# Alxaline/BraTS21

Measured on AMD Instinct MI355X. Metric: train patches/sec (4x128^3, width-48), higher is better.
Workload: dtype bf16; 1 GPU; equiunet width=48, batch=2/GPU of 4x128^3 synthetic patches, fwd + deep-supervision Dice + bwd + ranger (BASELINE.json configs[1]); global_batch=2, parallelism=dp1

## Files before the change

### brats21_amd/csrc/conv_wgrad.hip

```cpp
#include <stdlib.h>
#include "twin_begin.hpp"
#include "common.hpp"

typedef __attribute__((ext_vector_type(4))) short s16x4;

struct WgradParams {
  const void* x1; const void* x2; int c1, c2, p1, p2;
  const void* dy; int dyp;
  float* ws;
  int N, D, H, W, cin, cout;
  int tz, ty, tx, ntiles, nsplit;
  int nlane;
  int ntaps, dil;
  int seglen, nsegz;
};

constexpr int WG_TZ = 4, WG_TY = 4, WG_TX = 16, WG_VOX = 256;

template <typename T, int DIL, int COF, int CIF, int KS = 3>
struct WgGeom {
  static constexpr bool BF = std::is_same<T, bf16_t>::value;
  static constexpr int ESZ = sizeof(T);
  static constexpr int EPL = 16 / ESZ;
  static constexpr int R = KS == 3 ? DIL : 0;
  static constexpr int HY = WG_TY + 2 * R, HX = WG_TX + 2 * R;
  static constexpr int HVOX = WG_TZ * HY * HX;
  static constexpr int CI_T = 16 * CIF, CO_T = 16 * COF;
  static constexpr int XROWB = CI_T * ESZ, YROWB = CO_T * ESZ;
  static constexpr int SX = BF ? (CIF == 1 ? 32 : 96) : XROWB + 16;
  static constexpr int SY = BF ? (COF == 1 ? 32 : 96) : YROWB + 16;
  static constexpr int XPPV = XROWB / 16, YPPV = YROWB / 16;
  static constexpr int XPPR = HX * XPPV, XIPR = (XPPR + 63) / 64, XROWS = WG_TZ * HY, XRPW = (XROWS + 3) / 4;
  static constexpr int YPPR = WG_TX * YPPV, YIPR = (YPPR + 63) / 64, YROWS = WG_TZ * WG_TY, YRPW = YROWS / 4;
  static constexpr int LDS_X = HVOX * SX, LDS_Y = WG_VOX * SY;
  static constexpr int LDS = LDS_X + LDS_Y;
  static constexpr int PAIRS = (KS == 3 ? 9 : 1) * CIF;
  static constexpr int PPW = (PAIRS + 3) / 4;
  static constexpr int NB = BF ? 32 : 64;
};

DEVI bf16x8 tr_pair(const char* p0, const char* p1) {
  const s16x4 lo = __builtin_amdgcn_ds_read_tr16_b64_v4i16((__attribute__((address_space(3))) s16x4*)p0);
  const s16x4 hi = __builtin_amdgcn_ds_read_tr16_b64_v4i16((__attribute__((address_space(3))) s16x4*)p1);
  typedef __attribute__((ext_vector_type(8))) short s16x8;
  const s16x8 v = {lo[0], lo[1], lo[2], lo[3], hi[0], hi[1], hi[2], hi[3]};
  return __builtin_bit_cast(bf16x8, v);
}

template <typename T, int DIL, int COF, int CIF, int KS = 3>
__global__ __launch_bounds__(256, 2) void conv_wgrad_kernel(const WgradParams p) {
  using G = WgGeom<T, DIL, COF, CIF, KS>;
  extern __shared__ __attribute__((aligned(16))) char lds[];
  char* ldx = lds;
  char* ldy = lds + G::LDS_X;
  const int tid = threadIdx.x, lane = tid & 63;
  const int wave = __builtin_amdgcn_readfirstlane(tid >> 6);
  const int q = lane >> 4, v = lane & 15;
  const int NP = KS == 3 ? 3 : p.ntaps;
  const int lane8 = blockIdx.x % p.nlane, rr = blockIdx.x / p.nlane;
  const int tzg = rr % NP, gsub = rr / NP, g8 = gridDim.x / (NP * p.nlane);
  const int shz = (KS == 3 || p.ntaps == 1) ? 0 : (tzg / 9 - 1) * p.dil;
  const int shy = (KS == 3 || p.ntaps == 1) ? 0 : ((tzg / 3) % 3 - 1) * p.dil;
  const int shx = (KS == 3 || p.ntaps == 1) ? 0 : (tzg % 3 - 1) * p.dil;
  const int split = lane8 + p.nlane * gsub;
  const int tpx = (p.ntiles + p.nlane - 1) / p.nlane;
  const int tile_end = min(p.ntiles, (lane8 + 1) * tpx);
  const int cot = blockIdx.y, cit = blockIdx.z;
  const int co0 = cot * G::CO_T, ci0 = cit * G::CI_T;
  const T* xsrc;
  int xpitch;
  if (ci0 < p.c1) { xsrc = (const T*)p.x1 + ci0; xpitch = p.p1; }
  else { xsrc = (const T*)p.x2 + (ci0 - p.c1); xpitch = p.p2; }
  const int ci_lim = (ci0 < p.c1 ? p.c1 : p.c1 + p.c2) - ci0;
  const int co_lim = p.cout - co0;

  int xhx[G::XIPR], xlo[G::XIPR];
  int xvo[G::XRPW][G::XIPR];
#pragma unroll
  for (int j = 0; j < G::XIPR; ++j) {
    const int pc = lane + 64 * j;
    const int hx = pc / G::XPPV, part = pc % G::XPPV;
    const bool ok = pc < G::XPPR && part * G::EPL < ci_lim;
    xhx[j] = ok ? hx : -100000;
    xlo[j] = pc < G::XPPR ? wave * (G::HX * G::SX) + hx * G::SX + part * 16 : -1;
#pragma unroll
    for (int k = 0; k < G::XRPW; ++k) {
      const int row = wave + 4 * k;
      xvo[k][j] = (((row / G::HY) * p.H + row % G::HY) * p.W + hx) * xpitch * G::ESZ + part * 16;
    }
  }
  int yvx[G::YIPR], ylo[G::YIPR];
  int yvo[G::YRPW][G::YIPR];
#pragma unroll
  for (int j = 0; j < G::YIPR; ++j) {
    const int pc = lane + 64 * j;
    const int vx = pc / G::YPPV, part = pc % G::YPPV;
    const bool ok = pc < G::YPPR && part * G::EPL < co_lim;
    yvx[j] = ok ? vx : 100000;
    ylo[j] = pc < G::YPPR ? wave * (WG_TX * G::SY) + vx * G::SY + part * 16 : -1;
#pragma unroll
    for (int k = 0; k < G::YRPW; ++k) {
      const int row = wave + 4 * k;
      yvo[k][j] = (((row / WG_TY) * p.H + row % WG_TY) * p.W + vx) * p.dyp * G::ESZ + part * 16;
    }
  }
  const unsigned xsample_bytes = (unsigned)p.D * p.H * p.W * xpitch * G::ESZ;
  const unsigned ysample_bytes = (unsigned)p.D * p.H * p.W * p.dyp * G::ESZ;

  int poff[G::PPW];
#pragma unroll
  for (int jj = 0; jj < G::PPW; ++jj) {
    const int pid = wave + 4 * jj;
    const int t9 = pid / CIF, nn = pid % CIF;
    poff[jj] = pid < G::PAIRS ? (((t9 / 3) * G::R) * G::HX + (t9 % 3) * G::R) * G::SX + nn * G::NB : 0;
  }
  f32x4 acc[G::PPW][COF];
#pragma unroll
  for (int jj = 0; jj < G::PPW; ++jj)
#pragma unroll
    for (int m = 0; m < COF; ++m) acc[jj][m] = f32x4{0.f, 0.f, 0.f, 0.f};

  u32x4 rx[G::XRPW][G::XIPR], ry[G::YRPW][G::YIPR];
  auto issue_loads = [&](int tile) {
    int bt = tile;
    const int x0 = (bt % p.tx) * WG_TX; bt /= p.tx;
    const int y0 = (bt % p.ty) * WG_TY; bt /= p.ty;
    const int z0 = (bt % p.tz) * WG_TZ;
    const int n = bt / p.tz;
    const int gz0 = KS == 3 ? z0 + (tzg - 1) * DIL : z0 + shz;
    const int gy0 = KS == 3 ? y0 - DIL : y0 + shy, gx0 = KS == 3 ? x0 - DIL : x0 + shx;
    const size_t sample_vox = (size_t)n * p.D * p.H * p.W;
    const __amdgpu_buffer_rsrc_t xrs = __builtin_amdgcn_make_buffer_rsrc((void*)(xsrc + sample_vox * xpitch), (short)0,
                                                                          (int)xsample_bytes, 0x00020000);
    const __amdgpu_buffer_rsrc_t yrs = __builtin_amdgcn_make_buffer_rsrc((void*)((const T*)p.dy + sample_vox * p.dyp + co0),
                                                                          (short)0, (int)ysample_bytes, 0x00020000);
    const int xorg = ((gz0 * p.H + gy0) * p.W + gx0) * xpitch * G::ESZ;
    const int yorg = ((z0 * p.H + y0) * p.W + x0) * p.dyp * G::ESZ;
    bool xok[G::XIPR], yok[G::YIPR];
#pragma unroll
    for (int j = 0; j < G::XIPR; ++j) xok[j] = (unsigned)(gx0 + xhx[j]) < (unsigned)p.W;
#pragma unroll
    for (int j = 0; j < G::YIPR; ++j) yok[j] = x0 + yvx[j] < p.W;
#pragma unroll
    for (int k = 0; k < G::XRPW; ++k) {
      const int row = wave + 4 * k;
      const int gz = gz0 + row / G::HY, gy = gy0 + row % G::HY;
      const bool row_ok = row < G::XROWS && (unsigned)gz < (unsigned)p.D && (unsigned)gy < (unsigned)p.H;
#pragma unroll
      for (int j = 0; j < G::XIPR; ++j) {
        const int vo = (row_ok && xok[j]) ? xorg + xvo[k][j] : -1;
        rx[k][j] = __builtin_bit_cast(u32x4, __builtin_amdgcn_raw_buffer_load_b128(xrs, vo, 0, 0));
      }
    }
#pragma unroll
    for (int k = 0; k < G::YRPW; ++k) {
      const int row = wave + 4 * k;
      const bool row_ok = z0 + row / WG_TY < p.D && y0 + row % WG_TY < p.H;
#pragma unroll
      for (int j = 0; j < G::YIPR; ++j) {
        const int vo = (row_ok && yok[j]) ? yorg + yvo[k][j] : -1;
        ry[k][j] = __builtin_bit_cast(u32x4, __builtin_amdgcn_raw_buffer_load_b128(yrs, vo, 0, 0));
      }
    }
  };
  constexpr bool PREFETCH = !(G::BF && KS == 3 && DIL == 2 && COF * CIF == 9);
  const int tile_first = lane8 * tpx + gsub;
  if (PREFETCH && tile_first < tile_end) issue_loads(tile_first);
// ... 117 lines not shown
  const int ci_lim = (ci0 < p.c1 ? p.c1 : p.c1 + p.c2) - ci0;
  const T* xsrc;
  int xpitch;
  if (ci0 < p.c1) { xsrc = (const T*)p.x1 + ci0; xpitch = p.p1; }
  else { xsrc = (const T*)p.x2 + (ci0 - p.c1); xpitch = p.p2; }

  int xcode[G::XI], ycode[G::YI];
#pragma unroll
  for (int i = 0; i < G::XI; ++i) {
    const int P = tid + 512 * i;
    const int vox = P / G::XPPV, part = P % G::XPPV;
    const int hx = vox % G::HX, hy = (vox / G::HX) % G::HY, hz = vox / (G::HX * G::HY);
    xcode[i] = (P < G::XPIECES && part * 8 < ci_lim) ? (hz | hy << 3 | hx << 6 | part << 11 | 1 << 14) : 0;
  }
#pragma unroll
  for (int i = 0; i < G::YI; ++i) {
    const int P = tid + 512 * i;
    const int vox = P / G::YPPV, part = P % G::YPPV;
    ycode[i] = (vox >> 6) | ((vox >> 4) & 3) << 3 | (vox & 15) << 6 | part << 11 | 1 << 14;
  }
  const unsigned xsample_bytes = (unsigned)p.D * p.H * p.W * xpitch * 2;
  const unsigned ysample_bytes = (unsigned)p.D * p.H * p.W * p.dyp * 2;

  int poff[G::PPW];
#pragma unroll
  for (int jj = 0; jj < G::PPW; ++jj) {
    const int pid = wave + 8 * jj;
    const int t = pid / CIF, nn = pid % CIF;
    poff[jj] = pid < G::PAIRS ? (((t / 9) * G::HY + (t / 3) % 3) * G::HX + t % 3) * G::SX + nn * 32 : 0;
  }
  f32x4 acc[G::PPW][COF];
#pragma unroll
  for (int jj = 0; jj < G::PPW; ++jj)
#pragma unroll
    for (int m = 0; m < COF; ++m) acc[jj][m] = f32x4{0.f, 0.f, 0.f, 0.f};

  u32x4 rx[G::XI], ry[G::YI];
  auto issue_loads = [&](int tile) {
    int bt = tile;
    const int x0 = (bt % p.tx) * WG_TX; bt /= p.tx;
    const int y0 = (bt % p.ty) * WG_TY; bt /= p.ty;
    const int z0 = (bt % p.tz) * WG_TZ;
    const int n = bt / p.tz;
    const size_t sample_vox = (size_t)n * p.D * p.H * p.W;
    const __amdgpu_buffer_rsrc_t xrs = __builtin_amdgcn_make_buffer_rsrc((void*)(xsrc + sample_vox * xpitch), (short)0,
                                                                          (int)xsample_bytes, 0x00020000);
    const __amdgpu_buffer_rsrc_t yrs = __builtin_amdgcn_make_buffer_rsrc((void*)((const T*)p.dy + sample_vox * p.dyp + co0),
                                                                          (short)0, (int)ysample_bytes, 0x00020000);
    unsigned zm = 0, ym = 0, xm = 0, zy = 0, yy = 0, xy = 0;
#pragma unroll
    for (int h = 0; h < G::HZ; ++h) zm |= ((unsigned)(z0 - 1 + h) < (unsigned)p.D ? 1u : 0u) << h;
#pragma unroll
    for (int h = 0; h < G::HY; ++h) ym |= ((unsigned)(y0 - 1 + h) < (unsigned)p.H ? 1u : 0u) << h;
#pragma unroll
    for (int h = 0; h < G::HX; ++h) xm |= ((unsigned)(x0 - 1 + h) < (unsigned)p.W ? 1u : 0u) << h;
    zy = zm >> 1; yy = ym >> 1; xy = xm >> 1;
    const int xorg = ((z0 - 1) * p.H + (y0 - 1)) * p.W + (x0 - 1);
    const int yorg = (z0 * p.H + y0) * p.W + x0;
    const int xpb = xpitch * 2, ypb = p.dyp * 2;
#pragma unroll
    for (int i = 0; i < G::XI; ++i) {
      int c = xcode[i];
      asm volatile("" : "+v"(c));
      const unsigned ok = (unsigned)(c >> 14) & (zm >> (c & 7)) & (ym >> ((c >> 3) & 7)) & (xm >> ((c >> 6) & 31)) & 1u;
      const int pv = ((c & 7) * p.H + ((c >> 3) & 7)) * p.W + ((c >> 6) & 31);
      const int vo = ok ? (xorg + pv) * xpb + ((c >> 11) & 7) * 16 : -1;
      rx[i] = __builtin_bit_cast(u32x4, __builtin_amdgcn_raw_buffer_load_b128(xrs, vo, 0, 0));
    }
#pragma unroll
    for (int i = 0; i < G::YI; ++i) {
      int c = ycode[i];
      asm volatile("" : "+v"(c));
      const unsigned ok = (zy >> (c & 7)) & (yy >> ((c >> 3) & 7)) & (xy >> ((c >> 6) & 31)) & 1u;
      const int pv = ((c & 7) * p.H + ((c >> 3) & 7)) * p.W + ((c >> 6) & 31);
      const int vo = ok ? (yorg + pv) * ypb + ((c >> 11) & 7) * 16 : -1;
      ry[i] = __builtin_bit_cast(u32x4, __builtin_amdgcn_raw_buffer_load_b128(yrs, vo, 0, 0));
    }
  };

  const int tile_first = lane8 * tpx + gsub;
  if (tile_first < tile_end) issue_loads(tile_first);
  for (int tile = tile_first; tile < tile_end; tile += g8) {
    __syncthreads();
#pragma unroll
    for (int i = 0; i < G::XI; ++i)
      if (tid + 512 * i < G::XPIECES) *(u32x4*)(ldx + (tid + 512 * i) * 16) = rx[i];
#pragma unroll
    for (int i = 0; i < G::YI; ++i) {
      const int P = tid + 512 * i;
      *(u32x4*)(ldy + (P / G::YPPV) * G::SY + (P % G::YPPV) * 16) = ry[i];
    }
    __syncthreads();
    if (tile + g8 < tile_end) issue_loads(tile + g8);
    __builtin_amdgcn_sched_barrier(0);
    const int qq = v >> 2, pp = v & 3;
    const int ybase = (4 * q + qq) * G::SY + pp * 8;
    const int xbase = (4 * q + qq) * G::SX + pp * 8;
    constexpr int PD = 2;
    bf16x8 a[2][COF], b[PD + 1];
    auto read_a = [&](auto s_) {
      constexpr int s = s_;
      const int yoff = ybase + (32 * s) * G::SY;
#pragma unroll
      for (int m = 0; m < COF; ++m) a[s & 1][m] = tr_pair(ldy + yoff + m * 32, ldy + yoff + 16 * G::SY + m * 32);
    };
    auto read_b = [&](auto u_) {
      constexpr int u = u_;
      constexpr int s = u / G::PPW, jj = u % G::PPW;
      const int xoff = xbase + (((s >> 1) * G::HY + 2 * (s & 1)) * G::HX) * G::SX + poff[jj];
      b[u % (PD + 1)] = tr_pair(ldx + xoff, ldx + xoff + G::HX * G::SX);
    };
    constexpr int NU = 8 * G::PPW;
    read_a(std::integral_constant<int, 0>{});
    static_for<0, PD>([&](auto u_) { read_b(u_); });
    static_for<0, NU>([&](auto u_) {
      constexpr int u = u_;
      constexpr int s = u / G::PPW, jj = u % G::PPW;
      if constexpr (u + PD < NU) read_b(std::integral_constant<int, u + PD>{});
      if constexpr (jj == 0 && s + 1 < 8) read_a(std::integral_constant<int, s + 1>{});
      __builtin_amdgcn_sched_barrier(0);
#pragma unroll
      for (int m = 0; m < COF; ++m)
        acc[jj][m] = MFMA16_16x16x32(a[s & 1][m], b[u % (PD + 1)], acc[jj][m]);
      __builtin_amdgcn_sched_barrier(0);
    });
  }

#pragma unroll
  for (int jj = 0; jj < G::PPW; ++jj) {
    const int pid = wave + 8 * jj;
    if (pid < G::PAIRS) {
      const int t = pid / CIF, nn = pid % CIF;
      float* base = p.ws + ((size_t)split * 27 + t) * p.cout * p.cin;
      const int ci = ci0 + nn * 16 + v;
      if (nn * 16 + v < ci_lim) {
#pragma unroll
        for (int m = 0; m < COF; ++m)
#pragma unroll
          for (int r = 0; r < 4; ++r) base[(size_t)(co0 + m * 16 + 4 * q + r) * p.cin + ci] = acc[jj][m][r];
      }
    }
  }
}

template <int COF, int CIF> struct Wg3b {
  static constexpr int HZ = WG_TZ + 2, HY = WG_TY + 2, HX = WG_TX + 2, HVOX = HZ * HY * HX;
  static constexpr int CO = 16 * COF, CI = 16 * CIF;
  static constexpr int SX = 2 * CI, SY = 2 * CO, XPPV = CI / 8, YPPV = CO / 8;
  static constexpr int XPIECES = HVOX * XPPV, YPIECES = WG_VOX * YPPV;
  static constexpr int XI = (XPIECES + 511) / 512, YI = YPIECES / 512;
  static constexpr int XB = XI * 512 * 16;
  static constexpr int LDS = 2 * XB + WG_VOX * SY;
  static constexpr int PAIRS = 27 * CIF, PPW = (PAIRS + 7) / 8;
  static_assert(YPIECES % 512 == 0, "");
};

template <int COF, int CIF>
__global__ __launch_bounds__(512, 1) void conv_wgrad_alltaps2_kernel(const WgradParams p) {
  typedef bf16_t T;
  using G = Wg3b<COF, CIF>;
  extern __shared__ __attribute__((aligned(16))) char lds[];
  char* ldy = lds + 2 * G::XB;
  const int tid = threadIdx.x, lane = tid & 63;
  const int wave = __builtin_amdgcn_readfirstlane(tid >> 6);
  const int q = lane >> 4, v = lane & 15;
  const int lane8 = blockIdx.x % p.nlane, gsub = blockIdx.x / p.nlane, g8 = gridDim.x / p.nlane;
  const int split = blockIdx.x;
  const int tpx = (p.ntiles + p.nlane - 1) / p.nlane;
  const int tile_end = min(p.ntiles, (lane8 + 1) * tpx);
  const int co0 = blockIdx.y * G::CO, ci0 = blockIdx.z * G::CI;
  const T* xsrc;
  int xpitch;
  if (ci0 < p.c1) { xsrc = (const T*)p.x1 + ci0; xpitch = p.p1; }
  else { xsrc = (const T*)p.x2 + (ci0 - p.c1); xpitch = p.p2; }
  const int xpb = xpitch * 2, ypb = p.dyp * 2;

  int xoffs[G::XI], xcode[G::XI];
#pragma unroll
  for (int i = 0; i < G::XI; ++i) {
    const int P = tid + 512 * i;
    const int vox = P / G::XPPV, part = P % G::XPPV;
    const int hx = vox % G::HX, hy = (vox / G::HX) % G::HY, hz = vox / (G::HX * G::HY);
    const bool ok = P < G::XPIECES && (CIF > 1 || part * 8 < p.c1);
    xoffs[i] = ok ? ((hz * p.H + hy) * p.W + hx) * xpb + part * 16 : (int)0x80000000;
    xcode[i] = ok ? (hz | hy << 3 | hx << 6 | 1 << 14) : 0;
  }
  const unsigned xsample_bytes = (unsigned)p.D * p.H * p.W * xpitch * 2;
  const unsigned ysample_bytes = (unsigned)p.D * p.H * p.W * p.dyp * 2;

  int poff[G::PPW];
#pragma unroll
  for (int jj = 0; jj < G::PPW; ++jj) {
    const int pid = wave + 8 * jj;
    const int t = pid / CIF, nn = pid % CIF;
    poff[jj] = pid < G::PAIRS ? (((t / 9) * G::HY + (t / 3) % 3) * G::HX + t % 3) * G::SX + nn * 32 : 0;
  }
  f32x4 acc[G::PPW][COF];
#pragma unroll
  for (int jj = 0; jj < G::PPW; ++jj)
#pragma unroll
    for (int m = 0; m < COF; ++m) acc[jj][m] = f32x4{0.f, 0.f, 0.f, 0.f};

  u32x4 ry[G::YI];
  struct TileLoads {
    rsrc4_t xrs;
    __amdgpu_buffer_rsrc_t yrs;
    int xorg, yorg;
    unsigned zm, ym, xm, inter;
    char* xdst;
  };
  auto setup_loads = [&](int tile, int buf) {
    TileLoads L;
    int bt = tile;
    const int x0 = (bt % p.tx) * WG_TX; bt /= p.tx;
    const int y0 = (bt % p.ty) * WG_TY; bt /= p.ty;
    const int z0 = (bt % p.tz) * WG_TZ;
    const int n = bt / p.tz;
    const size_t sample_vox = (size_t)n * p.D * p.H * p.W;
    L.xrs = make_rsrc4(xsrc + sample_vox * xpitch, xsample_bytes);
    L.yrs = __builtin_amdgcn_make_buffer_rsrc((void*)((const T*)p.dy + sample_vox * p.dyp + co0), (short)0, (int)ysample_bytes, 0x00020000);
    L.xorg = (((z0 - 1) * p.H + (y0 - 1)) * p.W + (x0 - 1)) * xpb;
    L.yorg = ((z0 * p.H + y0) * p.W + x0) * ypb;
    L.xdst = lds + buf * G::XB + wave * 1024;
    auto inside = [](int o, int size, int hn) {
      const int lo = o >= 1 ? 0 : 1 - o, hi = size - o + 1 < hn ? size - o + 1 : hn;
      return hi > lo ? ((1u << hi) - 1u) & ~((1u << lo) - 1u) : 0u;
    };
    L.zm = inside(z0, p.D, G::HZ); L.ym = inside(y0, p.H, G::HY); L.xm = inside(x0, p.W, G::HX);
    L.inter = (L.zm == (1u << G::HZ) - 1 && L.ym == (1u << G::HY) - 1 && L.xm == (1u << G::HX) - 1) ? 1u : 0u;
    return L;
  };
  auto issue_x = [&](const TileLoads& L, auto i_) {
    constexpr int i = i_;
    const int c = xcode[i];
    const unsigned ok = (unsigned)(c >> 14) & (L.inter | ((L.zm >> (c & 7)) & (L.ym >> ((c >> 3) & 7)) & (L.xm >> ((c >> 6) & 31)))) & 1u;
    lds_dma16_async(L.xrs, L.xdst + i * 8192, (L.xorg + xoffs[i]) | ((int)ok - 1));
  };
  auto issue_y = [&](const TileLoads& L, auto i_) {
    constexpr int i = i_;
    const int P = tid + 512 * i;
    const int vox = P / G::YPPV, part = P % G::YPPV;
    const int z = vox >> 6, y = (vox >> 4) & 3, x = vox & 15;
    const int yo = ((z * p.H + y) * p.W + x) * ypb + part * 16;
    const unsigned ok = (L.inter | ((L.zm >> (z + 1)) & (L.ym >> (y + 1)) & (L.xm >> (x + 1)))) & 1u;
    ry[i] = __builtin_bit_cast(u32x4, __builtin_amdgcn_raw_buffer_load_b128(L.yrs, (L.yorg + yo) | ((int)ok - 1), 0, 0));
  };

  const int tile_first = lane8 * tpx + gsub;
  const int qq = v >> 2, pp = v & 3;
  const int ybase = (4 * q + qq) * G::SY + pp * 8;
  const int xbase = (4 * q + qq) * G::SX + pp * 8;
  int cur = 0;
#ifdef BRATS_WGRAD_STAMPS
  long long tacc[5] = {0, 0, 0, 0, 0}, tlast = __builtin_amdgcn_s_memtime();
#define WG_STAMP(i) do { const long long t_ = __builtin_amdgcn_s_memtime(); tacc[i] += t_ - tlast; tlast = t_; } while (0)
#else
#define WG_STAMP(i) do { } while (0)
#endif
  if (tile_first < tile_end) {
    const TileLoads L = setup_loads(tile_first, 0);
    static_for<0, G::XI>([&](auto i_) { issue_x(L, i_); });
    static_for<0, G::YI>([&](auto i_) { issue_y(L, i_); });
  }
  for (int tile = tile_first; tile < tile_end; tile += g8, cur ^= 1) {
    WG_STAMP(4);
    asm volatile("s_waitcnt vmcnt(0)" ::: "memory");
    WG_STAMP(0);
    __syncthreads();
    WG_STAMP(1);
#pragma unroll
    for (int i = 0; i < G::YI; ++i) *(u32x4*)(ldy + (tid + 512 * i) * 16) = ry[i];
    __syncthreads();
    WG_STAMP(2);
    const bool more = tile + g8 < tile_end;
    TileLoads L = setup_loads(more ? tile + g8 : tile, cur ^ 1);
    if (!more) L.zm = L.inter = 0;
    __builtin_amdgcn_sched_barrier(0);
    WG_STAMP(3);
    const char* ldx = lds + cur * G::XB;
    constexpr int PD = 3;
    bf16x8 a[2][COF], b[PD + 1];
    auto read_a = [&](auto s_) {
      constexpr int s = s_;
      const int yoff = ybase + (32 * s) * G::SY;
#pragma unroll
      for (int m = 0; m < COF; ++m) a[s & 1][m] = tr_pair(ldy + yoff + m * 32, ldy + yoff + 16 * G::SY + m * 32);
    };
    auto read_b = [&](auto u_) {
      constexpr int u = u_;
      constexpr int s = u / G::PPW, jj = u % G::PPW;
      const int xoff = xbase + (((s >> 1) * G::HY + 2 * (s & 1)) * G::HX) * G::SX + poff[jj];
      b[u % (PD + 1)] = tr_pair(ldx + xoff, ldx + xoff + G::HX * G::SX);
    };
    constexpr int NU = 8 * G::PPW;
    static_for<0, G::XI>([&](auto i_) { issue_x(L, i_); });
    static_for<0, G::YI>([&](auto i_) { issue_y(L, i_); });
    __builtin_amdgcn_sched_barrier(0);
    read_a(std::integral_constant<int, 0>{});
    static_for<0, PD>([&](auto u_) { read_b(u_); });
    static_for<0, NU>([&](auto u_) {
      constexpr int u = u_;
      constexpr int s = u / G::PPW, jj = u % G::PPW;
      if constexpr (u + PD < NU) read_b(std::integral_constant<int, u + PD>{});
      if constexpr (jj == 0 && s + 1 < 8) read_a(std::integral_constant<int, s + 1>{});
      __builtin_amdgcn_sched_barrier(0);
#pragma unroll
      for (int m = 0; m < COF; ++m)
        acc[jj][m] = MFMA16_16x16x32(a[s & 1][m], b[u % (PD + 1)], acc[jj][m]);
      __builtin_amdgcn_sched_barrier(0);
    });
  }

#ifdef BRATS_WGRAD_STAMPS
  WG_STAMP(4);
  if (lane == 0 && blockIdx.y == 0 && blockIdx.z == 0) {
    long long* st = (long long*)(p.ws + (size_t)gridDim.x * 27 * p.cout * p.cin) + ((size_t)blockIdx.x * 8 + wave) * 5;
    for (int i = 0; i < 5; ++i) st[i] = tacc[i];
  }
#endif
#pragma unroll
  for (int jj = 0; jj < G::PPW; ++jj) {
    const int pid = wave + 8 * jj;
    if (pid < G::PAIRS) {
      const int t = pid / CIF, nn = pid % CIF;
      float* base = p.ws + ((size_t)split * 27 + t) * p.cout * p.cin;
      const int ci = ci0 + nn * 16 + v;
      if (CIF > 1 || ci < p.cin) {
#pragma unroll
        for (int m = 0; m < COF; ++m)
#pragma unroll
          for (int r = 0; r < 4; ++r) base[(size_t)(co0 + m * 16 + 4 * q + r) * p.cin + ci] = acc[jj][m][r];
      }
    }
  }
}

template <int COF, int CIF> struct Wg3f {
  static constexpr int HZ = WG_TZ + 2, HY = WG_TY + 2, HX = WG_TX + 2, HVOX = HZ * HY * HX;
  static constexpr int CO = 16 * COF, CI = 16 * CIF;
  static constexpr int SX = CI, SY = CO;
  static constexpr int XPPV = CI / 8, YPPV = CO / 8;
  static constexpr int XPIECES = HVOX * XPPV, YPIECES = WG_VOX * YPPV;
  static constexpr int XI = (XPIECES + 511) / 512, YI = YPIECES / 512;
  static constexpr int XB = XI * 512 * 16, YB = YI * 512 * 16;
  static constexpr int LDS_X = HVOX * SX;
  static constexpr int LDS = XB + YB + LDS_X + WG_VOX * SY;
  static constexpr int PAIRS = 27 * CIF, PPW = (PAIRS + 7) / 8;
  static_assert(YPIECES % 512 == 0, "");
};

template <int STRIDE> DEVI i32x8 tr8_frag(const char* base, int o0, int o1) {
  typedef __attribute__((ext_vector_type(2))) int v2i;
  typedef __attribute__((address_space(3))) v2i* lp;
  const v2i a0 = __builtin_amdgcn_ds_read_tr8_b64_v2i32((lp)(base + o0));
  const v2i a1 = __builtin_amdgcn_ds_read_tr8_b64_v2i32((lp)(base + o0 + 8 * STRIDE));
  const v2i a2 = __builtin_amdgcn_ds_read_tr8_b64_v2i32((lp)(base + o1));
  const v2i a3 = __builtin_amdgcn_ds_read_tr8_b64_v2i32((lp)(base + o1 + 8 * STRIDE));
  return i32x8{a0[0], a0[1], a1[0], a1[1], a2[0], a2[1], a3[0], a3[1]};
}

struct WgradF8Params { WgradParams w; const float* amax_x1; const float* amax_x2; const float* amax_dy; };

template <int COF, int CIF>
__global__ __launch_bounds__(512, 1) void conv_wgrad_alltaps_f8_kernel(const WgradF8Params pp) {
  typedef bf16_t T;
  using G = Wg3f<COF, CIF>;
  const WgradParams& p = pp.w;
  extern __shared__ __attribute__((aligned(16))) char lds[];
  char* ldx = lds + G::XB + G::YB;
  char* ldy = ldx + G::LDS_X;
  const int tid = threadIdx.x, lane = tid & 63;
  const int wave = __builtin_amdgcn_readfirstlane(tid >> 6);
  const int kq = lane >> 4, L = lane & 15;
  const int lane8 = blockIdx.x % p.nlane, gsub = blockIdx.x / p.nlane, g8 = gridDim.x / p.nlane;
  const int split = blockIdx.x;
  const int tpx = (p.ntiles + p.nlane - 1) / p.nlane;
  const int tile_end = min(p.ntiles, (lane8 + 1) * tpx);
  const int co0 = blockIdx.y * G::CO, ci0 = blockIdx.z * G::CI;
  const T* xsrc;
  int xpitch;
  if (ci0 < p.c1) { xsrc = (const T*)p.x1 + ci0; xpitch = p.p1; }
  else { xsrc = (const T*)p.x2 + (ci0 - p.c1); xpitch = p.p2; }
  const int xpb = xpitch * 2, ypb = p.dyp * 2;
  float ax = *pp.amax_x1;
  if (pp.amax_x2) ax = fmaxf(ax, *pp.amax_x2);
  const float xs = f8_scale_from_amax(ax), ys = f8_scale_from_amax(*pp.amax_dy);

  int xoffs[G::XI], xcode[G::XI];
#pragma unroll
  for (int i = 0; i < G::XI; ++i) {
    const int P = tid + 512 * i;
    const int vox = P / G::XPPV, part = P % G::XPPV;
    const int hx = vox % G::HX, hy = (vox / G::HX) % G::HY, hz = vox / (G::HX * G::HY);
    const bool ok = P < G::XPIECES;
    xoffs[i] = ok ? ((hz * p.H + hy) * p.W + hx) * xpb + part * 16 : (int)0x80000000;
    xcode[i] = ok ? (hz | hy << 3 | hx << 6 | 1 << 14) : 0;
  }
  const unsigned xsample_bytes = (unsigned)p.D * p.H * p.W * xpitch * 2;
  const unsigned ysample_bytes = (unsigned)p.D * p.H * p.W * p.dyp * 2;

  int poff[G::PPW];
#pragma unroll
  for (int jj = 0; jj < G::PPW; ++jj) {
    const int pid = wave + 8 * jj;
    const int t = pid / CIF, nn = pid % CIF;
    poff[jj] = pid < G::PAIRS ? (((t / 9) * G::HY + (t / 3) % 3) * G::HX + t % 3) * G::SX + nn * 16 : 0;
  }
  f32x4 acc[G::PPW][COF];
#pragma unroll
  for (int jj = 0; jj < G::PPW; ++jj)
#pragma unroll
    for (int m = 0; m < COF; ++m) acc[jj][m] = f32x4{0.f, 0.f, 0.f, 0.f};

  struct TileLoads {
    rsrc4_t xrs, yrs;
    int xorg, yorg;
    unsigned zm, ym, xm, inter;
  };
  auto setup_loads = [&](int tile) {
    TileLoads T_;
    int bt = tile;
    const int x0 = (bt % p.tx) * WG_TX; bt /= p.tx;
    const int y0 = (bt % p.ty) * WG_TY; bt /= p.ty;
    const int z0 = (bt % p.tz) * WG_TZ;
    const int n = bt / p.tz;
    const size_t sample_vox = (size_t)n * p.D * p.H * p.W;
    T_.xrs = make_rsrc4(xsrc + sample_vox * xpitch, xsample_bytes);
    T_.yrs = make_rsrc4((const T*)p.dy + sample_vox * p.dyp + co0, ysample_bytes);
    T_.xorg = (((z0 - 1) * p.H + (y0 - 1)) * p.W + (x0 - 1)) * xpb;
    T_.yorg = ((z0 * p.H + y0) * p.W + x0) * ypb;
    auto inside = [](int o, int size, int hn) {
      const int lo = o >= 1 ? 0 : 1 - o, hi = size - o + 1 < hn ? size - o + 1 : hn;
      return hi > lo ? ((1u << hi) - 1u) & ~((1u << lo) - 1u) : 0u;
    };
    T_.zm = inside(z0, p.D, G::HZ); T_.ym = inside(y0, p.H, G::HY); T_.xm = inside(x0, p.W, G::HX);
    T_.inter = (T_.zm == (1u << G::HZ) - 1 && T_.ym == (1u << G::HY) - 1 && T_.xm == (1u << G::HX) - 1) ? 1u : 0u;
    return T_;
  };
  char* const xdst = lds + wave * 1024;
  auto issue_x = [&](const TileLoads& T_, auto i_) {
    constexpr int i = i_;
    int c = xcode[i];
    OPAQUE_V(c);
    const unsigned ok = (unsigned)(c >> 14) & (T_.inter | ((T_.zm >> (c & 7)) & (T_.ym >> ((c >> 3) & 7)) & (T_.xm >> ((c >> 6) & 31)))) & 1u;
    lds_dma16_async(T_.xrs, xdst + i * 8192, (T_.xorg + xoffs[i]) | ((int)ok - 1));
  };
  auto issue_y = [&](const TileLoads& T_, auto i_) {
    constexpr int i = i_;
    int t_ = tid;
    OPAQUE_V(t_);
    const int P = t_ + 512 * i;
    const int vox = P / G::YPPV, part = P % G::YPPV;
    const int z = vox >> 6, y = (vox >> 4) & 3, x = vox & 15;
    const int yo = ((z * p.H + y) * p.W + x) * ypb + part * 16;
    const unsigned ok = (T_.inter | ((T_.zm >> (z + 1)) & (T_.ym >> (y + 1)) & (T_.xm >> (x + 1)))) & 1u;
    lds_dma16_async(T_.yrs, xdst + G::XB + i * 8192, (T_.yorg + yo) | ((int)ok - 1));
  };

  int xl[2], yl[2];
#pragma unroll
  for (int e = 0; e < 2; ++e) {
    const int r = 2 * kq + e;
    xl[e] = (((r >> 2) * G::HY + (r & 3)) * G::HX + (L >> 1)) * G::SX + (L & 1) * 8;
    yl[e] = (r * 16 + (L >> 1)) * G::SY + (L & 1) * 8;
  }

  const int tile_first = lane8 * tpx + gsub;
  if (tile_first < tile_end) {
    const TileLoads T_ = setup_loads(tile_first);
    static_for<0, G::XI>([&](auto i_) { issue_x(T_, i_); });
    static_for<0, G::YI>([&](auto i_) { issue_y(T_, i_); });
  }
  for (int tile = tile_first; tile < tile_end; tile += g8) {
    asm volatile("s_waitcnt vmcnt(0)" ::: "memory");
    u32x2 qx[G::XI], qy[G::YI];
#pragma unroll
    for (int i = 0; i < G::XI; ++i) qx[i] = f8_quant8(*(const u32x4*)(lds + (tid + 512 * i) * 16), xs);
#pragma unroll
    for (int i = 0; i < G::YI; ++i) qy[i] = f8_quant8(*(const u32x4*)(lds + G::XB + (tid + 512 * i) * 16), ys);
    __syncthreads();
#pragma unroll
    for (int i = 0; i < G::XI; ++i)
      if (i + 1 < G::XI || tid + 512 * i < G::XPIECES) *(u32x2*)(ldx + (tid + 512 * i) * 8) = qx[i];
#pragma unroll
    for (int i = 0; i < G::YI; ++i) *(u32x2*)(ldy + (tid + 512 * i) * 8) = qy[i];
    __syncthreads();
    const bool more = tile + g8 < tile_end;
// ... 7 lines not shown
      constexpr int ks = ks_;
      const char* xk = ldx + ks * (2 * G::HY * G::HX * G::SX);
      i32x8 a[COF];
#pragma unroll
      for (int m = 0; m < COF; ++m) a[m] = tr8_frag<G::SY>(ldy + ks * (8 * 16 * G::SY) + m * 16, yl[0], yl[1]);
      i32x8 b[2];
      auto read_b = [&](auto jj_) {
        constexpr int jj = jj_;
        int o[2] = {xl[0] + poff[jj], xl[1] + poff[jj]};
        OPAQUE_V(o[0]); OPAQUE_V(o[1]);
        b[jj & 1] = tr8_frag<G::SX>(xk, o[0], o[1]);
      };
      read_b(std::integral_constant<int, 0>{});
      static_for<0, G::PPW>([&](auto jj_) {
        constexpr int jj = jj_;
        if constexpr (jj + 1 < G::PPW) read_b(std::integral_constant<int, jj + 1>{});
        __builtin_amdgcn_sched_barrier(0);
#pragma unroll
        for (int m = 0; m < COF; ++m)
          acc[jj][m] = __builtin_amdgcn_mfma_scale_f32_16x16x128_f8f6f4(a[m], b[jj & 1], acc[jj][m], 0, 0, 0, 0, 0, 0);
        __builtin_amdgcn_sched_barrier(0);
      });
    });
  }

  const float os = xs * ys;
#pragma unroll
  for (int jj = 0; jj < G::PPW; ++jj) {
    const int pid = wave + 8 * jj;
    if (pid < G::PAIRS) {
      const int t = pid / CIF, nn = pid % CIF;
      float* base = p.ws + ((size_t)split * 27 + t) * p.cout * p.cin;
      const int ci = ci0 + nn * 16 + L;
#pragma unroll
      for (int m = 0; m < COF; ++m)
#pragma unroll
        for (int r = 0; r < 4; ++r) base[(size_t)(co0 + m * 16 + 4 * kq + r) * p.cin + ci] = acc[jj][m][r] * os;
    }
  }
}

__global__ void __launch_bounds__(256) wgrad_reduce_kernel(const float* __restrict__ ws, float* __restrict__ dw, int nsplit,
                                                           int cout, int cin, int taps, const float* __restrict__ amax) {
  const size_t per = (size_t)taps * cout * cin;
  const size_t per4 = per / 4;
  const int e = threadIdx.x & 31, g = threadIdx.x >> 5;
  const size_t i4 = (size_t)blockIdx.x * 32 + e;
  f32x4 s = {0.f, 0.f, 0.f, 0.f};
  if (i4 < per4) {
    const float* src = ws + i4 * 4;
    int k = g;
    for (; k + 56 < nsplit; k += 64) {
      f32x4 v[8];
#pragma unroll
      for (int u = 0; u < 8; ++u) v[u] = *(const f32x4*)(src + (size_t)(k + 8 * u) * per);
#pragma unroll
      for (int u = 0; u < 8; ++u) s += v[u];
    }
    for (; k < nsplit; k += 8) s += *(const f32x4*)(src + (size_t)k * per);
  }
  __shared__ f32x4 part[8][32];
  part[g][e] = s;
  __syncthreads();
  if (g == 0 && i4 < per4) {
#pragma unroll
    for (int k = 1; k < 8; ++k) s += part[k][e];
    if (amax) s *= x3_inv_scale(x3_scale_from_amax(*amax));
    const size_t i = i4 * 4;
    const int ci = i % cin;
    const int co = (i / cin) % cout;
    const int tap = (int)(i / ((size_t)cin * cout));
#pragma unroll
    for (int j = 0; j < 4; ++j) dw[((size_t)co * cin + ci + j) * taps + tap] = s[j];
  }
}

__global__ void __launch_bounds__(256) wgrad_reduce_taps_kernel(const float* __restrict__ ws, float* __restrict__ dw, int nsplit,
                                                                int cout, int cin, int taps, const float* __restrict__ amax) {
  extern __shared__ __attribute__((aligned(16))) float red_tile[];
  const size_t per = (size_t)taps * cout * cin, pairs4 = (size_t)cout * cin / 4;
  const int e = threadIdx.x & 31, g = threadIdx.x >> 5;
  const size_t p4 = (size_t)blockIdx.x * 32 + e;
  if (p4 < pairs4) {
    f32x4 s[4];
#pragma unroll
    for (int t = 0; t < 4; ++t) s[t] = f32x4{0.f, 0.f, 0.f, 0.f};
    for (int k0 = 0; k0 < nsplit; k0 += 8) {
      f32x4 v[4][8];
#pragma unroll
      for (int t = 0; t < 4; ++t) {
        const int tap = g + 8 * t;
        const float* src = ws + ((size_t)(tap < taps ? tap : 0) * cout * cin + p4 * 4);
#pragma unroll
        for (int u = 0; u < 8; ++u)
          v[t][u] = (tap < taps && k0 + u < nsplit) ? *(const f32x4*)(src + (size_t)(k0 + u) * per) : f32x4{0.f, 0.f, 0.f, 0.f};
      }
#pragma unroll
      for (int t = 0; t < 4; ++t)
#pragma unroll
        for (int u = 0; u < 8; ++u)
          if (k0 + u < nsplit) s[t] += v[t][u];
    }
#pragma unroll
    for (int t = 0; t < 4; ++t)
      if (g + 8 * t < taps) *(f32x4*)(red_tile + (g + 8 * t) * 128 + e * 4) = s[t];
  }
  __syncthreads();
  const size_t pair0 = (size_t)blockIdx.x * 128, npairs = (size_t)cout * cin;
  float* dst = dw + pair0 * taps;
  const float isc = amax ? x3_inv_scale(x3_scale_from_amax(*amax)) : 1.f;
  for (int i = threadIdx.x; i < 128 * taps; i += blockDim.x) {
    const int pr = i / taps, tap = i % taps;
    if (pair0 + pr < npairs) dst[i] = red_tile[tap * 128 + pr] * isc;
  }
}

static void wgrad_reduce_launch(const float* ws, float* dw, int nsplit, int cout, int cin, int taps, hipStream_t st,
                                const float* amax = nullptr) {
  const size_t per = (size_t)taps * cout * cin;
  const size_t tblocks = ((size_t)cout * cin / 4 + 31) / 32;
  if (taps > 1 && taps <= 32 && tblocks >= 256)
    hipLaunchKernelGGL(wgrad_reduce_taps_kernel, dim3((unsigned)tblocks), dim3(256), (size_t)taps * 128 * sizeof(float), st, ws, dw,
                       nsplit, cout, cin, taps, amax);
  else
    hipLaunchKernelGGL(wgrad_reduce_kernel, dim3((unsigned)((per / 4 + 31) / 32)), dim3(256), 0, st, ws, dw, nsplit, cout, cin, taps, amax);
}

template <typename T>
__global__ void dbias_kernel(const T* __restrict__ dy, int pitch, float* __restrict__ db, size_t voxels, int C) {
  __shared__ float red[256];
  const int c = blockIdx.x;
  float s = 0.f;
  for (size_t v = threadIdx.x; v < voxels; v += blockDim.x) s += to_f<T>(dy[v * pitch + c]);
  red[threadIdx.x] = s;
  __syncthreads();
  for (int m = 128; m > 0; m >>= 1) {
    if ((int)threadIdx.x < m) red[threadIdx.x] += red[threadIdx.x + m];
    __syncthreads();
  }
  if (threadIdx.x == 0) db[c] = red[0];
}
static void wgrad_dbias_launch(int dtype, const void* dy, int dypitch, float* dbias, size_t vox, int cout, hipStream_t st) {
  with_storage(dtype, [&](auto t) {
    using T = typename decltype(t)::type;
    hipLaunchKernelGGL(dbias_kernel<T>, dim3(cout), dim3(256), 0, st, (const T*)dy, dypitch, dbias, vox, cout);
  });
}

struct WgradArgs {
  const void* x1; int c1, p1;
  const void* x2; int c2, p2;
  const void* dy; int dyp;
  int N, D, H, W, cout;
  int cin() const { return c1 + c2; }
  size_t vox() const { return (size_t)N * D * H * W; }
};
static WgradArgs wgrad_shape(int N, int D, int H, int W, int c1, int c2, int cout) {
  return WgradArgs{nullptr, c1, 0, nullptr, c2 > 0 ? c2 : 0, 0, nullptr, 0, N, D, H, W, cout};
}
static int wgrad_sample_overflow(const WgradArgs& a, int esize) {
  const int mp = a.p1 > a.p2 ? (a.p1 > a.dyp ? a.p1 : a.dyp) : (a.p2 > a.dyp ? a.p2 : a.dyp);
  return (double)a.D * a.H * a.W * mp * esize >= 2147483648.0 ? mp : 0;
}

struct WgradTileGrid { int tz, ty, tx, ntiles; };
static WgradTileGrid wgrad_tile_grid(const WgradArgs& a, int TZ = WG_TZ, int TY = WG_TY, int TX = WG_TX) {
  WgradTileGrid t{ceil_div(a.D, TZ), ceil_div(a.H, TY), ceil_div(a.W, TX), 0};
  t.ntiles = a.N * t.tz * t.ty * t.tx;
  return t;
}
static WgradParams wgrad_params(const WgradArgs& a, float* ws, const WgradTileGrid& t, int nlane, int nsplit, int ntaps, int dil) {
  WgradParams p{};
  p.x1 = a.x1; p.x2 = a.x2; p.c1 = a.c1; p.c2 = a.c2; p.p1 = a.p1; p.p2 = a.p2;
  p.dy = a.dy; p.dyp = a.dyp; p.ws = ws;
  p.N = a.N; p.D = a.D; p.H = a.H; p.W = a.W; p.cin = a.cin(); p.cout = a.cout;
  p.tz = t.tz; p.ty = t.ty; p.tx = t.tx; p.ntiles = t.ntiles;
  p.nlane = nlane; p.nsplit = nsplit; p.ntaps = ntaps; p.dil = dil;
  return p;
}

static int wgrad_nlane(int ntiles) {
  int nl = 8;
  while (nl > 1 && ntiles / nl < 16) nl >>= 1;
  return nl;
}
static int wgrad_split_g8(int ntiles, int nlane, int groups, int cot, int cit) {
  int g8 = ceil_div(512, groups * nlane * cot * cit);
  const int cap = ceil_div(ntiles, nlane);
  if (g8 > cap) g8 = cap;
  return g8 < 1 ? 1 : g8;
}
static bool wgrad_blocks_g8(int ntiles, int blocks, int* nlane, int* g8) {
  *nlane = wgrad_nlane(ntiles);
  *g8 = ceil_div(device_cus(), *nlane * blocks);
  if (*g8 < 1) *g8 = 1;
  return ntiles >= 4 * *nlane * *g8;
}
static void wgrad_tiles(int dtype, int c1, int c2, int cout, int* cof, int* cif) {
  const int co16 = ceil_div(cout, 16);
  *cof = co16 % 3 == 0 ? 3 : (co16 % 2 == 0 ? 2 : 1);
  if (dtype == BRATS_F32) { *cif = 1; return; }
  const int a = ceil_div(c1, 16), b = c2 > 0 ? ceil_div(c2, 16) : 0;
  auto ok = [&](int f) { return a % f == 0 && (b == 0 || b % f == 0); };
  *cif = ok(3) ? 3 : (ok(2) ? 2 : 1);
}

int g_wgrad_alltaps_mode = -1;
extern "C" int BRATS_API(brats_conv3d_set_wgrad_alltaps)(int mode) {
  const int old = g_wgrad_alltaps_mode;
  g_wgrad_alltaps_mode = mode < 0 ? -1 : (mode ? 1 : 0);
  return old;
}
static int wgrad_alltaps_mode() {
  static int env_mode = -1;
  if (env_mode < 0) {
    const char* e = getenv("BRATS_WGRAD_ALLTAPS");
    env_mode = e ? atoi(e) : 1;
  }
  return g_wgrad_alltaps_mode >= 0 ? g_wgrad_alltaps_mode : env_mode;
}

enum WgradForm {
  WG_TAP_PLANE, WG_SHIFTED_TAP,
  WG_ALLTAPS2_33, WG_ALLTAPS2_42, WG_ALLTAPS2_31,
  WG_ALLTAPS_1, WG_ALLTAPS_1_4,
  WG_F8_33, WG_F8_42
};
struct WgradPlan {
  WgradForm form;
  int cof, cif;
  int cot, cit;
  int nlane, g8, nsplit;
  int ntaps, groups;
  bool clear;
  WgradTileGrid tiles;
  size_t per;
  size_t slab_bytes() const { return nsplit * per * sizeof(float); }
};

static WgradPlan wgrad_plan(int dtype, bool shifted, int ksize, int dil, const WgradArgs& a) {
  WgradPlan pl;
  const int c1 = a.c1, c2 = a.c2, cin = a.cin(), cout = a.cout;
  pl.tiles = wgrad_tile_grid(a);
  pl.ntaps = ksize == 3 ? 27 : 1;
  pl.per = (size_t)pl.ntaps * cout * cin;
  const bool narrow = c2 == 0 && c1 <= 16;
  auto blocks_of = [&](int co, int ci) { return cout % co == 0 && (narrow || (c1 % ci == 0 && c2 % ci == 0)); };
  if (!shifted && wgrad_alltaps_mode() && dtype == BRATS_BF16 && dil == 1 && (blocks_of(48, 48) || blocks_of(64, 32))) {
    const bool wide = !blocks_of(48, 48);
    pl.cof = wide ? 4 : 3; pl.cif = narrow ? 1 : (wide ? 2 : 3);
    pl.cot = cout / (16 * pl.cof); pl.cit = narrow ? 1 : cin / (16 * pl.cif);
    if (wgrad_blocks_g8(pl.tiles.ntiles, pl.cot * pl.cit, &pl.nlane, &pl.g8)) {
      pl.form = wide ? (narrow ? WG_ALLTAPS_1_4 : WG_ALLTAPS2_42) : narrow ? (c1 % 8 == 0 ? WG_ALLTAPS2_31 : WG_ALLTAPS_1) : WG_ALLTAPS2_33;
      pl.groups = 1;
      pl.clear = false;
      pl.nsplit = pl.nlane * pl.g8;
      return pl;
    }
  }
  pl.form = shifted ? WG_SHIFTED_TAP : WG_TAP_PLANE;
  wgrad_tiles(dtype, c1, c2, cout, &pl.cof, &pl.cif);
  pl.cot = ceil_div(cout, 16 * pl.cof);
  pl.cit = ceil_div(c1, 16 * pl.cif) + (c2 > 0 ? ceil_div(c2, 16 * pl.cif) : 0);
  pl.groups = shifted ? pl.ntaps : 3;
  pl.nlane = wgrad_nlane(pl.tiles.ntiles);
  pl.g8 = wgrad_split_g8(pl.tiles.ntiles, pl.nlane, pl.groups, pl.cot, pl.cit);
  pl.nsplit = pl.nlane * pl.g8;
  pl.clear = cin % 16 || cout % 16;
  return pl;
}
static size_t wgrad_slab_room(int dtype, bool shifted, int ksize, const WgradArgs& a) {
  const size_t d1 = wgrad_plan(dtype, shifted, ksize, 1, a).slab_bytes();
  const size_t d2 = shifted ? 0 : wgrad_plan(dtype, shifted, ksize, 2, a).slab_bytes();
  return d1 > d2 ? d1 : d2;
}

template <typename T, int DIL, int COF, int CIF, int KS = 3>
static int wgrad_launch(const WgradParams& p, dim3 grid, hipStream_t st) {
  using G = WgGeom<T, DIL, COF, CIF, KS>;
  auto kern = conv_wgrad_kernel<T, DIL, COF, CIF, KS>;
  static std::atomic<uint64_t> attr_done{0};
  BRATS_ENSURE_LDS_ATTR(kern, G::LDS, attr_done);
  hipLaunchKernelGGL(kern, grid, dim3(256), G::LDS, st, p);
  BRATS_CHECK_LAUNCH();
  return 0;
}

template <typename T, int DIL, int KS = 3>
static int wgrad_dispatch(const WgradParams& p, int cof, int cif, dim3 grid, hipStream_t st) {
#define WG_CASE(A, B) if (cof == A && cif == B) return wgrad_launch<T, DIL, A, B, KS>(p, grid, st);
  WG_CASE(3, 1) WG_CASE(2, 1) WG_CASE(1, 1)
  if constexpr (std::is_same<T, bf16_t>::value) {
    WG_CASE(3, 3) WG_CASE(3, 2) WG_CASE(2, 3) WG_CASE(2, 2) WG_CASE(1, 3) WG_CASE(1, 2)
  }
#undef WG_CASE
  BRATS_FAIL(BRATS_E_UNSUPPORTED, "wgrad: unsupported tile %dx%d", cof, cif);
}

template <auto KERN, int LDS>
static int wgrad_alltaps_launch(const WgradParams& p, dim3 grid, hipStream_t st) {
  static std::atomic<uint64_t> attr_done{0};
  BRATS_ENSURE_LDS_ATTR(KERN, LDS, attr_done);
  hipLaunchKernelGGL(KERN, grid, dim3(512), LDS, st, p);
  BRATS_CHECK_LAUNCH();
  return 0;
}

static int wgrad_run(const WgradPlan& pl, int dtype, int dil, const WgradArgs& a, float* ws, size_t room, hipStream_t st) {
  const char* who = pl.form == WG_SHIFTED_TAP ? "wgrad_shift" : "wgrad";
  if (a.c2 > 0 && a.c1 % (16 * pl.cif)) BRATS_FAIL(BRATS_E_UNSUPPORTED, "wgrad: c1=%d must be a multiple of the ci tile %d", a.c1, 16 * pl.cif);
  if (pl.slab_bytes() > room) BRATS_FAIL(BRATS_E_ARG, "%s: the plan's %zu bytes of slabs exceed the workspace size %zu", who, pl.slab_bytes(), room);
  const WgradParams p = wgrad_params(a, ws, pl.tiles, pl.nlane, pl.nsplit, pl.ntaps, dil);
  if (pl.clear) {
    hipError_t e = hipMemsetAsync(ws, 0, pl.slab_bytes(), st);
    if (e != hipSuccess) BRATS_FAIL(BRATS_E_HIP, "%s: memset: %s", who, hipGetErrorString(e));
  }
  const dim3 grid(pl.groups * pl.nsplit, pl.cot, pl.cit);
  const bool bf = dtype == BRATS_BF16;
  switch (pl.form) {
    case WG_TAP_PLANE:
      if (bf) return dil == 1 ? wgrad_dispatch<bf16_t, 1>(p, pl.cof, pl.cif, grid, st) : wgrad_dispatch<bf16_t, 2>(p, pl.cof, pl.cif, grid, st);
      return dil == 1 ? wgrad_dispatch<float, 1>(p, pl.cof, pl.cif, grid, st) : wgrad_dispatch<float, 2>(p, pl.cof, pl.cif, grid, st);
    case WG_SHIFTED_TAP:
      return bf ? wgrad_dispatch<bf16_t, 1, 1>(p, pl.cof, pl.cif, grid, st) : wgrad_dispatch<float, 1, 1>(p, pl.cof, pl.cif, grid, st);
    case WG_ALLTAPS2_33: return wgrad_alltaps_launch<conv_wgrad_alltaps2_kernel<3, 3>, Wg3b<3, 3>::LDS>(p, grid, st);
    case WG_ALLTAPS2_42: return wgrad_alltaps_launch<conv_wgrad_alltaps2_kernel<4, 2>, Wg3b<4, 2>::LDS>(p, grid, st);
    case WG_ALLTAPS2_31: return wgrad_alltaps_launch<conv_wgrad_alltaps2_kernel<3, 1>, Wg3b<3, 1>::LDS>(p, grid, st);
    case WG_ALLTAPS_1: return wgrad_alltaps_launch<conv_wgrad_alltaps_kernel<1>, Wg3<1>::LDS>(p, grid, st);
    case WG_ALLTAPS_1_4: return wgrad_alltaps_launch<conv_wgrad_alltaps_kernel<1, 4>, Wg3<1, 4>::LDS>(p, grid, st);
    default: BRATS_FAIL(BRATS_E_UNSUPPORTED, "wgrad: form %d is not a 16-bit / f32 kernel", (int)pl.form);
  }
}

template <int V>
__global__ void __launch_bounds__(256) x3_split_kernel(const float* __restrict__ src, int pitch, bf16_t* __restrict__ hi,
                                                       bf16_t* __restrict__ lo, size_t voxels, int C, const float* __restrict__ amax) {
  const float sc = amax ? x3_scale_from_amax(*amax) : 1.f;
  const int cv = C / 8;
  const size_t total = voxels * cv;
  const size_t stride = (size_t)gridDim.x * 256;
  auto load = [&](size_t i, u32x4& a, u32x4& b) {
    const float* p = src + (i / cv) * pitch + (i % cv) * 8;
    a = __builtin_nontemporal_load((const u32x4*)p);
    b = __builtin_nontemporal_load((const u32x4*)(p + 4));
  };
  auto emit = [&](size_t i, const u32x4& a, const u32x4& b) {
    const uint32_t w[8] = {a[0], a[1], a[2], a[3], b[0], b[1], b[2], b[3]};
    uint32_t h[4], l[4];
#pragma unroll
    for (int e = 0; e < 4; ++e) {
      const float x0 = __uint_as_float(w[2 * e]) * sc, x1 = __uint_as_float(w[2 * e + 1]) * sc;
      x3_split2(x0, x1, h[e], l[e]);
    }
    const size_t o = (i / cv) * C + (i % cv) * 8;
    __builtin_nontemporal_store(u32x4{h[0], h[1], h[2], h[3]}, (u32x4*)(hi + o));
    __builtin_nontemporal_store(u32x4{l[0], l[1], l[2], l[3]}, (u32x4*)(lo + o));
  };
  size_t i = (size_t)blockIdx.x * 256 + threadIdx.x;
  for (; i + stride < total; i += 2 * stride) {
    u32x4 a0, b0, a1, b1;
    load(i, a0, b0);
    load(i + stride, a1, b1);
    emit(i, a0, b0);
    emit(i + stride, a1, b1);
  }
  if (i < total) {
    u32x4 a0, b0;
    load(i, a0, b0);
    emit(i, a0, b0);
  }
}
static size_t x3_align(size_t b) { return (b + 255) / 256 * 256; }
static void x3_split_launch(const float* src, int pitch, bf16_t* hi, bf16_t* lo, size_t vox, int c, const float* amax, hipStream_t st) {
  const size_t total = vox * (c / 8);
  size_t nb = (total + 511) / 512;
  const unsigned blocks = (unsigned)(nb < 1 ? 1 : (nb > 262144 ? 262144 : nb));
  hipLaunchKernelGGL(x3_split_kernel<0>, dim3(blocks), dim3(256), 0, st, src, pitch, hi, lo, vox, c, amax);
}

struct X3Carve {
  size_t off[7];
  X3Carve(size_t room16, const WgradArgs& a) {
    const int c[3] = {a.c1, a.c2, a.cout};
    size_t b = x3_align(3 * room16);
    for (int i = 0; i < 6; ++i) {
      off[i] = b;
      b += c[i / 2] > 0 ? x3_align(a.vox() * c[i / 2] * 2) : 0;
    }
    off[6] = b;
  }
  size_t bytes() const { return off[6]; }
  bf16_t* at(float* ws, int i) const { return (bf16_t*)((char*)ws + off[i]); }
};

static int wgrad_x3(const WgradPlan& pl, int dil, const WgradArgs& a, const float* amax_dy, float* ws, float* dw, size_t room16,
                          hipStream_t st) {
  const X3Carve cv(room16, a);
  bf16_t *h1 = cv.at(ws, 0), *l1 = cv.at(ws, 1), *h2 = cv.at(ws, 2), *l2 = cv.at(ws, 3), *hy = cv.at(ws, 4), *ly = cv.at(ws, 5);
  x3_split_launch((const float*)a.x1, a.p1, h1, l1, a.vox(), a.c1, nullptr, st);
  if (a.c2 > 0) x3_split_launch((const float*)a.x2, a.p2, h2, l2, a.vox(), a.c2, nullptr, st);
  x3_split_launch((const float*)a.dy, a.dyp, hy, ly, a.vox(), a.cout, amax_dy, st);
  BRATS_CHECK_LAUNCH();
  WgradArgs t = a;
  t.p1 = a.c1; t.p2 = a.c2; t.dyp = a.cout;
  const bool xlo[3] = {true, false, false}, ylo[3] = {false, true, false};
  for (int k = 0; k < 3; ++k) {
    t.x1 = xlo[k] ? l1 : h1;
    t.x2 = a.c2 > 0 ? (xlo[k] ? l2 : h2) : nullptr;
    t.dy = ylo[k] ? ly : hy;
    const int rc = wgrad_run(pl, BRATS_BF16, dil, t, ws + (size_t)k * pl.nsplit * pl.per, room16, st);
    if (rc) return rc;
  }
  wgrad_reduce_launch((const float*)ws, dw, 3 * pl.nsplit, a.cout, a.cin(), pl.ntaps, st, amax_dy);
  return 0;
}

#include "conv_wgrad_x3.hpp"
extern "C" int BRATS_API(brats_conv3d_set_x3_wgrad_fused)(int mode) {
  const int old = g_x3_wgrad_fused_mode;
  g_x3_wgrad_fused_mode = mode < 0 ? -1 : (mode > 2 ? 2 : mode);
  return old;
}

static size_t wgrad_ws_bytes(int dtype, bool shifted, int ksize, const WgradArgs& a) {
  if (dtype != BRATS_X3_BF16) return wgrad_slab_room(dtype, shifted, ksize, a);
  const size_t three = X3Carve(wgrad_slab_room(BRATS_BF16, shifted, ksize, a), a).bytes();
  const size_t fused = shifted ? 0 : wgrad_x3_fused_ws_bytes(a);
  return three > fused ? three : fused;
}
extern "C" size_t BRATS_API(brats_conv3d_wgrad_ws_bytes)(int dtype, int ksize, int N, int D, int H, int W, int c1, int c2, int cout) {
  return ksize == 3 ? wgrad_ws_bytes(dtype, false, 3, wgrad_shape(N, D, H, W, c1, c2, cout)) : 0;
}
extern "C" size_t BRATS_API(brats_conv3d_wgrad_shift_ws_bytes)(int dtype, int ksize, int N, int D, int H, int W, int cin, int cout) {
  return ksize == 1 || ksize == 3 ? wgrad_ws_bytes(dtype, true, ksize, wgrad_shape(N, D, H, W, cin, 0, cout)) : 0;
}

static int wgrad_impl(bool shifted, WgradArgs a, const float* amax_dy, float* ws, float* dw, float* dbias, int dtype, int ksize, int dil,
                      brats_stream_t s) {
  const char* who = shifted ? "wgrad_shift" : "wgrad";
  if (!a.x1 || !a.dy || !ws || !dw || a.c1 <= 0 || a.cout <= 0 || (shifted && (a.N <= 0 || a.D <= 0 || a.H <= 0 || a.W <= 0)))
    BRATS_FAIL(BRATS_E_ARG, "%s: null pointer / bad size", who);
  if (shifted ? (ksize != 1 && ksize != 3) || dil < 1 : ksize != 3 || (dil != 1 && dil != 2))
    BRATS_FAIL(BRATS_E_UNSUPPORTED, "%s: ksize=%d dil=%d unsupported", who, ksize, dil);
  if (shifted && dtype != BRATS_BF16 && dtype != BRATS_F32 && dtype != BRATS_X3_BF16) BRATS_FAIL(BRATS_E_UNSUPPORTED, "wgrad_shift: dtype %d", dtype);
  if (a.c2 < 0) a.c2 = 0;
  if (a.c2 > 0 && !a.x2) BRATS_FAIL(BRATS_E_ARG, "wgrad: c2 > 0 but x2 NULL");
  const bool x3 = dtype == BRATS_X3_BF16;
  const int epl = vec_width(dtype);
  if (a.p1 % epl || (a.c2 && a.p2 % epl) || a.dyp % epl || a.c1 % epl || a.c2 % epl || a.cout % epl)
    BRATS_FAIL(BRATS_E_ARG, "%s: channel counts / pitches must be multiples of %d", who, epl);
  if (x3 && (a.c1 % 8 || a.c2 % 8 || a.cout % 8)) BRATS_FAIL(BRATS_E_ARG, "%s (split precision): channel counts must be multiples of 8", who);
  if (const int mp = wgrad_sample_overflow(a, dtype == BRATS_BF16 ? 2 : 4))
    BRATS_FAIL(BRATS_E_UNSUPPORTED, "%s: one sample of %dx%dx%d x pitch %d exceeds the 2 GiB buffer-offset range", who, a.D, a.H, a.W, mp);
  hipStream_t st = (hipStream_t)s;
  int rc = x3 && !shifted ? wgrad_x3_fused(a, amax_dy, ws, dw, dil, st) : 1;
  if (rc == 1) {
    const int dt = x3 ? BRATS_BF16 : dtype;
    const WgradPlan pl = wgrad_plan(dt, shifted, ksize, dil, a);
    const size_t room = wgrad_slab_room(dt, shifted, ksize, a);
    if (x3) rc = wgrad_x3(pl, dil, a, amax_dy, ws, dw, room, st);
    else if (!(rc = wgrad_run(pl, dtype, dil, a, ws, room, st))) wgrad_reduce_launch((const float*)ws, dw, pl.nsplit, a.cout, a.cin(), pl.ntaps, st);
  }
  if (rc) return rc;
  if (dbias) wgrad_dbias_launch(dtype, a.dy, a.dyp, dbias, a.vox(), a.cout, st);
  BRATS_CHECK_LAUNCH();
  return 0;
}

extern "C" int BRATS_API(brats_conv3d_wgrad)(const void* x1, int c1, int pitch1, const void* x2, int c2, int pitch2, const void* dy,
                                  int dypitch, float* ws, float* dw, float* dbias, int dtype, int ksize, int dil, int N,
                                  int D, int H, int W, int cout, brats_stream_t s) {
  return wgrad_impl(false, WgradArgs{x1, c1, pitch1, x2, c2, pitch2, dy, dypitch, N, D, H, W, cout}, nullptr, ws, dw, dbias, dtype, ksize, dil, s);
}
extern "C" int BRATS_API(brats_conv3d_x3_wgrad)(const void* x1, int c1, int pitch1, const void* x2, int c2, int pitch2, const void* dy,
                                     int dypitch, const float* amax_dy, float* ws, float* dw, float* dbias, int dtype, int dil,
                                     int N, int D, int H, int W, int cout, brats_stream_t s) {
  if (dtype != BRATS_X3_BF16) BRATS_FAIL(BRATS_E_ARG, "conv3d_x3_wgrad: dtype must be BRATS_X3_F16 or BRATS_X3_BF16");
  return wgrad_impl(false, WgradArgs{x1, c1, pitch1, x2, c2, pitch2, dy, dypitch, N, D, H, W, cout}, amax_dy, ws, dw, dbias, dtype, 3, dil, s);
}
extern "C" int BRATS_API(brats_conv3d_wgrad_shift)(const void* x, int cin, int xpitch, const void* dy, int dypitch, float* ws, float* dw,
                                        float* dbias, int dtype, int ksize, int dil, int N, int D, int H, int W, int cout,
                                        brats_stream_t s) {
  return wgrad_impl(true, WgradArgs{x, cin, xpitch, nullptr, 0, 0, dy, dypitch, N, D, H, W, cout}, nullptr, ws, dw, dbias, dtype, ksize, dil, s);
}
extern "C" int BRATS_API(brats_conv3d_x3_wgrad_shift)(const void* x, int cin, int xpitch, const void* dy, int dypitch, const float* amax_dy,
                                           float* ws, float* dw, float* dbias, int dtype, int ksize, int dil, int N, int D, int H,
                                           int W, int cout, brats_stream_t s) {
  if (dtype != BRATS_X3_BF16) BRATS_FAIL(BRATS_E_ARG, "conv3d_x3_wgrad_shift: dtype must be BRATS_X3_F16 or BRATS_X3_BF16");
  return wgrad_impl(true, WgradArgs{x, cin, xpitch, nullptr, 0, 0, dy, dypitch, N, D, H, W, cout}, amax_dy, ws, dw, dbias, dtype, ksize, dil, s);
}

static bool wgrad_f8_plan(const WgradArgs& a, WgradPlan* pl) {
  const int c1 = a.c1, c2 = a.c2, cout = a.cout;
  if (c1 <= 0 || cout <= 0) return false;
  if (cout % 48 == 0 && c1 % 48 == 0 && c2 % 48 == 0) { pl->form = WG_F8_33; pl->cof = 3; pl->cif = 3; }
  else if (cout % 64 == 0 && c1 % 32 == 0 && c2 % 32 == 0) { pl->form = WG_F8_42; pl->cof = 4; pl->cif = 2; }
  else return false;
  pl->tiles = wgrad_tile_grid(a);
  pl->cot = cout / (16 * pl->cof); pl->cit = a.cin() / (16 * pl->cif);
  if (!wgrad_blocks_g8(pl->tiles.ntiles, pl->cot * pl->cit, &pl->nlane, &pl->g8)) return false;
  pl->nsplit = pl->nlane * pl->g8;
  pl->ntaps = 27; pl->groups = 1; pl->clear = false;
  pl->per = (size_t)27 * cout * a.cin();
  return true;
}

extern "C" size_t BRATS_API(brats_conv3d_wgrad_f8_ws_bytes)(int N, int D, int H, int W, int c1, int c2, int cout) {
  WgradPlan pl;
  return wgrad_f8_plan(wgrad_shape(N, D, H, W, c1, c2, cout), &pl) ? pl.slab_bytes() : 0;
}

template <int COF, int CIF>
static int wgrad_f8_launch(const WgradF8Params& pp, dim3 grid, hipStream_t st) {
  using G = Wg3f<COF, CIF>;
  auto kern = conv_wgrad_alltaps_f8_kernel<COF, CIF>;
  static std::atomic<uint64_t> attr_done{0};
  BRATS_ENSURE_LDS_ATTR(kern, G::LDS, attr_done);
  hipLaunchKernelGGL(kern, grid, dim3(512), G::LDS, st, pp);
  BRATS_CHECK_LAUNCH();
  return 0;
}

extern "C" int BRATS_API(brats_conv3d_wgrad_f8)(const void* x1, int c1, int pitch1, const float* amax1, const void* x2, int c2, int pitch2,
                                     const float* amax2, const void* dy, int dypitch, const float* amax_dy, float* ws, float* dw,
                                     int N, int D, int H, int W, int cout, brats_stream_t s) {
  if (!x1 || !dy || !ws || !dw || !amax1 || !amax_dy || c1 <= 0 || cout <= 0) BRATS_FAIL(BRATS_E_ARG, "wgrad_f8: null pointer / bad size");
  if (c2 < 0) c2 = 0;
  if (c2 > 0 && (!x2 || !amax2)) BRATS_FAIL(BRATS_E_ARG, "wgrad_f8: c2 > 0 needs x2 and its |max|");
  const WgradArgs a{x1, c1, pitch1, x2, c2, pitch2, dy, dypitch, N, D, H, W, cout};
  WgradPlan pl;
  if (!wgrad_f8_plan(a, &pl))
    BRATS_FAIL(BRATS_E_UNSUPPORTED, "wgrad_f8: built for 48 x 48 / 64 x 32 channel blocks of layers with enough tiles "
               "(brats_conv3d_wgrad_f8_ws_bytes() == 0 otherwise): use brats_conv3d_wgrad");
  if (pitch1 % 8 || (c2 && pitch2 % 8) || dypitch % 8) BRATS_FAIL(BRATS_E_ARG, "wgrad_f8: pitches must be multiples of 8");
  if (wgrad_sample_overflow(a, 2)) BRATS_FAIL(BRATS_E_UNSUPPORTED, "wgrad_f8: sample exceeds the 2 GiB buffer-offset range");
  const WgradF8Params pp{wgrad_params(a, ws, pl.tiles, pl.nlane, pl.nsplit, 27, 1), amax1, c2 ? amax2 : nullptr, amax_dy};
  hipStream_t st = (hipStream_t)s;
  const dim3 grid(pl.nsplit, pl.cot, pl.cit);
  const int rc = pl.form == WG_F8_33 ? wgrad_f8_launch<3, 3>(pp, grid, st) : wgrad_f8_launch<4, 2>(pp, grid, st);
  if (rc) return rc;
  wgrad_reduce_launch((const float*)ws, dw, pl.nsplit, cout, a.cin(), 27, st);
  BRATS_CHECK_LAUNCH();
  return 0;
}
#include "twin_end.hpp"
```

### brats21_amd/csrc/norm.hip

```cpp
#include "twin_begin.hpp"
#include "common.hpp"

#include "se.hpp"

constexpr int GN_MAX_SPLITS = 64;
__global__ void gn_chan_reduce_kernel(const float* __restrict__ stats, int tps, int C, double* __restrict__ part) {
  const int n = blockIdx.y, c0 = blockIdx.x * 16;
  const int cl = threadIdx.x & 15, tl = threadIdx.x >> 4;
  const int c = c0 + cl;
  const int per = (tps + gridDim.z - 1) / gridDim.z;
  const int t0 = blockIdx.z * per, t1 = min(tps, t0 + per);
  double s1 = 0.0, s2 = 0.0;
  if (c < C) {
    for (int t = t0 + tl; t < t1; t += 16) {
      const f32x2 v = *(const f32x2*)(stats + (((size_t)n * tps + t) * C + c) * 2);
      s1 += v[0];
      s2 += v[1];
    }
  }
  __shared__ double r1[256], r2[256];
  r1[threadIdx.x] = s1;
  r2[threadIdx.x] = s2;
  __syncthreads();
  for (int m = 128; m >= 16; m >>= 1) {
    if ((int)threadIdx.x < m) { r1[threadIdx.x] += r1[threadIdx.x + m]; r2[threadIdx.x] += r2[threadIdx.x + m]; }
    __syncthreads();
  }
  if (threadIdx.x < 16 && c < C) {
    double* dst = part + (((size_t)blockIdx.z * gridDim.y + n) * C + c) * 2;
    dst[0] = r1[threadIdx.x];
    dst[1] = r2[threadIdx.x];
  }
}

static int gn_splits(int tps) {
  int splits = tps / 64;
  return splits < 1 ? 1 : (splits > GN_MAX_SPLITS ? GN_MAX_SPLITS : splits);
}

static int chan_reduce_launch(const float* stats, int tps, int N, int C, double* chan_ws, hipStream_t st) {
  hipLaunchKernelGGL(gn_chan_reduce_kernel, dim3((C + 15) / 16, N, gn_splits(tps)), dim3(256), 0, st, stats, tps, C,
                     chan_ws + (size_t)N * C * 2);
  return 0;
}

__global__ void gn_finalize_kernel(double* __restrict__ chan, int splits, int N, int C, int groups, double count_per_channel,
                                   float eps, int unbiased, const float* __restrict__ gamma, const float* __restrict__ beta,
                                   float* __restrict__ mean_rstd, float* __restrict__ scale_shift) {
  const int n = blockIdx.x / groups, g = blockIdx.x % groups;
  const int cpg = C / groups;
  __shared__ double r1[256], r2[256];
  double s1 = 0.0, s2 = 0.0;
  {
    const int ZL = 256 / cpg;
    const int cl = threadIdx.x % cpg, zl = threadIdx.x / cpg;
    const double* part = chan + (size_t)N * C * 2;
    double p1 = 0.0, p2 = 0.0;
    if (zl < ZL) {
      const int c = g * cpg + cl;
      for (int z = zl; z < splits; z += ZL) {
        p1 += part[(((size_t)z * N + n) * C + c) * 2];
        p2 += part[(((size_t)z * N + n) * C + c) * 2 + 1];
      }
    }
    r1[threadIdx.x] = p1;
    r2[threadIdx.x] = p2;
    __syncthreads();
    if ((int)threadIdx.x < cpg) {
      for (int z = 0; z < ZL; ++z) { s1 += r1[z * cpg + threadIdx.x]; s2 += r2[z * cpg + threadIdx.x]; }
      const int c = g * cpg + threadIdx.x;
      chan[((size_t)n * C + c) * 2] = s1;
      chan[((size_t)n * C + c) * 2 + 1] = s2;
    }
    __syncthreads();
  }
  r1[threadIdx.x] = s1;
  r2[threadIdx.x] = s2;
  __syncthreads();
  for (int m = blockDim.x / 2; m > 0; m >>= 1) {
    if ((int)threadIdx.x < m) { r1[threadIdx.x] += r1[threadIdx.x + m]; r2[threadIdx.x] += r2[threadIdx.x + m]; }
    __syncthreads();
  }
  const double M = count_per_channel * cpg;
  const double mean = r1[0] / M;
  double var = r2[0] / M - mean * mean;
  if (unbiased) var = var * M / (M - 1.0);
  if (var < 0.0) var = 0.0;
  const float rstd = (float)(1.0 / sqrt(var + (double)eps));
  if (threadIdx.x == 0) {
    mean_rstd[(n * groups + g) * 2] = (float)mean;
    mean_rstd[(n * groups + g) * 2 + 1] = rstd;
  }
  if (scale_shift && (int)threadIdx.x < cpg) {
    const int c = g * cpg + threadIdx.x;
    const float sc = rstd * gamma[c];
    scale_shift[((size_t)n * C + c) * 2] = sc;
    scale_shift[((size_t)n * C + c) * 2 + 1] = beta[c] - (float)mean * sc;
  }
}

__global__ void __launch_bounds__(1024) gn_finalize_direct_kernel(const float* __restrict__ stats, int tps, double* __restrict__ chan,
                                                                  int N, int C, int groups, double count_per_channel, float eps,
                                                                  int unbiased, const float* __restrict__ gamma,
                                                                  const float* __restrict__ beta, float* __restrict__ mean_rstd,
                                                                  float* __restrict__ scale_shift) {
  const int n = blockIdx.x / groups, g = blockIdx.x % groups;
  const int cpg = C / groups;
  __shared__ double r1[1024], r2[1024];
  const int TL = 1024 / cpg;
  const int cl = threadIdx.x % cpg, tl = threadIdx.x / cpg;
  double p1 = 0.0, p2 = 0.0;
  if (tl < TL) {
    const float* src = stats + (((size_t)n * tps) * C + g * cpg + cl) * 2;
    int t = tl;
    for (; t + 7 * TL < tps; t += 8 * TL) {
      f32x2 v[8];
#pragma unroll
      for (int u = 0; u < 8; ++u) v[u] = *(const f32x2*)(src + (size_t)(t + u * TL) * C * 2);
#pragma unroll
      for (int u = 0; u < 8; ++u) { p1 += v[u][0]; p2 += v[u][1]; }
    }
    for (; t < tps; t += TL) {
      const f32x2 v = *(const f32x2*)(src + (size_t)t * C * 2);
      p1 += v[0];
      p2 += v[1];
    }
  }
  r1[threadIdx.x] = p1;
  r2[threadIdx.x] = p2;
  __syncthreads();
  double s1 = 0.0, s2 = 0.0;
  if ((int)threadIdx.x < cpg) {
    for (int z = 0; z < TL; ++z) { s1 += r1[z * cpg + threadIdx.x]; s2 += r2[z * cpg + threadIdx.x]; }
    const int c = g * cpg + threadIdx.x;
    chan[((size_t)n * C + c) * 2] = s1;
    chan[((size_t)n * C + c) * 2 + 1] = s2;
  }
  __syncthreads();
  r1[threadIdx.x] = s1;
  r2[threadIdx.x] = s2;
  __syncthreads();
  for (int m = 128; m > 0; m >>= 1) {
    if ((int)threadIdx.x < m) { r1[threadIdx.x] += r1[threadIdx.x + m]; r2[threadIdx.x] += r2[threadIdx.x + m]; }
    __syncthreads();
  }
  const double M = count_per_channel * cpg;
  const double mean = r1[0] / M;
  double var = r2[0] / M - mean * mean;
  if (unbiased) var = var * M / (M - 1.0);
  if (var < 0.0) var = 0.0;
  const float rstd = (float)(1.0 / sqrt(var + (double)eps));
  if (threadIdx.x == 0) {
    mean_rstd[(n * groups + g) * 2] = (float)mean;
    mean_rstd[(n * groups + g) * 2 + 1] = rstd;
  }
  if (scale_shift && (int)threadIdx.x < cpg) {
    const int c = g * cpg + threadIdx.x;
    const float sc = rstd * gamma[c];
    scale_shift[((size_t)n * C + c) * 2] = sc;
    scale_shift[((size_t)n * C + c) * 2 + 1] = beta[c] - (float)mean * sc;
  }
}

static int gn_finalize_launch(const float* stats, int tps, int N, int C, int groups, double count_per_channel, float eps, int unbiased,
                              const float* gamma, const float* beta, float* mean_rstd, float* scale_shift, double* chan_ws,
                              hipStream_t st) {
  if ((size_t)tps * (C / groups) <= 32768) {
    hipLaunchKernelGGL(gn_finalize_direct_kernel, dim3(N * groups), dim3(1024), 0, st, stats, tps, chan_ws, N, C, groups,
                       count_per_channel, eps, unbiased, gamma, beta, mean_rstd, scale_shift);
  } else {
    if (int rc = chan_reduce_launch(stats, tps, N, C, chan_ws, st)) return rc;
    hipLaunchKernelGGL(gn_finalize_kernel, dim3(N * groups), dim3(256), 0, st, chan_ws, gn_splits(tps), N, C, groups, count_per_channel,
                       eps, unbiased, gamma, beta, mean_rstd, scale_shift);
  }
  BRATS_CHECK_LAUNCH();
  return 0;
}

extern "C" size_t BRATS_API(brats_gn_ws_doubles)(int N, int C) { return (size_t)(1 + GN_MAX_SPLITS) * N * C * 2; }

extern "C" int BRATS_API(brats_gn_finalize)(const float* stats, int tiles_per_sample, int N, int C, int groups,
                                 double count_per_channel, float eps, const float* gamma, const float* beta,
                                 float* mean_rstd, float* scale_shift, double* chan_ws, brats_stream_t s) {
  if (!stats || !mean_rstd || !chan_ws || C % groups || C / groups > 256) BRATS_FAIL(BRATS_E_ARG, "gn_finalize: bad argument");
  if (scale_shift && (!gamma || !beta)) BRATS_FAIL(BRATS_E_ARG, "gn_finalize: scale_shift needs gamma/beta");
  return gn_finalize_launch(stats, tiles_per_sample, N, C, groups, count_per_channel, eps, 0, gamma, beta, mean_rstd, scale_shift, chan_ws,
                            (hipStream_t)s);
}

struct SlopeArg { float v; const float* p; };
template <bool HEAVY>
DEVI float act_fwd(float x, int act, float slope) {
  if (act == BRATS_ACT_RELU) return x > 0.f ? x : 0.f;
  if (act == BRATS_ACT_LEAKY) return x > 0.f ? x : x * slope;
  if constexpr (!HEAVY) return x;
  if (act == BRATS_ACT_ELU) return x > 0.f ? x : expm1f(x);
  if (act == BRATS_ACT_SWISH) return x / (1.f + __expf(-x));
  if (act == BRATS_ACT_MISH) {
    const float sp = x > 20.f ? x : log1pf(__expf(x));
    return x * tanhf(sp);
  }
  return x;
}
template <bool HEAVY>
DEVI float act_grad(float x, int act, float slope) {
  if (act == BRATS_ACT_RELU) return x > 0.f ? 1.f : 0.f;
  if (act == BRATS_ACT_LEAKY) return x > 0.f ? 1.f : slope;
  if constexpr (!HEAVY) return 1.f;
  if (act == BRATS_ACT_ELU) return x > 0.f ? 1.f : __expf(x);
  if (act == BRATS_ACT_SWISH) {
    const float sg = 1.f / (1.f + __expf(-x));
    return sg * (1.f + x * (1.f - sg));
  }
  if (act == BRATS_ACT_MISH) {
    const float sp = x > 20.f ? x : log1pf(__expf(x));
    const float th = tanhf(sp);
    const float sg = 1.f / (1.f + __expf(-x));
    return th + x * (1.f - th * th) * sg;
  }
  return 1.f;
}

template <typename T> DEVI void record_absmax(float mx, uint32_t* amax) {
  mx = to_f<T>(from_f<T>(mx));
#pragma unroll
  for (int o = 32; o > 0; o >>= 1) mx = fmaxf(mx, __shfl_xor(mx, o, 64));
  __shared__ float wmax[16];
  if ((threadIdx.x & 63) == 0) wmax[threadIdx.x >> 6] = mx;
  __syncthreads();
  if (threadIdx.x == 0) {
    for (int w = 1; w < (int)(blockDim.x >> 6); ++w) mx = fmaxf(mx, wmax[w]);
    const uint32_t bits = __float_as_uint(mx);
    if (bits > *(volatile uint32_t*)amax) atomicMax(amax, bits);
  }
}

template <typename T, bool HEAVY, bool NT = false>
__global__ void __launch_bounds__(256) affine_act_kernel(const T* __restrict__ y, int ypitch, const float* __restrict__ scale_shift,
                                                         T* __restrict__ z, int zpitch, int act, SlopeArg sl, int voxels, int C,
                                                         uint32_t* __restrict__ amax) {
  constexpr int VW = 16 / sizeof(T);
  const float slope = sl.p ? *sl.p : sl.v;
  const int n = blockIdx.y;
  const int cv = C / VW;
  const int vl_n = blockDim.x / cv;
  const int mycv = threadIdx.x % cv, myvl = threadIdx.x / cv;
  const bool live = myvl < vl_n;
  const int c0 = mycv * VW;
  float sc[VW], sh[VW];
#pragma unroll
  for (int j = 0; j < VW; ++j) {
    sc[j] = scale_shift[((size_t)n * C + c0 + j) * 2];
    sh[j] = scale_shift[((size_t)n * C + c0 + j) * 2 + 1];
  }
  const T* yb = y + (size_t)n * voxels * ypitch + c0;
  T* zb = z + (size_t)n * voxels * zpitch + c0;
  const int stride = gridDim.x * vl_n;
  float mx = 0.f;
  auto run = [&](auto relu_) {
    constexpr bool RELU = decltype(relu_)::value;
    auto body = [&](float* a) {
#pragma unroll
      for (int j = 0; j < VW; ++j) {
        const float t = a[j] * sc[j] + sh[j];
        if constexpr (RELU) a[j] = __builtin_fmaxf(t, 0.f);
        else a[j] = act_fwd<HEAVY>(t, act, slope);
      }
      if (amax) {
#pragma unroll
        for (int j = 0; j < VW; j += 2) mx = __builtin_fmaxf(__builtin_fmaxf(mx, __builtin_fabsf(a[j])), __builtin_fabsf(a[j + 1]));
      }
    };
    int vox = live ? blockIdx.x * vl_n + myvl : voxels;
    for (; vox + stride < voxels; vox += 2 * stride) {
      float a0[VW], a1[VW];
      vload<T, VW, NT>(yb + (size_t)vox * ypitch, a0);
      vload<T, VW, NT>(yb + (size_t)(vox + stride) * ypitch, a1);
      body(a0);
      body(a1);
      vstore<T, VW, NT>(zb + (size_t)vox * zpitch, a0);
      vstore<T, VW, NT>(zb + (size_t)(vox + stride) * zpitch, a1);
    }
    if (vox < voxels) {
      float a0[VW];
      vload<T, VW, NT>(yb + (size_t)vox * ypitch, a0);
      body(a0);
      vstore<T, VW, NT>(zb + (size_t)vox * zpitch, a0);
    }
  };
  if (!HEAVY && act == BRATS_ACT_RELU) run(std::true_type{});
  else run(std::false_type{});
  if (amax) record_absmax<T>(mx, amax);
}

extern "C" int BRATS_API(brats_affine_act_fwd)(const void* y, int ypitch, const float* scale_shift, void* z, int zpitch,
                                    int dtype, int act, float slope_value, const float* slope_dev, int N, int voxels, int C,
                                    float* amax, brats_stream_t s) {
  const SlopeArg slope{slope_value, slope_dev};
  const int vw = vec_width(dtype);
  if (!y || !z || !scale_shift || C % vw || ypitch % vw || zpitch % vw || C / vw > 256)
    BRATS_FAIL(BRATS_E_ARG, "affine_act_fwd: C and pitches must be multiples of %d (C <= %d)", vw, 256 * vw);
  const bool big = big_tensor(dtype, (size_t)N * voxels * C);
  dim3 grid(voxel_walk(vw, voxels, C).grid(big ? 8192 : 2048), N);
  with_act_stream(dtype, act > BRATS_ACT_LEAKY, big, [&](auto t, auto heavy, auto nt) {
    using T = typename decltype(t)::type;
    hipLaunchKernelGGL((affine_act_kernel<T, decltype(heavy)::value, decltype(nt)::value>), grid, dim3(256), 0, (hipStream_t)s, (const T*)y,
                       ypitch, scale_shift, (T*)z, zpitch, act, slope, voxels, C, (uint32_t*)amax);
  });
  BRATS_CHECK_LAUNCH();
  return 0;
}

template <typename T> struct Raw16;
template <> struct Raw16<bf16_t> {
  typedef u32x4 type;
  template <bool NT> static DEVI type load(const bf16_t* p) {
    if constexpr (NT) return __builtin_nontemporal_load((const u32x4*)p); else return *(const u32x4*)p;
  }
  static DEVI void unpack(const type& v, float* o) {
#pragma unroll
    for (int i = 0; i < 4; ++i) unpack2(v[i], o[2 * i], o[2 * i + 1]);
  }
};
template <> struct Raw16<float> {
  typedef f32x4 type;
  template <bool NT> static DEVI type load(const float* p) { return *(const f32x4*)p; }
  static DEVI void unpack(const type& v, float* o) { o[0] = v[0]; o[1] = v[1]; o[2] = v[2]; o[3] = v[3]; }
};

template <typename T, bool NT = false, bool AM = false>
__global__ void __launch_bounds__(256) affine_act_pool_kernel(const T* __restrict__ y, int ypitch, const float* __restrict__ scale_shift,
                                                              T* __restrict__ z, int zpitch, T* __restrict__ p, int ppitch, int act,
                                                              SlopeArg sl, int D, int H, int W, int C, int with_avg,
                                                              uint32_t* __restrict__ amax, uint8_t* __restrict__ argmax) {
  constexpr int VW = 16 / sizeof(T);
  typedef typename Raw16<T>::type raw_t;
  extern __shared__ __attribute__((aligned(16))) char pool_lds[];
  raw_t* xch = (raw_t*)pool_lds;
  const float slope = sl.p ? *sl.p : sl.v;
  const bool relu = act == BRATS_ACT_RELU;
  const int n = blockIdx.y;
  const int cv = C / VW;
  int xb = (blockDim.x / cv) & ~1;
  if (xb > W) xb = W;
  const int mycv = threadIdx.x % cv, myvl = threadIdx.x / cv, c0 = mycv * VW;
  const bool lane_on = myvl < xb;
  const int Do = D / 2, Ho = H / 2, Wo = W / 2;
  const int segs = (W + xb - 1) / xb;
  const size_t items = (size_t)Do * Ho * segs, voxels = (size_t)D * H * W;
  float sc[VW], sh[VW];
#pragma unroll
  for (int j = 0; j < VW; ++j) {
    sc[j] = lane_on ? scale_shift[((size_t)n * C + c0 + j) * 2] : 0.f;
    sh[j] = lane_on ? scale_shift[((size_t)n * C + c0 + j) * 2 + 1] : 0.f;
  }
  const T* yb = y + (size_t)n * voxels * ypitch + c0;
  T* zb = z + (size_t)n * voxels * zpitch + c0;
  T* pb = p + (size_t)n * Do * Ho * Wo * ppitch + c0;
  float amx = 0.f;
  int buf = 0;
  for (size_t item = blockIdx.x; item < items; item += gridDim.x, buf ^= 1) {
// ... 270 lines not shown
          for (int k = 0; k < HK; ++k) gq[i][k] = dl[(size_t)k * voxels + v0 + i * stride];
#pragma unroll
        for (int i = 0; i < NV; ++i) {
          float yy[VW];
          Raw16<T>::unpack(yr[i], yy);
          hbody(gq[i], yy);
        }
      };
      for (; vox + 3 * stride < (size_t)voxels; vox += 4 * stride) step(vox, std::integral_constant<int, 4>{});
      for (; vox < (size_t)voxels; vox += stride) step(vox, std::integral_constant<int, 1>{});
#pragma unroll
      for (int j = 0; j < VW; ++j) a2[j] = a2[j] * rs[j] + mo[j] * a1[j];
    } else {
    auto body = [&](const float* g, const float* yy) {
#pragma unroll
      for (int j = 0; j < VW; ++j) {
        const float u = g[j] * act_grad<HEAVY>(yy[j] * sc[j] + sh[j], act, slope);
        a1[j] += u;
        a2[j] += u * (yy[j] * rs[j] + mo[j]);
      }
    };
    for (; vox + 3 * stride < (size_t)voxels; vox += 4 * stride) {
      float g0[VW], y0[VW], g1[VW], y1[VW], g2[VW], y2[VW], g3[VW], y3[VW];
      vload<T, VW, NT>(dzb + vox * dzpitch, g0);
      vload<T, VW, NT>(yb + vox * ypitch, y0);
      vload<T, VW, NT>(dzb + (vox + stride) * dzpitch, g1);
      vload<T, VW, NT>(yb + (vox + stride) * ypitch, y1);
      vload<T, VW, NT>(dzb + (vox + 2 * stride) * dzpitch, g2);
      vload<T, VW, NT>(yb + (vox + 2 * stride) * ypitch, y2);
      vload<T, VW, NT>(dzb + (vox + 3 * stride) * dzpitch, g3);
      vload<T, VW, NT>(yb + (vox + 3 * stride) * ypitch, y3);
      body(g0, y0);
      body(g1, y1);
      body(g2, y2);
      body(g3, y3);
    }
    for (; vox < (size_t)voxels; vox += stride) {
      float g0[VW], y0[VW];
      vload<T, VW, NT>(dzb + vox * dzpitch, g0);
      vload<T, VW, NT>(yb + vox * ypitch, y0);
      body(g0, y0);
    }
    }
  }
  float* scr = sm;
  if (myvl < vl_n) {
#pragma unroll
    for (int j = 0; j < VW; ++j) {
      scr[(myvl * C + c0 + j) * 2] = a1[j];
      scr[(myvl * C + c0 + j) * 2 + 1] = a2[j];
    }
  }
  __syncthreads();
  float* part = red + (size_t)gridDim.y * C * 2 + ((size_t)blockIdx.x * gridDim.y + n) * C * 2;
  for (int i = threadIdx.x; i < 2 * C; i += blockDim.x) {
    float t = 0.f;
    for (int l = 0; l < vl_n; ++l) t += scr[l * C * 2 + i];
    part[i] = t;
  }
  if constexpr (HK > 0) {
    const bool live = myvl < vl_n;
    float* hb = sm + vl_n * C * 2;
    if (live && mycv == 0) {
#pragma unroll
      for (int k = 0; k < HK; ++k) hb[myvl * HK + k] = ab[k];
    }
    float* hp = hf.hpart + ((size_t)n * gridDim.x + blockIdx.x) * (HK * C + HK);
#pragma unroll
    for (int k = 0; k < HK; ++k)
      lane_reduce_plane<VW>(sm, aw[k], live, myvl, vl_n, C, c0, [&](int c, float t) { hp[k * C + c] = t; });
    if ((int)threadIdx.x < HK) {
      float t = 0.f;
      for (int l = 0; l < vl_n; ++l) t += hb[l * HK + threadIdx.x];
      hp[HK * C + threadIdx.x] = t;
    }
  }
}

__global__ void __launch_bounds__(256) gn_bwd_finish_kernel(float* __restrict__ red, int nb, int total ) {
  const int e = threadIdx.x & 7, g = threadIdx.x >> 3;
  const int i = blockIdx.x * 8 + e;
  const float* part = red + total;
  float s = 0.f;
  if (i < total) {
    const float* src = part + i;
    int b = g;
    for (; b + 7 * 32 < nb; b += 8 * 32) {
      float v[8];
#pragma unroll
      for (int u = 0; u < 8; ++u) v[u] = src[(size_t)(b + 32 * u) * total];
#pragma unroll
      for (int u = 0; u < 8; ++u) s += v[u];
    }
    for (; b < nb; b += 32) s += src[(size_t)b * total];
  }
  __shared__ float sm[32][8];
  sm[g][e] = s;
  __syncthreads();
  if (g == 0 && i < total) {
#pragma unroll
    for (int k = 1; k < 32; ++k) s += sm[k][e];
    red[i] = s;
  }
}

template <typename T, bool HEAVY, bool NT = false, int HK = 0>
__global__ void __launch_bounds__(256) gn_bwd_apply_kernel(const T* __restrict__ dz, int dzpitch, const T* __restrict__ y,
                                                           int ypitch, const float* __restrict__ scale_shift,
                                                           const float* __restrict__ mean_rstd, const float* __restrict__ gamma,
                                                           const float* __restrict__ red, T* __restrict__ dy, int dypitch,
                                                           float* __restrict__ dgamma, float* __restrict__ dbeta, int act,
                                                           SlopeArg sl, int N, int voxels, int C, int groups,
                                                           uint32_t* __restrict__ amax, HeadFold hf) {
  constexpr int VW = 16 / sizeof(T);
  constexpr int HKA = HK > 0 ? HK : 1;
  const float slope = sl.p ? *sl.p : sl.v;
  extern __shared__ float sm[];
  float* m12 = sm;
  const int n = blockIdx.y;
  const int cpg = C / groups;
  const float invM = 1.f / ((float)cpg * (float)voxels);
  for (int g = threadIdx.x; g < groups; g += blockDim.x) {
    float t1 = 0.f, t2 = 0.f;
    for (int j = 0; j < cpg; ++j) {
      const int c = g * cpg + j;
      t1 += gamma[c] * red[((size_t)n * C + c) * 2];
      t2 += gamma[c] * red[((size_t)n * C + c) * 2 + 1];
    }
    m12[g * 2] = t1 * invM;
    m12[g * 2 + 1] = t2 * invM;
  }
  if (blockIdx.x == 0 && blockIdx.y == 0 && dgamma) {
    for (int c = threadIdx.x; c < C; c += blockDim.x) {
      float b = 0.f, g = 0.f;
      for (int m = 0; m < N; ++m) { b += red[((size_t)m * C + c) * 2]; g += red[((size_t)m * C + c) * 2 + 1]; }
      dbeta[c] = b;
      dgamma[c] = g;
    }
  }
  __syncthreads();
  const int cv = C / VW;
  const int vl_n = blockDim.x / cv;
  const int mycv = threadIdx.x % cv, myvl = threadIdx.x / cv;
  const bool live = myvl < vl_n;
  const int c0 = mycv * VW;
  float sc[VW], sh[VW], ca[VW], cb[VW], ck[VW];
#pragma unroll
  for (int j = 0; j < VW; ++j) {
    const int c = c0 + j, g = c / cpg;
    sc[j] = scale_shift[((size_t)n * C + c) * 2];
    sh[j] = scale_shift[((size_t)n * C + c) * 2 + 1];
    const float mean = mean_rstd[(n * groups + g) * 2], rstd = mean_rstd[(n * groups + g) * 2 + 1];
    const float m1 = m12[g * 2], m2 = m12[g * 2 + 1];
    ca[j] = rstd * gamma[c];
    cb[j] = -rstd * rstd * m2;
    ck[j] = rstd * (mean * rstd * m2 - m1);
  }
  const T* dzb = dz + (size_t)n * voxels * dzpitch + c0;
  const T* yb = y + (size_t)n * voxels * ypitch + c0;
  T* dyb = dy + (size_t)n * voxels * dypitch + c0;
  const size_t stride = (size_t)gridDim.x * vl_n;
  size_t vox = live ? (size_t)blockIdx.x * vl_n + myvl : (size_t)voxels;
  float mx = 0.f;
  auto body = [&](const float* g, const float* yy, float* o) {
#pragma unroll
    for (int j = 0; j < VW; ++j) {
      const float u = g[j] * act_grad<HEAVY>(yy[j] * sc[j] + sh[j], act, slope);
      o[j] = u * ca[j] + (yy[j] * cb[j] + ck[j]);
    }
    if (amax) {
#pragma unroll
      for (int j = 0; j < VW; j += 2) mx = __builtin_fmaxf(__builtin_fmaxf(mx, __builtin_fabsf(o[j])), __builtin_fabsf(o[j + 1]));
    }
  };
  if constexpr (HK < 0) {
    const float nslope = act == BRATS_ACT_RELU ? 0.f : slope;
    auto step = [&](size_t v0, auto cnt) {
      constexpr int NVX = decltype(cnt)::value;
      typename Raw16<T>::type yr[NVX], skr[NVX], dpr[NVX], avr[NVX];
      uint32_t aw[NVX][VW / 4];
      int kk[NVX];
#pragma unroll
      for (int i = 0; i < NVX; ++i) {
        yr[i] = Raw16<T>::template load<NT>(yb + (v0 + i * stride) * ypitch);
        pool_dz<T, VW>(hf, n, v0 + i * stride, c0, C, skr[i], dpr[i], avr[i], aw[i], kk[i]);
      }
#pragma unroll
      for (int i = 0; i < NVX; ++i) {
        float yy[VW], g[VW], o[VW];
        Raw16<T>::unpack(yr[i], yy);
        pool_dz_finish<T, VW>(skr[i], dpr[i], avr[i], hf.with_avg, aw[i], kk[i], g);
#pragma unroll
        for (int j = 0; j < VW; ++j) {
          const float u = g[j] * (yy[j] * sc[j] + sh[j] > 0.f ? 1.f : nslope);
          o[j] = u * ca[j] + (yy[j] * cb[j] + ck[j]);
        }
        if (amax) {
#pragma unroll
          for (int j = 0; j < VW; j += 2) mx = __builtin_fmaxf(__builtin_fmaxf(mx, __builtin_fabsf(o[j])), __builtin_fabsf(o[j + 1]));
        }
        vstore<T, VW, NT>(dyb + (v0 + i * stride) * dypitch, o);
      }
    };
    for (; vox + stride < (size_t)voxels; vox += 2 * stride) step(vox, std::integral_constant<int, 2>{});
    for (; vox < (size_t)voxels; vox += stride) step(vox, std::integral_constant<int, 1>{});
  } else if constexpr (HK > 0) {
    float wr[HKA][VW];
#pragma unroll
    for (int k = 0; k < HK; ++k)
#pragma unroll
      for (int j = 0; j < VW; ++j) wr[k][j] = hf.w[k * C + c0 + j];
    const float* dl = hf.dl + (size_t)n * HK * voxels;
    const float nslope = act == BRATS_ACT_RELU ? 0.f : slope;
    auto step = [&](size_t v0, auto cnt) {
      constexpr int NV = decltype(cnt)::value;
      typename Raw16<T>::type yr[NV];
      float gq[NV][HKA];
#pragma unroll
      for (int i = 0; i < NV; ++i) yr[i] = Raw16<T>::template load<NT>(yb + (v0 + i * stride) * ypitch);
#pragma unroll
      for (int i = 0; i < NV; ++i)
#pragma unroll
        for (int k = 0; k < HK; ++k) gq[i][k] = dl[(size_t)k * voxels + v0 + i * stride];
#pragma unroll
      for (int i = 0; i < NV; ++i) {
        float yy[VW], o[VW];
        Raw16<T>::unpack(yr[i], yy);
#pragma unroll
        for (int j = 0; j < VW; ++j) {
          float d = 0.f;
#pragma unroll
          for (int k = 0; k < HK; ++k) d += gq[i][k] * wr[k][j];
          const float u = d * (yy[j] * sc[j] + sh[j] > 0.f ? 1.f : nslope);
          o[j] = u * ca[j] + (yy[j] * cb[j] + ck[j]);
        }
        if (amax) {
#pragma unroll
          for (int j = 0; j < VW; j += 2) mx = __builtin_fmaxf(__builtin_fmaxf(mx, __builtin_fabsf(o[j])), __builtin_fabsf(o[j + 1]));
        }
        vstore<T, VW, NT>(dyb + (v0 + i * stride) * dypitch, o);
      }
    };
    for (; vox + 3 * stride < (size_t)voxels; vox += 4 * stride) step(vox, std::integral_constant<int, 4>{});
    for (; vox < (size_t)voxels; vox += stride) step(vox, std::integral_constant<int, 1>{});
  } else {
  for (; vox + stride < (size_t)voxels; vox += 2 * stride) {
    float g0[VW], y0[VW], g1[VW], y1[VW], o0[VW], o1[VW];
    vload<T, VW, NT>(dzb + vox * dzpitch, g0);
    vload<T, VW, NT>(yb + vox * ypitch, y0);
    vload<T, VW, NT>(dzb + (vox + stride) * dzpitch, g1);
    vload<T, VW, NT>(yb + (vox + stride) * ypitch, y1);
    body(g0, y0, o0);
    body(g1, y1, o1);
    vstore<T, VW, NT>(dyb + vox * dypitch, o0);
    vstore<T, VW, NT>(dyb + (vox + stride) * dypitch, o1);
  }
  if (vox < (size_t)voxels) {
    float g0[VW], y0[VW], o0[VW];
    vload<T, VW, NT>(dzb + vox * dzpitch, g0);
    vload<T, VW, NT>(yb + vox * ypitch, y0);
    body(g0, y0, o0);
    vstore<T, VW, NT>(dyb + vox * dypitch, o0);
  }
  }
  if (amax) record_absmax<T>(mx, amax);
}

constexpr int GN_BWD_MAX_BLOCKS = 2048;
extern "C" size_t BRATS_API(brats_gn_bwd_ws_floats)(int N, int C) { return (size_t)(1 + GN_BWD_MAX_BLOCKS) * N * C * 2; }

template <typename F> static inline void with_fold(int fold, F&& f) {
  if (fold > 0) f(std::integral_constant<int, 3>{});
  else if (fold < 0) f(std::integral_constant<int, -1>{});
  else f(std::integral_constant<int, 0>{});
}

static int gn_act_bwd_impl(const void* dz, int dzpitch, const void* y, int ypitch, const float* scale_shift, const float* mean_rstd,
                           const float* gamma, void* dy, int dypitch, float* red, float* dgamma, float* dbeta, int dtype, int act,
                           SlopeArg slope, int N, int voxels, int C, int groups, float* amax, HeadFold hf, int K, hipStream_t st) {
  const int vw = vec_width(dtype);
  if (C % vw || C % groups || dzpitch % vw || ypitch % vw || dypitch % vw || C / vw > 256)
    BRATS_FAIL(BRATS_E_ARG, "gn_act_bwd: C=%d / pitches must be multiples of %d", C, vw);
  const Walk w = voxel_walk(vw, voxels, C);
  const bool big = big_tensor(dtype, (size_t)N * voxels * C);
  dim3 g1(w.grid(big ? GN_BWD_MAX_BLOCKS : 512), N), g2(w.grid(big ? 8192 : 2048), N);
  const size_t lds1 = (size_t)(w.vl * C * 2 + (K > 0 ? w.vl * K : 0)) * sizeof(float);
  const size_t lds2 = (size_t)2 * groups * sizeof(float);
  auto go = [&](auto t, auto heavy, auto nt, auto hk) {
    using T = typename decltype(t)::type;
    constexpr bool HEAVY = decltype(heavy)::value, NT = decltype(nt)::value;
    constexpr int HK = decltype(hk)::value;
    hipLaunchKernelGGL((gn_bwd_reduce_kernel<T, HEAVY, NT, HK>), g1, dim3(256), lds1, st, (const T*)dz, dzpitch, (const T*)y, ypitch,
                       scale_shift, mean_rstd, red, act, slope, voxels, C, groups, hf);
    hipLaunchKernelGGL(gn_bwd_finish_kernel, dim3((N * C * 2 + 7) / 8), dim3(256), 0, st, red, (int)g1.x, N * C * 2);
    hipLaunchKernelGGL((gn_bwd_apply_kernel<T, HEAVY, NT, HK>), g2, dim3(256), lds2, st, (const T*)dz, dzpitch, (const T*)y, ypitch,
                       scale_shift, mean_rstd, gamma, red, (T*)dy, dypitch, dgamma, dbeta, act, slope, N, voxels, C, groups,
                       (uint32_t*)amax, hf);
  };
  with_fold(K, [&](auto hk) {
    if constexpr (decltype(hk)::value != 0)
      with_stream(dtype, big, [&](auto t, auto nt) { go(t, std::false_type{}, nt, hk); });
    else
      with_act_stream(dtype, act > BRATS_ACT_LEAKY, big, [&](auto t, auto heavy, auto nt) { go(t, heavy, nt, hk); });
  });
  BRATS_CHECK_LAUNCH();
  return (int)g1.x;
}

extern "C" int BRATS_API(brats_gn_act_bwd)(const void* dz, int dzpitch, const void* y, int ypitch, const float* scale_shift,
                                const float* mean_rstd, const float* gamma, void* dy, int dypitch, float* red,
                                float* dgamma, float* dbeta, int dtype, int act, float slope_value, const float* slope_dev,
                                int N, int voxels, int C, int groups, float* amax, brats_stream_t s) {
  if (!dz || !y || !dy || !red || !scale_shift || !mean_rstd || !gamma) BRATS_FAIL(BRATS_E_ARG, "gn_act_bwd: null pointer");
  const int rc = gn_act_bwd_impl(dz, dzpitch, y, ypitch, scale_shift, mean_rstd, gamma, dy, dypitch, red, dgamma, dbeta, dtype, act,
                                 SlopeArg{slope_value, slope_dev}, N, voxels, C, groups, amax, HeadFold{}, 0, (hipStream_t)s);
  return rc < 0 ? rc : 0;
}

__global__ void __launch_bounds__(256) gn_bwd_tiles_finish_kernel(const double* __restrict__ part, int splits, int N, int C, int groups,
                                                                  const float* __restrict__ mean_rstd, float* __restrict__ red) {
  const int i = blockIdx.x * blockDim.x + threadIdx.x;
  if (i >= N * C) return;
  const int n = i / C, c = i % C;
  double s1 = 0.0, s2 = 0.0;
  const double* src = part + ((size_t)n * C + c) * 2;
  const size_t zs = (size_t)N * C * 2;
  int z = 0;
  for (; z + 8 <= splits; z += 8) {
    double v1[8], v2[8];
#pragma unroll
    for (int u = 0; u < 8; ++u) { v1[u] = src[(z + u) * zs]; v2[u] = src[(z + u) * zs + 1]; }
#pragma unroll
    for (int u = 0; u < 8; ++u) { s1 += v1[u]; s2 += v2[u]; }
  }
  for (; z < splits; ++z) { s1 += src[z * zs]; s2 += src[z * zs + 1]; }
  const int g = c / (C / groups);
  const double mean = mean_rstd[(n * groups + g) * 2], rstd = mean_rstd[(n * groups + g) * 2 + 1];
  red[(size_t)i * 2] = (float)s1;
  red[(size_t)i * 2 + 1] = (float)(rstd * (s2 - mean * s1));
}

extern "C" int BRATS_API(brats_gn_act_bwd_tiles)(const float* tile_stats, int tiles_per_sample, const void* dz, int dzpitch, const void* y,
                                      int ypitch, const float* scale_shift, const float* mean_rstd, const float* gamma, void* dy,
                                      int dypitch, float* red, float* dgamma, float* dbeta, int dtype, int act, float slope,
                                      int N, int voxels, int C, int groups, float* amax, brats_stream_t s) {
  if (!tile_stats || !dz || !y || !dy || !red || !scale_shift || !mean_rstd || !gamma || tiles_per_sample <= 0)
    BRATS_FAIL(BRATS_E_ARG, "gn_act_bwd_tiles: null pointer");
  if (dtype != BRATS_BF16 && dtype != BRATS_F32) BRATS_FAIL(BRATS_E_UNSUPPORTED, "gn_act_bwd_tiles: 16-bit or f32 (split-precision mode) activations");
  if (act != BRATS_ACT_RELU && act != BRATS_ACT_LEAKY) BRATS_FAIL(BRATS_E_UNSUPPORTED, "gn_act_bwd_tiles: relu / leakyrelu only (act %d)", act);
  const int vw = vec_width(dtype);
  if (C % vw || C % groups || dzpitch % vw || ypitch % vw || dypitch % vw || C / vw > 256)
    BRATS_FAIL(BRATS_E_ARG, "gn_act_bwd_tiles: C=%d / pitches must be multiples of %d", C, vw);
  hipStream_t st = (hipStream_t)s;
  double* part = (double*)(red + (((size_t)N * C * 2 + 1) / 2) * 2);
  const int splits = gn_splits(tiles_per_sample);
  hipLaunchKernelGGL(gn_chan_reduce_kernel, dim3((C + 15) / 16, N, splits), dim3(256), 0, st, tile_stats, tiles_per_sample, C, part);
  hipLaunchKernelGGL(gn_bwd_tiles_finish_kernel, dim3((N * C + 255) / 256), dim3(256), 0, st, part, splits, N, C, groups, mean_rstd, red);
  const bool big = big_tensor(dtype, (size_t)N * voxels * C);
  dim3 g2(voxel_walk(vw, voxels, C).grid(big ? 8192 : 2048), N);
  const size_t lds2 = (size_t)2 * groups * sizeof(float);
  with_stream(dtype, big, [&](auto t, auto nt) {
    using T = typename decltype(t)::type;
    hipLaunchKernelGGL((gn_bwd_apply_kernel<T, false, decltype(nt)::value, 0>), g2, dim3(256), lds2, st, (const T*)dz, dzpitch, (const T*)y,
                       ypitch, scale_shift, mean_rstd, gamma, red, (T*)dy, dypitch, dgamma, dbeta, act, SlopeArg{slope, nullptr}, N, voxels,
                       C, groups, (uint32_t*)amax, HeadFold{});
  });
  BRATS_CHECK_LAUNCH();
  return 0;
}

extern "C" size_t BRATS_API(brats_gn_bwd_head_ws_floats)(int N, int C, int K) { return (size_t)N * GN_BWD_MAX_BLOCKS * (K * C + K); }
extern "C" int BRATS_API(brats_gn_act_bwd_head)(const float* dlogits, const float* hw, int K, const void* y, int ypitch,
                                     const float* scale_shift, const float* mean_rstd, const float* gamma, void* dy, int dypitch,
                                     float* red, float* hws, float* dgamma, float* dbeta, float* dhw, float* dhb, int dtype,
                                     int act, float slope_value, int N, int voxels, int C, int groups, float* amax,
                                     brats_stream_t s) {
  if (!dlogits || !hw || !y || !dy || !red || !hws || !scale_shift || !mean_rstd || !gamma || !dhw || !dhb)
    BRATS_FAIL(BRATS_E_ARG, "gn_act_bwd_head: null pointer");
  if (K != 3 || act > BRATS_ACT_LEAKY)
    BRATS_FAIL(BRATS_E_UNSUPPORTED, "gn_act_bwd_head: built for K = 3 logit planes and relu / leakyrelu (K=%d, act=%d)", K, act);
  HeadFold hf;
  hf.dl = dlogits; hf.w = hw; hf.hpart = hws;
  const int nb = gn_act_bwd_impl(nullptr, 8, y, ypitch, scale_shift, mean_rstd, gamma, dy, dypitch, red, dgamma, dbeta, dtype, act,
                                 SlopeArg{slope_value, nullptr}, N, voxels, C, groups, amax, hf, K, (hipStream_t)s);
  if (nb < 0) return nb;
  return brats_ordered_sum2(hws, dhw, K * C, dhb, N * nb, K * C + K, (hipStream_t)s);
}

extern "C" int BRATS_API(brats_gn_act_bwd_pool)(const void* dskip, int dskip_pitch, const void* dpool, int dpool_pitch,
                                     const unsigned char* argmax, const void* y, int ypitch, const float* scale_shift,
                                     const float* mean_rstd, const float* gamma, void* dy, int dypitch, float* red, float* dgamma,
                                     float* dbeta, int dtype, int act, float slope_value, int N, int D, int H, int W, int C,
                                     int groups, float* amax, brats_stream_t s) {
  const int vw = vec_width(dtype);
  if (!dskip || !dpool || !argmax || !y || !dy || !red || !scale_shift || !mean_rstd || !gamma)
    BRATS_FAIL(BRATS_E_ARG, "gn_act_bwd_pool: null pointer");
  if (act > BRATS_ACT_LEAKY || ((D | H | W) & 1) || dskip_pitch % vw || dpool_pitch % vw)
    BRATS_FAIL(BRATS_E_UNSUPPORTED, "gn_act_bwd_pool: relu / leakyrelu, even spatial dims, pitches multiples of %d (act=%d)", vw, act);
  HeadFold hf;
  hf.dskip = dskip; hf.dpool = dpool; hf.argmax = argmax; hf.dskip_pitch = dskip_pitch; hf.dpool_pitch = dpool_pitch;
  hf.D = D; hf.H = H; hf.W = W;
  const int rc = gn_act_bwd_impl(nullptr, vw, y, ypitch, scale_shift, mean_rstd, gamma, dy, dypitch, red, dgamma, dbeta, dtype, act,
                                 SlopeArg{slope_value, nullptr}, N, D * H * W, C, groups, amax, hf, -1, (hipStream_t)s);
  return rc < 0 ? rc : 0;
}

template <typename T>
__global__ void __launch_bounds__(256) prelu_slope_grad_kernel(const T* __restrict__ dz, int dzpitch, const T* __restrict__ y, int ypitch,
                                                               const float* __restrict__ scale_shift, float* __restrict__ part,
                                                               int voxels, int C) {
  constexpr int VW = 16 / sizeof(T);
  const int n = blockIdx.y;
  const int cv = C / VW, vl_n = blockDim.x / cv;
  const int mycv = threadIdx.x % cv, myvl = threadIdx.x / cv, c0 = mycv * VW;
  float acc = 0.f;
  if (myvl < vl_n) {
    float sc[VW], sh[VW];
#pragma unroll
    for (int j = 0; j < VW; ++j) { sc[j] = scale_shift[((size_t)n * C + c0 + j) * 2]; sh[j] = scale_shift[((size_t)n * C + c0 + j) * 2 + 1]; }
    const T* dzb = dz + (size_t)n * voxels * dzpitch + c0;
    const T* yb = y + (size_t)n * voxels * ypitch + c0;
    for (size_t vox = (size_t)blockIdx.x * vl_n + myvl; vox < (size_t)voxels; vox += (size_t)gridDim.x * vl_n) {
      float g[VW], yy[VW];
      Vec<T, VW>::load(dzb + vox * dzpitch, g);
      Vec<T, VW>::load(yb + vox * ypitch, yy);
#pragma unroll
      for (int j = 0; j < VW; ++j) acc += g[j] * fminf(yy[j] * sc[j] + sh[j], 0.f);
    }
  }
  __shared__ float r[256];
  r[threadIdx.x] = acc;
  __syncthreads();
  for (int m = 128; m > 0; m >>= 1) {
    if ((int)threadIdx.x < m) r[threadIdx.x] += r[threadIdx.x + m];
    __syncthreads();
  }
  if (threadIdx.x == 0) part[(size_t)n * gridDim.x + blockIdx.x] = r[0];
}

constexpr int PRELU_MAX_BLOCKS = 1024;
extern "C" size_t BRATS_API(brats_prelu_ws_floats)(int N) { return (size_t)N * PRELU_MAX_BLOCKS; }
extern "C" int BRATS_API(brats_prelu_slope_grad)(const void* dz, int dzpitch, const void* y, int ypitch, const float* scale_shift, float* ws,
                                      float* dslope, int dtype, int N, int voxels, int C, brats_stream_t s) {
  const int vw = vec_width(dtype);
  if (!dz || !y || !scale_shift || !ws || !dslope || C % vw || dzpitch % vw || ypitch % vw || C / vw > 256)
    BRATS_FAIL(BRATS_E_ARG, "prelu_slope_grad: bad argument");
  hipStream_t st = (hipStream_t)s;
  const unsigned gx = voxel_walk(vw, voxels, C).grid(PRELU_MAX_BLOCKS);
  with_storage(dtype, [&](auto t) {
    using T = typename decltype(t)::type;
    hipLaunchKernelGGL(prelu_slope_grad_kernel<T>, dim3(gx, N), dim3(256), 0, st, (const T*)dz, dzpitch, (const T*)y, ypitch, scale_shift,
                       ws, voxels, C);
  });
  BRATS_CHECK_LAUNCH();
  return brats_ordered_sum(ws, dslope, N * (int)gx, 1, st);
}

extern "C" int BRATS_API(brats_evonorm_finalize)(const float* stats, int tiles_per_sample, int N, int C, int groups,
                                      double count_per_channel, float eps, float* mean_rstd, double* chan_ws,
                                      brats_stream_t s) {
  if (!stats || !mean_rstd || !chan_ws || C % groups || C / groups > 256) BRATS_FAIL(BRATS_E_ARG, "evonorm_finalize: bad argument");
  return gn_finalize_launch(stats, tiles_per_sample, N, C, groups, count_per_channel, eps, 1, nullptr, nullptr, mean_rstd, nullptr, chan_ws,
                            (hipStream_t)s);
}

DEVI float sigmoidf_(float x) { return __builtin_amdgcn_rcpf(1.f + __expf(-x)); }

template <typename T, bool NT = false>
__global__ void __launch_bounds__(256) evonorm_fwd_kernel(const T* __restrict__ x, int xpitch, const float* __restrict__ mean_rstd,
                                   const float* __restrict__ gamma, const float* __restrict__ beta, T* __restrict__ z,
                                   int zpitch, float* __restrict__ chansum, int voxels, int C, int groups,
                                   uint32_t* __restrict__ amax, const float* __restrict__ gscale) {
  constexpr int VW = 16 / sizeof(T);
  extern __shared__ float sm[];
  float* sc = sm;
  float* be = sm + C;
  const int n = blockIdx.y, cpg = C / groups;
  for (int c = threadIdx.x; c < C; c += blockDim.x) {
    const float gs = gscale ? gscale[(size_t)n * C + c] : 1.f;
    sc[c] = mean_rstd[(n * groups + c / cpg) * 2 + 1] * gamma[c] * gs;
    be[c] = beta[c] * gs;
  }
  __syncthreads();
  const int cv = C / VW, vl_n = blockDim.x / cv;
  const int mycv = threadIdx.x % cv, myvl = threadIdx.x / cv, c0 = mycv * VW;
  float acc[VW];
  float mx = 0.f;
#pragma unroll
  for (int j = 0; j < VW; ++j) acc[j] = 0.f;
  if (myvl < vl_n) {
    const T* xb = x + (size_t)n * voxels * xpitch;
    T* zb = z + (size_t)n * voxels * zpitch;
// ... 876 lines not shown
```

### brats21_amd/networks/_program.py

```python
import os

import torch
import torch.nn as nn

from .. import ops
from .._lib import BratsHipError


class _PackedWeightsModule(nn.Module):

    PRECISIONS = ("auto", "bf16", "fp16", "fp32", "x3", "fp16x3", "bf16x3", "x3fwd", "x3bwd")
    _cpu_hint = ""

    @property
    def precision(self):
        return self._precision

    @precision.setter
    def precision(self, value):
        if value not in self.PRECISIONS:
            raise ValueError(f"model.precision / BRATS_PRECISION must be one of {self.PRECISIONS}, got {value!r}")
        self._precision = value

    def train(self, mode=True):
        if mode != self.training:
            ops.invalidate_packed_weights()
        return super().train(mode)

    def _init_switches(self, pack_plan):
        self.precision = os.environ.get("BRATS_PRECISION", "auto")
        self.conv_fp8 = None
        self.skip_deep_heads_in_eval = False
        self._grad_sink = None
        self._grad_dest = None
        self.pack_plan = os.environ.get("BRATS_PACK_PLAN", pack_plan) != "0"
        self.fold_head_bwd = os.environ.get("BRATS_FOLD_HEAD", "1") != "0"
        self.fold_pool_bwd = os.environ.get("BRATS_FOLD_POOL", "1") != "0"
        self.fold_bwd_stats = os.environ.get("BRATS_FOLD_BWD_STATS", "1") != "0"
        self.fold_head_fwd = os.environ.get("BRATS_FOLD_HEAD_FWD", os.environ.get("BRATS_FOLD_HEAD", "1")) != "0"

    def _init_dropout(self, p):
        if not 0.0 <= float(p) < 1.0:
            raise ValueError(f"dropout probability has to be in [0, 1), got {p}")
        self.dropout_p = float(p)
        seed = 0
        if self.dropout_p > 0.0:
            seed = int(torch.randint(0, 2 ** 62, (1,), generator=torch.Generator().manual_seed(torch.initial_seed())))
        self._dropout_seed_base, self._dropout_rank_mixed = seed, self.dropout_p == 0.0
        self.register_buffer("_dropout_state", torch.tensor([seed, 0], dtype=torch.int64), persistent=False)

    def _advance_dropout(self, device):
        if self._dropout_state.device != device:
            raise BratsHipError("brats21_amd: module and input are on different devices")
        if not self._dropout_rank_mixed:
            rank = os.environ.get("RANK")
            if rank is None:
                import torch.distributed as dist
                rank = dist.get_rank() if dist.is_available() and dist.is_initialized() else 0
            self._dropout_state[0] = (self._dropout_seed_base + 0x9E3779B97F4A7C15 * int(rank)) % (2 ** 63)
            self._dropout_rank_mixed = True
        self._dropout_state[1] += 1
        return self._dropout_state.clone()

    def _weights_may_have_changed(self):
        if torch.is_grad_enabled():
            ops.invalidate_packed_weights()

    def _dtype(self):
        if self.precision == "bf16":
            return torch.bfloat16
        if self.precision == "fp16":
            return torch.float16
        if self.precision in ("fp32", "x3", "fp16x3", "bf16x3", "x3fwd", "x3bwd"):
            return torch.float32
        if torch.is_autocast_enabled():
            return torch.float16 if torch.get_autocast_dtype("cuda") == torch.float16 else torch.bfloat16
        return torch.float32

    def _x3_modes(self):
        if self.precision in ("x3", "fp16x3"):
            return ops.X3F, ops.X3F
        if self.precision == "bf16x3":
            return ops.X3B, ops.X3B
        if self.precision in ("x3fwd", "x3bwd"):
            return (ops.X3F, None) if self.precision == "x3fwd" else (None, ops.X3F)
        return None, None

    MAX_INPLANES = MAX_CLASSES = 16

    def _check_shape_limits(self, inplanes, num_classes, features, width_multiple):
        if int(inplanes) != inplanes or int(num_classes) != num_classes or inplanes < 1 or num_classes < 1:
            raise ValueError(f"{self.name}: inplanes and num_classes must be positive integers (got {inplanes!r}, {num_classes!r})")
        if inplanes > self.MAX_INPLANES:
            raise NotImplementedError(f"{self.name}: the input layer is built for inplanes <= {self.MAX_INPLANES} (got {inplanes})")
        if num_classes > self.MAX_CLASSES:
            raise NotImplementedError(f"{self.name}: the head kernels are built for num_classes <= {self.MAX_CLASSES} (got {num_classes})")
        if any(c % width_multiple for c in features):
            raise NotImplementedError(f"{self.name}: the convolution kernels need widths that are multiples of {width_multiple} "
                                      f"(got {list(features)})")
        self.inplanes = int(inplanes)

    def _run(self, fn, x):
        if not x.is_cuda:
            raise BratsHipError(f"brats21_amd.{self.name} runs on the GPU only (no CPU fallback){self._cpu_hint}")
        if x.dim() != 5 or x.shape[1] != self.inplanes or any(s % 8 for s in x.shape[2:]):
            raise ValueError(f"expected input [N, {self.inplanes}, D, H, W] with D, H, W divisible by 8")
        refinement = getattr(self, "refinement", False)
        if refinement and any(s % 16 for s in x.shape[2:]):
            raise ValueError(f"refinement=True: expected input [N, {self.inplanes}, D, H, W] with D, H, W divisible by 16")
        if refinement and self.conv_fp8:
            raise NotImplementedError("refinement=True with the e4m3 convolution path (conv_fp8) is not implemented")
        self._fwd_grad = torch.is_grad_enabled()
        self._weights_may_have_changed()
        if self.training and self.pack_plan and torch.is_grad_enabled():
            ops.plan_for(self, x.device)
        outs = fn.apply(self, x.float(), self._dtype(), *self.parameters())
        if refinement:
            return ([outs[0], outs[1]], list(outs[2:])) if self.deep_supervision else [outs[0], outs[1]]
        if self.deep_supervision:
            return outs[0], list(outs[1:])
        return outs[0]


class _AmaxSlots:

    def __init__(self, n, device):
        self.buf = torch.zeros(n, dtype=torch.float32, device=device)
        self.i = 0

    def take(self):
        s = self.buf[self.i:self.i + 1]
        self.i += 1
        return s


def _inherit_amax(dst, src):
    a = getattr(src, "_amax", None)
    if a is not None:
        dst._amax = a
    return dst


def douts_device(douts):
    return next(d.device for d in douts if d is not None)


class _Ctx:

    def __init__(self, model, dtype, will_bwd=False):
        self.m, self.dtype = model, dtype
        self.fp8 = getattr(model, "conv_fp8", None) if ops.is16(dtype) else None
        self.x3s = ops.x3_mode() == ops.X3F and dtype == torch.float32
        self.slots = None
        self._names = None
        self.grads = {}
        self.recs = {}
        self.drop = None
        self.act, self.training = getattr(model, "act", None), model.training
        self.will_bwd = will_bwd
        self.lazy_ok = (not will_bwd and not torch.is_grad_enabled() and getattr(model, "norm_on_load", False)
                        and ops.is16(dtype))

    @property
    def names(self):
        if self._names is None:
            self._names = {p: i for i, p in enumerate(self.m.parameters())}
        return self._names

    def start_dropout(self, device):
        m = self.m
        if m.training and m.dropout_p > 0.0:
            if self.fp8:
                raise NotImplementedError("--dropout > 0 with the e4m3 convolution path is not implemented")
            self.drop = (m.dropout_p, m._advance_dropout(device))

    def drop_of(self, unit):
        return self.m._unit_ids[unit] if self.drop is not None else None

    def dropped(self, t, uid, out=None):
        if self.drop is None or uid is None:
            return t
        return ops.dropout(t, self.drop[0], self.drop[1], uid, out=out)

    def slot(self, device, force=False):
        if not self.fp8 and not force:
            return None
        if self.slots is None or self.slots.i >= self.slots.buf.numel():
            self.slots = _AmaxSlots(64, device)
        return self.slots.take()

    def identity_ss(self, n, c, device):
        key = (n, c)
# ... 64 lines not shown
```

### brats21_amd/networks/equiunet.py

```python
import contextlib
import functools
import math
import os

import torch
import torch.nn as nn

from .. import ops
from .._lib import PACK_DGRAD, PACK_FWD, BratsHipError
from ._program import _PackedWeightsModule, _fn_backward, _fn_forward, _heads_bwd, _inherit_amax, input_cpad


class _ConvParams(nn.Module):

    def __init__(self, cin, cout, k, bias):
        super().__init__()
        self.weight = nn.Parameter(torch.empty(cout, cin, k, k, k))
        self.bias = nn.Parameter(torch.empty(cout)) if bias else None
        nn.init.kaiming_uniform_(self.weight, a=math.sqrt(5))
        if bias:
            bound = 1.0 / math.sqrt(cin * k * k * k)
            nn.init.uniform_(self.bias, -bound, bound)


# ... 107 lines not shown
            ops.conv_f8_chunk(x.shape[-1], x2.shape[-1] if x2 is not None else 0) > 0)


def _unit_act(unit, act):
    if act == "prelu":
        return "leakyrelu", unit.prelu.weight.detach()
    return act, None


def _one_sample(t):
    n, d, h, w, c = t.shape
    if not t.is_contiguous():
        raise BratsHipError("--norm batch needs dense activations")
    return t.view(1, n * d, h, w, c)


def _blk(b):
    return b.ConvBnRelu1, b.ConvBnRelu2


def _bn_fwd_tail(cx, unit, x, x2, y, stats, pool):
    n, d, h, wd, c = y.shape
    bn = unit.bn
    if cx.training:
        mean_rstd, scale_shift = ops.gn_finalize(stats.view(1, -1, c, 2), 1, c, c, n * d * h * wd, bn.weight.detach(), bn.bias.detach())
        with torch.no_grad():
            cnt = float(n * d * h * wd)
            mean = mean_rstd[0, :, 0]
            var = (1.0 / mean_rstd[0, :, 1].double() ** 2 - 1e-5).clamp_min(0).float()
            bn.running_mean.mul_(0.9).add_(mean, alpha=0.1)
            bn.running_var.mul_(0.9).add_(var, alpha=0.1 * cnt / max(cnt - 1.0, 1.0))
            bn.num_batches_tracked += 1
    else:
        mean_rstd = None
        scale = bn.weight.detach() * torch.rsqrt(bn.running_var + 1e-5)
        scale_shift = torch.stack([scale, bn.bias.detach() - bn.running_mean * scale], -1).reshape(1, c, 2).contiguous().float()
    kact, slope_t = _unit_act(unit, cx.act)
    z = ops.affine_act(_one_sample(y), scale_shift, kact, slope_t=slope_t).view(n, d, h, wd, c)
    cx.dropped(z, cx.drop_of(unit), out=z)
    cx.recs[unit] = (unit, x, x2, y, mean_rstd, scale_shift)
    if pool:
        return z, ops.maxpool2(z, want_argmax=pool == "argmax")
    return z


def _cgr_fwd(cx, unit, x, x2=None, *, no_act=False, pool=False, lazy=False):
    dtype, fp8 = cx.dtype, cx.fp8
    uid = cx.drop_of(unit)
    lazy = lazy and cx.lazy_ok and uid is None
    if pool:
        pool = "argmax" if cx.will_bwd else True
    w = unit.conv.weight
    cbias, gamma_c, beta_c = None, unit.bn.weight.detach(), unit.bn.bias.detach()
    if unit.bcn:
        if torch.is_grad_enabled():
            a_c, cbias, gamma_c, beta_c = unit.bn.tables()
            w = w.detach() * a_c.view(-1, 1, 1, 1, 1)
        else:
            srcs = (unit.conv.weight, unit.bn.weight, unit.bn.bias, unit.bn.bn.weight, unit.bn.bn.bias, unit.bn.bn.running_var,
                    unit.bn.bn.running_mean)
            key = (ops.pack_generation(),) + tuple((t._version, t.data_ptr()) for t in srcs)
            hit = getattr(unit, "_bcn_fold", None)
            if hit is None or hit[0] != key:
                a_c, cbias, gamma_c, beta_c = unit.bn.tables()
                hit = unit._bcn_fold = (key, (w.detach() * a_c.view(-1, 1, 1, 1, 1), cbias, gamma_c, beta_c))
            w, cbias, gamma_c, beta_c = hit[1]
        fp8, lazy = None, False
    cout = w.shape[0]
    cin_pad = x.shape[-1] + (x2.shape[-1] if x2 is not None else 0)
    c1 = x.shape[-1] if x2 is not None else None
    if isinstance(x, ops.Pending) or isinstance(x2, ops.Pending):
        if fp8 or not ops.conv_pre_ok(dtype, 3, unit.dilation, x.shape[-1], x2.shape[-1] if x2 is not None else 0, cout):
            x = x.materialize() if isinstance(x, ops.Pending) else x
            x2 = x2.materialize() if isinstance(x2, ops.Pending) else x2
    if _f8_ok(fp8, dtype, x, x2):
        wpk = ops.pack_weights_f8(w, PACK_FWD, cin_pad=cin_pad, c1=c1)
        y, stats = ops.conv3d_f8(x, wpk, cout, unit.dilation, want_stats=True, x2=x2, amax=getattr(x, "_amax", None),
                                 amax2=getattr(x2, "_amax", None) if x2 is not None else None)
    else:
        with ops.use_plan(None) if unit.bcn else contextlib.nullcontext():
            wpk = ops.pack_weights(w, dtype, PACK_FWD, cin_pad=cin_pad, dil=unit.dilation, c1=c1)
        y, stats = ops.conv3d(x, wpk, cout, 3, unit.dilation, want_stats=True, x2=x2, amax=getattr(x, "_x3amax", None), bias=cbias)
    n, d, h, wd, _ = y.shape
    if unit.batch_norm:
        return _bn_fwd_tail(cx, unit, x, x2, y, stats, pool)
    mean_rstd, scale_shift = ops.gn_finalize(stats, n, cout, unit.groups, d * h * wd, gamma_c, beta_c)
    rec = (unit, x, x2, y, mean_rstd, scale_shift)
    if no_act:
        cx.recs[unit] = rec
        return y
    amax = cx.slot(y.device)
    kact, slope_t = _unit_act(unit, cx.act)
    if lazy and slope_t is None and kact in ("relu", "leakyrelu") and amax is None and not pool:
        return ops.Pending(y, scale_shift, kact)
    cx.recs[unit] = rec
    if pool and uid is None and kact in ("relu", "leakyrelu") and y.numel() * y.element_size() >= (256 << 20):
        z, pooled = ops.affine_act_pool(y, scale_shift, kact, amax=amax, slope_t=slope_t, want_argmax=pool == "argmax")
        if amax is not None:
            z._amax = pooled._amax = amax
        return z, pooled
    z = ops.affine_act(y, scale_shift, kact, amax=amax, slope_t=slope_t)
    if amax is not None:
        z._amax = amax
    cx.dropped(z, uid, out=z)
    if pool:
        return z, _inherit_amax(ops.maxpool2(z, want_argmax=pool == "argmax"), z)
    return z


def _cgr_bwd(cx, unit, dz, *, need_dx=True, head=None, pool=None, bst=None):
    _, x, x2, y, mean_rstd, scale_shift = cx.recs[unit]
    dtype, fp8 = cx.dtype, cx.fp8
    if bst is not None:
        bst = cx.recs[bst] if (cx.m.fold_bwd_stats and cx.drop is None) else None
    cin = unit.conv.weight.shape[1]
    gamma_c = unit.bn.weight.detach()
    w_bwd = unit.conv.weight
    if unit.bcn:
        a_c, _, gamma_c, _ = unit.bn.tables()
        w_bwd = unit.conv.weight.detach() * a_c.view(-1, 1, 1, 1, 1)
        fp8 = None
    tiles = None
    if isinstance(dz, tuple):
        dz, tiles = dz
    dz = cx.dropped(dz, cx.drop_of(unit))
    all8 = fp8 == "all" and ops.is16(dtype)
    f8 = all8 and need_dx and ops.conv_f8_chunk(y.shape[-1]) > 0
    ax, ax2 = getattr(x, "_amax", None), (getattr(x2, "_amax", None) if x2 is not None else None)
    w8 = (all8 and unit.dilation == 1 and ax is not None and (x2 is None or ax2 is not None) and ops.is16(y.dtype)
          and ops.conv3d_wgrad_f8_ok(x, y, x2))
    x3s = cx.x3s
    amax = cx.slot(y.device, True) if (f8 or w8 or x3s) else None
    kact, slope_t = _unit_act(unit, cx.act)
    if slope_t is not None:
        cx.put(unit.prelu.weight, ops.prelu_slope_grad(dz, y, scale_shift))
    if unit.batch_norm:
        if mean_rstd is None:
            raise NotImplementedError("--norm batch: backward through an eval-mode forward (running statistics) is not implemented")
        n_, d_, h_, w_, c_ = y.shape
        dy, dgamma, dbeta = ops.gn_act_bwd(_one_sample(dz), _one_sample(y), scale_shift, mean_rstd, gamma_c, c_, kact,
                                           amax=amax, slope_t=slope_t)
        dy = dy.view(n_, d_, h_, w_, c_)
        if amax is not None:
            dy._amax = amax
    elif head is not None:
        hd, dout = head
        dy, dgamma, dbeta, dhw, dhb = ops.gn_act_bwd_head(dout, hd.weight, y, scale_shift, mean_rstd, gamma_c,
                                                          unit.groups, kact, amax=amax)
        cx.put(hd.weight, dhw)
        cx.put(hd.bias, dhb)
    elif pool is not None:
        dy, dgamma, dbeta = ops.gn_act_bwd_pool(pool[0], pool[1], pool[2], y, scale_shift, mean_rstd, gamma_c,
                                                unit.groups, kact, amax=amax)
    elif tiles is not None:
        dy, dgamma, dbeta = ops.gn_act_bwd_tiles(tiles, dz, y, scale_shift, mean_rstd, gamma_c, unit.groups, kact,
                                                 amax=amax)
    else:
        dy, dgamma, dbeta = ops.gn_act_bwd(dz, y, scale_shift, mean_rstd, gamma_c, unit.groups, kact, amax=amax,
                                           slope_t=slope_t)
    wdst = cx.dest(unit.conv.weight)
    if w8 and amax is not None:
        dw = ops.conv3d_wgrad_f8(x, dy, ax, amax, x2=x2, amax2=ax2, out=wdst)
    elif x2 is not None and x.shape[-1] % 16:
        dw, db = ops.conv3d_wgrad(torch.cat([x, x2], -1), dy, 3, unit.dilation, amax_dy=amax if x3s else None, want_dbias=unit.bcn)
    else:
        dw, db = ops.conv3d_wgrad(x, dy, 3, unit.dilation, x2=x2, out=None if unit.bcn else wdst, amax_dy=amax if x3s else None,
                                  want_dbias=unit.bcn)
    dw = dw[:, :cin].contiguous() if dw.shape[1] != cin else dw
    if unit.bcn:
        pg = _bcn_param_grads(unit, dw, db, dgamma, dbeta)
    else:
        pg = {unit.conv.weight: dw, unit.bn.weight: dgamma, unit.bn.bias: dbeta}
    for prm, g in pg.items():
        cx.put(prm, g)
    if not need_dx:
        return None
    if f8:
        wpk = ops.pack_weights_f8(unit.conv.weight, PACK_DGRAD)

        def dgrad(**kw):
            return ops.conv3d_f8(dy, wpk, cin, unit.dilation, amax=amax, **kw)
    else:
        with ops.use_plan(None) if unit.bcn else contextlib.nullcontext():
            wpk = ops.pack_weights(w_bwd, dtype, PACK_DGRAD, dil=unit.dilation)

        def dgrad(**kw):
            return ops.conv3d(dy, wpk, cin, 3, unit.dilation, amax=amax if x3s else None, **kw)
    if x2 is None:
        if bst is not None and not f8:
            u1, _, _, y1, mr1, ss1 = bst
            kact1, slope1 = _unit_act(u1, cx.act)
            if (not u1.batch_norm and not u1.bcn and not unit.bcn and mr1 is not None and y1.shape[-1] == cin and y1.dtype == dy.dtype
                    and ops.conv_bstats_ok(dtype, unit.dilation, dy.shape[-1], cin, kact1, slope1)):
                return ops.conv3d_bstats(dy, wpk, cin, unit.dilation, y1, ss1, kact1, amax=amax if x3s else None)
        dx, _ = dgrad()
        return dx
    c1 = x.shape[-1]
    if c1 % ops.split_granule(cin) == 0:
        dx, _ = dgrad(split=c1)
        return dx
    dx, _ = dgrad()
    return dx[..., :c1], dx[..., c1:]


def _level_bwd(cx, unit, down, d_pooled, d_skip, need_dx=True, bst=None):
    idx = getattr(down, "_pool_argmax", None)
    kact, slope_t = _unit_act(unit, cx.act)
    if (idx is not None and cx.m.fold_pool_bwd and cx.drop is None and not unit.batch_norm and slope_t is None
            and kact in ("relu", "leakyrelu")):
        return _cgr_bwd(cx, unit, None, need_dx=need_dx, pool=(d_skip, d_pooled, idx), bst=bst)
    return _cgr_bwd(cx, unit, ops.maxpool2_bwd(down, d_pooled, dx_skip=d_skip), need_dx=need_dx, bst=bst)


def _ref_cpad(k):
    return 8 if k <= 8 else 16


def _ref_amax(cx, t):
    return ops.absmax(t) if cx.x3s else None


def _ref_fwd(ctx, cx, out):
    r, dtype = cx.m.refunet, cx.dtype
    cgr = functools.partial(_cgr_fwd, cx)
    k, f0 = out.shape[1], r.conv0.weight.shape[0]
    x0 = ops.ncdhw_to_ndhwc(out, dtype, cpad=input_cpad(k, dtype))
    x0._net_input = True
    amax0 = ops.absmax(x0) if ops.x3_mode() == ops.X3F else None
    wpk = ops.pack_weights(r.conv0.weight, dtype, PACK_FWD, cin_pad=x0.shape[-1])
    hx, _ = ops.conv3d(x0, wpk, f0, 3, 1, bias=r.conv0.bias.detach(), amax=amax0)
    hx1, p = cgr(r.hx1, hx, pool=True)
    hx2, p = cgr(r.hx2, p, pool=True)
    hx3, p = cgr(r.hx3, p, pool=True)
    hx4, p = cgr(r.hx4, p, pool=True)
    d = cgr(r.hx5, p)
    for unit, skip in ((r.d4, hx4), (r.d3, hx3), (r.d2, hx2), (r.d1, hx1)):
        d = cgr(unit, ops.upsample(d, 2), x2=skip)
    ctx.ref = (x0, hx1, hx2, hx3, hx4, d)
    return ops.conv3d_narrow(d, ops.pack_weights_narrow(r.conv_d0.weight, PACK_FWD), k, bias=r.conv_d0.bias.detach(), add=out)


def _ref_bwd(ctx, cx, d_ref, d_out):
    r, dtype = cx.m.refunet, cx.dtype
    cbw = functools.partial(_cgr_bwd, cx)
    x0, hx1, hx2, hx3, hx4, d1 = ctx.ref
    ctx.ref = None
    if d_ref is None:
        d_ref = torch.zeros(ctx.out_shape, dtype=torch.float32, device=d1.device)
    d_ref = d_ref.contiguous().float()
    k, f0 = d_ref.shape[1], d1.shape[-1]
    dy = ops.ncdhw_to_ndhwc(d_ref, dtype, cpad=_ref_cpad(k))
    amax = _ref_amax(cx, dy)
    dw, _ = ops.conv3d_wgrad(d1, dy, 3, 1, amax_dy=amax)
    cx.put(r.conv_d0.weight, dw[:k].contiguous())
    cx.put(r.conv_d0.bias, ops.channel_dot(dy).sum(0)[:k].contiguous())
    wpad = torch.zeros((dy.shape[-1],) + tuple(r.conv_d0.weight.shape[1:]), dtype=torch.float32, device=d1.device)
    wpad[:k] = r.conv_d0.weight.detach()
    with ops.use_plan(None):
        wpk = ops.pack_weights(wpad, dtype, PACK_DGRAD)
    g, _ = ops.conv3d(dy, wpk, f0, 3, 1, amax=amax)
    skips = []
    for unit in (r.d1, r.d2, r.d3, r.d4):
        g_up, g_skip = cbw(unit, g)
        skips.append(g_skip)
        g = ops.upsample_bwd(g_up, 2)
    g = cbw(r.hx5, g)
    for unit, down in ((r.hx4, hx4), (r.hx3, hx3), (r.hx2, hx2), (r.hx1, hx1)):
        g = _level_bwd(cx, unit, down, g, skips.pop())
    dw0, _ = ops.conv3d_wgrad(x0, g, 3, 1, amax_dy=_ref_amax(cx, g))
    cx.put(r.conv0.weight, dw0[:, :k].contiguous())
    cx.put(r.conv0.bias, ops.channel_dot(g).sum(0))
    rest = d_ref if d_out is None else d_ref + d_out.float()
    return ops.conv3d_narrow(g, ops.pack_weights_narrow(r.conv0.weight, PACK_DGRAD), k, add=rest)


class _EquiUnetFn(torch.autograd.Function):
    @staticmethod
    def forward(ctx, model, x, dtype, *params):
        return _fn_forward(_EquiUnetFn._forward, ctx, model, x, dtype, params)

    @staticmethod
    def backward(ctx, *douts):
        return _fn_backward(_EquiUnetFn._backward, ctx, douts)

    @staticmethod
    def _forward(ctx, cx, x0):
        m = cx.m
        cgr = functools.partial(_cgr_fwd, cx)

        def up(t):
            return _inherit_amax(ops.upsample(t, 2), t)

        down1, p1 = cgr(m.encoder1.ConvBnRelu2, cgr(m.encoder1.ConvBnRelu1, x0, lazy=True), pool=True)
        down2, p2 = cgr(m.encoder2.ConvBnRelu2, cgr(m.encoder2.ConvBnRelu1, p1, lazy=True), pool=True)
        down3, p3 = cgr(m.encoder3.ConvBnRelu2, cgr(m.encoder3.ConvBnRelu1, p2, lazy=True), pool=True)
        down4 = cgr(m.encoder4.ConvBnRelu2, cgr(m.encoder4.ConvBnRelu1, p3, lazy=True))
        deep_heads = m.deep_supervision and not (m.skip_deep_heads_in_eval and not m.training)
        bottom = cgr(m.bottom.ConvBnRelu2, cgr(m.bottom.ConvBnRelu1, down4, lazy=True), lazy=not deep_heads)
        bottom_2 = cgr(m.bottom_2, down4, x2=bottom)
        up3 = cgr(m.decoder3.ConvBnRelu2, cgr(m.decoder3.ConvBnRelu1, down3, x2=up(bottom_2), lazy=True))
        up2 = cgr(m.decoder2.ConvBnRelu2, cgr(m.decoder2.ConvBnRelu1, down2, x2=up(up3), lazy=True))
        u1 = cgr(m.decoder1.ConvBnRelu1, down1, x2=up(up2), lazy=True)
        last = m.decoder1.ConvBnRelu2
        kact, slope_t = _unit_act(last, cx.act)
        nk = m.outconv.weight.shape[0]
        fuse_top = (m.fold_head_fwd and cx.drop is None and not last.batch_norm and slope_t is None and kact in ("relu", "leakyrelu")
# ... 117 lines not shown
```

### brats21_amd/ops.py

```python
import contextlib
import weakref

import numpy as np
import torch

from . import _lib
from ._lib import ACT_LEAKY, ACT_NONE, ACT_RELU, BF16, F16, F32, PACK_DGRAD, PACK_FWD, X3_BF16, X3_F16

ACTS = {"none": ACT_NONE, "relu": ACT_RELU, "leakyrelu": ACT_LEAKY, "elu": _lib.ACT_ELU, "swish": _lib.ACT_SWISH,
        "mish": _lib.ACT_MISH}


class KernelTimer:

    def __init__(self):
        self.records = {}

    def span(self, key):
        return _Span(self, key)

    def summary(self):
        torch.cuda.synchronize()
        out = {}
        for key, evs in self.records.items():
# ... 557 lines not shown
    nbytes = _lib.lib().brats_conv3d_wgrad_ws_bytes(code, ksize, n, d, h, w, c, c2, cout)
    ws = torch.empty(max(nbytes, 4) // 4, dtype=torch.float32, device=x.device)
    dw = _grad_out(out, (cout, c + c2, ksize, ksize, ksize), x.device)
    db = torch.empty(cout, dtype=torch.float32, device=x.device) if want_dbias else None
    if amax_dy is not None and kd in (X3F, X3B):
        with _span("conv_wgrad", c + c2, cout, ksize, dil, n, d, h, w, str(kd)):
            _lib.check(_lib.lib().brats_conv3d_x3_wgrad(ptr, c, p, ptr2, c2, p2, dptr, dp, _f32(amax_dy), ws.data_ptr(), dw.data_ptr(),
                                                        db.data_ptr() if db is not None else None, code, dil, n, d, h, w, cout,
                                                        _stream()), "conv3d_x3_wgrad")
        return dw, db
    with _span("conv_wgrad", c + c2, cout, ksize, dil, n, d, h, w, str(kd)):
        _lib.check(_lib.lib().brats_conv3d_wgrad(ptr, c, p, ptr2, c2, p2, dptr, dp, ws.data_ptr(), dw.data_ptr(),
                                                 db.data_ptr() if db is not None else None, code, ksize, dil, n, d, h, w,
                                                 cout, _stream()), "conv3d_wgrad")
    return dw, db


def conv3d_wgrad_f8_ok(x, dy, x2=None):
    n, d, h, w, c = x.shape
    return (is16(x.dtype) and dy.dtype == x.dtype and
            _lib.lib().brats_conv3d_wgrad_f8_ws_bytes(n, d, h, w, c, x2.shape[-1] if x2 is not None else 0, dy.shape[-1]) > 0)


def conv3d_wgrad_f8(x, dy, amax, amax_dy, x2=None, amax2=None, out=None):
    ptr, c, p = _desc(x)
    ptr2, c2, p2 = _desc2(x2)
    dptr, cout, dp = _desc(dy)
    n, d, h, w, _ = x.shape
    if not is16(x.dtype) or dy.dtype != x.dtype:
        raise _lib.BratsHipError("conv3d_wgrad_f8: bf16 activations only")
    nbytes = _lib.lib().brats_conv3d_wgrad_f8_ws_bytes(n, d, h, w, c, c2, cout)
    if nbytes == 0:
        raise _lib.BratsHipError(f"conv3d_wgrad_f8: not built for {c}+{c2} -> {cout} channels at {n}x{d}x{h}x{w} (use conv3d_wgrad)")
    ws = torch.empty(nbytes // 4, dtype=torch.float32, device=x.device)
    dw = _grad_out(out, (cout, c + c2, 3, 3, 3), x.device)
    with _span("conv_wgrad_f8", c + c2, cout, 3, 1, n, d, h, w, "e4m3"):
        _lib.check(_fn16("brats_conv3d_wgrad_f8", x.dtype)(ptr, c, p, _f32(amax), ptr2, c2, p2, _f32(amax2), dptr, dp, _f32(amax_dy),
                                                    ws.data_ptr(), dw.data_ptr(), n, d, h, w, cout, _stream()), "conv3d_wgrad_f8")
    return dw


def gn_finalize(stats, n, c, groups, voxels, gamma, beta, eps=1e-5):
    mean_rstd = torch.empty((n, groups, 2), dtype=torch.float32, device=stats.device)
    scale_shift = torch.empty((n, c, 2), dtype=torch.float32, device=stats.device)
    chan = torch.empty(_lib.lib().brats_gn_ws_doubles(n, c), dtype=torch.float64, device=stats.device)
    _lib.check(_lib.lib().brats_gn_finalize(stats.data_ptr(), stats.shape[1], n, c, groups, float(voxels), eps,
                                            _f32(gamma), _f32(beta), mean_rstd.data_ptr(), scale_shift.data_ptr(),
                                            chan.data_ptr(), _stream()), "gn_finalize")
    return mean_rstd, scale_shift


def affine_act(y, scale_shift, act="relu", out=None, slope=0.01, amax=None, slope_t=None):
    ptr, c, p = _desc(y)
    n, d, h, w, _ = y.shape
    if out is None:
        out = new_act(n, d, h, w, c, y.dtype, y.device)
    optr, oc, op = _desc(out)
    _lib.check(_lib.lib().brats_affine_act_fwd(ptr, p, scale_shift.data_ptr(), optr, op, _code(y.dtype), ACTS[act], slope,
                                               _f32(slope_t), n, d * h * w, c, _f32(amax), _stream()), "affine_act_fwd")
    return out


def dropout(x, p, state, unit, out=None):
    ptr, c, pitch = _desc(x)
    n, d, h, w, _ = x.shape
    if state.dtype != torch.int64 or state.numel() != 2 or not state.is_cuda:
        raise _lib.BratsHipError("dropout: state must be an int64[2] device tensor (seed, step counter)")
    if out is None:
        out = new_act(n, d, h, w, c, x.dtype, x.device)
    optr, oc, op = _desc(out)
    if oc != c or out.dtype != x.dtype:
        raise _lib.BratsHipError("dropout: bad output tensor")
    _lib.check(_lib.lib().brats_dropout(ptr, pitch, optr, op, _code(x.dtype), n * d * h * w, c, float(p), state.data_ptr(), int(unit),
                                        _stream()), "dropout")
    return out


def affine_act_pool(y, scale_shift, act="relu", slope=0.01, amax=None, slope_t=None, with_avg=False, want_argmax=False):
    ptr, c, p = _desc(y)
    n, d, h, w, _ = y.shape
    z = new_act(n, d, h, w, c, y.dtype, y.device)
    pooled = new_act(n, d // 2, h // 2, w // 2, c * (2 if with_avg else 1), y.dtype, y.device)
    idx = torch.empty((n, d // 2, h // 2, w // 2, c), dtype=torch.uint8, device=y.device) if want_argmax else None
    zp, _, zpitch = _desc(z)
    pp, _, ppitch = _desc(pooled)
    _lib.check(_lib.lib().brats_affine_act_pool_fwd(ptr, p, scale_shift.data_ptr(), zp, zpitch, pp, ppitch,
                                                    idx.data_ptr() if idx is not None else None, _code(y.dtype), ACTS[act],
                                                    slope, _f32(slope_t), n, d, h, w, c, int(with_avg), _f32(amax), _stream()),
               "affine_act_pool_fwd")
    if idx is not None:
        z._pool_argmax = idx
    return z, pooled


def _gn_bwd_bufs(y):
    n, c = y.shape[0], y.shape[-1]
    red = torch.empty(_lib.lib().brats_gn_bwd_ws_floats(n, c), dtype=torch.float32, device=y.device)
    dgamma = torch.empty(c, dtype=torch.float32, device=y.device)
    dbeta = torch.empty(c, dtype=torch.float32, device=y.device)
    return torch.empty(y.shape, dtype=y.dtype, device=y.device), red, dgamma, dbeta


def gn_act_bwd(dz, y, scale_shift, mean_rstd, gamma, groups=8, act="relu", slope=0.01, amax=None, slope_t=None):
    dzp, c, dzpitch = _desc(dz)
    yp, _, ypitch = _desc(y)
    n, d, h, w, _ = y.shape
    dy, red, dgamma, dbeta = _gn_bwd_bufs(y)
    _lib.check(_lib.lib().brats_gn_act_bwd(dzp, dzpitch, yp, ypitch, scale_shift.data_ptr(), mean_rstd.data_ptr(),
                                           _f32(gamma), dy.data_ptr(), c, red.data_ptr(), dgamma.data_ptr(),
                                           dbeta.data_ptr(), _code(y.dtype), ACTS[act], slope, _f32(slope_t), n, d * h * w, c,
                                           groups, _f32(amax), _stream()), "gn_act_bwd")
    return dy, dgamma, dbeta


def conv_bstats_ok(dtype, dil, c1, cout, act="relu", slope_t=None):
    dtype = _conv_dtype(dtype, 3)
    if not (is16(dtype) or dtype in (X3F, X3B)) or slope_t is not None or act not in ("relu", "leakyrelu"):
        return False
    return bool(_lib.lib().brats_conv3d_bstats_ok(_code(dtype), 3, dil, c1, cout))


def conv3d_bstats(x, packed_w, cout, dil, fwd_y, scale_shift, act="relu", slope=0.01, amax=None):
    ptr, c, p = _desc(x)
    n, d, h, w, _ = x.shape
    fp, fc, fpitch = _desc(fwd_y)
    if fc != cout or fwd_y.dtype != x.dtype or tuple(fwd_y.shape[:4]) != (n, d, h, w):
        raise _lib.BratsHipError("conv3d_bstats: the forward tensor must have the output's shape and dtype")
    out = new_act(n, d, h, w, cout, x.dtype, x.device)
    stats = torch.empty((n, tiles_per_sample(d, h, w), cout, 2), dtype=torch.float32, device=x.device)
    kd = _conv_dtype(x.dtype, 3)
    if kd in (X3F, X3B):
        with _span("conv_igemm_bst", c, cout, 3, dil, n, d, h, w, str(kd)):
            _lib.check(_lib.lib().brats_conv3d_x3_fwd_bstats(ptr, c, p, _f32(amax), packed_w.data_ptr(), out.data_ptr(), cout, fp, fpitch,
                                                             scale_shift.data_ptr(), ACTS[act], float(slope), stats.data_ptr(),
                                                             _code(kd), dil, n, d, h, w, cout, _stream()), "conv3d_x3_fwd_bstats")
        return out, stats
    with _span("conv_igemm_bst", c, cout, 3, dil, n, d, h, w, str(x.dtype)):
        _lib.check(_lib.lib().brats_conv3d_fwd_bstats(ptr, c, p, packed_w.data_ptr(), out.data_ptr(), cout, fp, fpitch,
                                                      scale_shift.data_ptr(), ACTS[act], float(slope), stats.data_ptr(),
                                                      _code(x.dtype), dil, n, d, h, w, cout, _stream()), "conv3d_fwd_bstats")
    return out, stats


def gn_act_bwd_tiles(tile_stats, dz, y, scale_shift, mean_rstd, gamma, groups=8, act="relu", slope=0.01, amax=None):
    dzp, c, dzpitch = _desc(dz)
    yp, _, ypitch = _desc(y)
    n, d, h, w, _ = y.shape
    dy, red, dgamma, dbeta = _gn_bwd_bufs(y)
    _lib.check(_lib.lib().brats_gn_act_bwd_tiles(tile_stats.data_ptr(), tile_stats.shape[1], dzp, dzpitch, yp, ypitch,
                                                 scale_shift.data_ptr(), mean_rstd.data_ptr(), _f32(gamma), dy.data_ptr(), c,
                                                 red.data_ptr(), dgamma.data_ptr(), dbeta.data_ptr(), _code(y.dtype), ACTS[act],
                                                 float(slope), n, d * h * w, c, groups, _f32(amax), _stream()), "gn_act_bwd_tiles")
    return dy, dgamma, dbeta


def gn_act_bwd_head(dlogits, head_weight, y, scale_shift, mean_rstd, gamma, groups=8, act="relu", slope=0.01, amax=None):
    yp, c, ypitch = _desc(y)
    n, d, h, w, _ = y.shape
    k = head_weight.shape[0]
    dev = y.device
    hw = head_weight.detach().reshape(k, c).contiguous().float()
    dl = dlogits.contiguous().float()
    dy, red, dgamma, dbeta = _gn_bwd_bufs(y)
    hws = torch.empty(_lib.lib().brats_gn_bwd_head_ws_floats(n, c, k), dtype=torch.float32, device=dev)
    dhw = torch.empty((k, c), dtype=torch.float32, device=dev)
    dhb = torch.empty(k, dtype=torch.float32, device=dev)
    _lib.check(_lib.lib().brats_gn_act_bwd_head(dl.data_ptr(), hw.data_ptr(), k, yp, ypitch, scale_shift.data_ptr(),
                                                mean_rstd.data_ptr(), _f32(gamma), dy.data_ptr(), c, red.data_ptr(), hws.data_ptr(),
                                                dgamma.data_ptr(), dbeta.data_ptr(), dhw.data_ptr(), dhb.data_ptr(), _code(y.dtype),
                                                ACTS[act], slope, n, d * h * w, c, groups, _f32(amax), _stream()), "gn_act_bwd_head")
    return dy, dgamma, dbeta, dhw.reshape(k, c, 1, 1, 1), dhb


def gn_act_bwd_pool(dskip, dpool, argmax, y, scale_shift, mean_rstd, gamma, groups=8, act="relu", slope=0.01, amax=None):
    yp, c, ypitch = _desc(y)
    n, d, h, w, _ = y.shape
    sp, _, spitch = _desc(dskip)
    pp, _, ppitch = _desc(dpool)
    dy, red, dgamma, dbeta = _gn_bwd_bufs(y)
    _lib.check(_lib.lib().brats_gn_act_bwd_pool(sp, spitch, pp, ppitch, argmax.data_ptr(), yp, ypitch, scale_shift.data_ptr(),
                                                mean_rstd.data_ptr(), _f32(gamma), dy.data_ptr(), c, red.data_ptr(),
                                                dgamma.data_ptr(), dbeta.data_ptr(), _code(y.dtype), ACTS[act], slope, n, d, h, w, c,
                                                groups, _f32(amax), _stream()), "gn_act_bwd_pool")
    return dy, dgamma, dbeta


def head_fold_ok(head_weight, act, slope_t):
    return head_weight.shape[0] == 3 and act in ("relu", "leakyrelu") and slope_t is None


def prelu_slope_grad(dz, y, scale_shift):
    dzp, c, dzpitch = _desc(dz)
    yp, _, ypitch = _desc(y)
    n, d, h, w, _ = y.shape
    ws = torch.empty(_lib.lib().brats_prelu_ws_floats(n), dtype=torch.float32, device=y.device)
    out = torch.empty(1, dtype=torch.float32, device=y.device)
    _lib.check(_lib.lib().brats_prelu_slope_grad(dzp, dzpitch, yp, ypitch, scale_shift.data_ptr(), ws.data_ptr(), out.data_ptr(),
                                                 _code(y.dtype), n, d * h * w, c, _stream()), "prelu_slope_grad")
    return out


def maxpool2(x, with_avg=False, out=None, want_argmax=False):
    ptr, c, p = _desc(x)
    n, d, h, w, _ = x.shape
    co = 2 * c if with_avg else c
    if out is None:
        out = new_act(n, d // 2, h // 2, w // 2, co, x.dtype, x.device)
    optr, oc, op = _desc(out)
    idx = torch.empty((n, d // 2, h // 2, w // 2, c), dtype=torch.uint8, device=x.device) if want_argmax else None
    _lib.check(_lib.lib().brats_maxpool2_fwd(ptr, p, optr, op, idx.data_ptr() if idx is not None else None, _code(x.dtype), n, c, d,
                                             h, w, int(with_avg), _stream()), "maxpool2_fwd")
    if idx is not None:
        x._pool_argmax = idx
    return out


def maxpool2_bwd(x, dy, dx_skip=None, with_avg=False):
    ptr, c, p = _desc(x)
    dptr, _, dp = _desc(dy)
    n, d, h, w, _ = x.shape
    dx = new_act(n, d, h, w, c, x.dtype, x.device)
    sptr, sp = (None, 0)
    if dx_skip is not None:
        sptr, _, sp = _desc(dx_skip)
    idx = getattr(x, "_pool_argmax", None)
    if idx is not None:
        _lib.check(_lib.lib().brats_maxpool2_bwd_idx(idx.data_ptr(), dptr, dp, sptr, sp, dx.data_ptr(), c, _code(x.dtype), n, c,
                                                     d, h, w, int(with_avg), _stream()), "maxpool2_bwd_idx")
        return dx
    _lib.check(_lib.lib().brats_maxpool2_bwd(ptr, p, None, 0, dptr, dp, sptr, sp, dx.data_ptr(), c, _code(x.dtype), n, c,
                                             d, h, w, int(with_avg), _stream()), "maxpool2_bwd")
    return dx


def upsample(x, scale=2, out=None):
    ptr, c, p = _desc(x)
    n, d, h, w, _ = x.shape
    if out is None:
        out = new_act(n, d * scale, h * scale, w * scale, c, x.dtype, x.device)
    optr, oc, op = _desc(out)
    _lib.check(_lib.lib().brats_upsample_fwd(ptr, p, optr, op, _code(x.dtype), n, c, d, h, w, scale, _stream()),
               "upsample_fwd")
    return out


def set_upsample_bwd_fused(mode):
    return _lib.lib().brats_upsample_bwd_set_fused(mode)


def upsample_bwd(dy, scale=2):
    dptr, c, dp = _desc(dy)
    n, do, ho, wo, _ = dy.shape
    d, h, w = do // scale, ho // scale, wo // scale
    code = _code(dy.dtype)
    ws = torch.empty(_lib.lib().brats_upsample_bwd_ws_bytes(code, n, c, d, h, w, scale), dtype=torch.uint8, device=dy.device)
    dx = new_act(n, d, h, w, c, dy.dtype, dy.device)
    _lib.check(_lib.lib().brats_upsample_bwd(dptr, dp, dx.data_ptr(), c, ws.data_ptr(), code, n, c, d, h, w, scale,
                                             _stream()), "upsample_bwd")
    return dx


def head(x, weight, bias, scale=1):
    ptr, c, p = _desc(x)
    n, d, h, w, _ = x.shape
    k = weight.shape[0]
    wf = weight.detach().reshape(k, c).contiguous().float()
    out = torch.empty((n, k, d * scale, h * scale, w * scale), dtype=torch.float32, device=x.device)
    low = torch.empty((n, k, d, h, w), dtype=torch.float32, device=x.device) if scale > 1 else None
    _lib.check(_lib.lib().brats_head_fwd(ptr, p, wf.data_ptr(), _f32(bias.detach()) if bias is not None else None,
                                         low.data_ptr() if low is not None else None, out.data_ptr(), _code(x.dtype), n, c,
                                         k, d, h, w, scale, _stream()), "head_fwd")
    return out


def gn_head(y, scale_shift, weight, bias, act="relu", slope=0.01):
    ptr, c, p = _desc(y)
    n, d, h, w, _ = y.shape
    k = weight.shape[0]
    wf = weight.detach().reshape(k, c).contiguous().float()
    out = torch.empty((n, k, d, h, w), dtype=torch.float32, device=y.device)
    _lib.check(_lib.lib().brats_gn_head_fwd(ptr, p, scale_shift.data_ptr(), ACTS[act], slope, wf.data_ptr(),
                                            _f32(bias.detach()) if bias is not None else None, out.data_ptr(), _code(y.dtype), n, c,
                                            k, d * h * w, _stream()), "gn_head_fwd")
    return out


def head_bwd(x, weight, dout, scale=1, want_dx=True):
    ptr, c, p = _desc(x)
    n, d, h, w, _ = x.shape
    k = weight.shape[0]
    wf = weight.detach().reshape(k, c).contiguous().float()
    dout = dout.contiguous().float()
    nbytes = _lib.lib().brats_head_bwd_ws_bytes(n, c, k, d, h, w, scale)
    ws = torch.empty(max(nbytes, 4) // 4, dtype=torch.float32, device=x.device)
    dx = new_act(n, d, h, w, c, x.dtype, x.device) if want_dx else None
    dw = torch.empty((k, c), dtype=torch.float32, device=x.device)
    db = torch.empty(k, dtype=torch.float32, device=x.device)
    _lib.check(_lib.lib().brats_head_bwd(ptr, p, wf.data_ptr(), dout.data_ptr(), ws.data_ptr(),
                                         dx.data_ptr() if dx is not None else None, c, dw.data_ptr(), db.data_ptr(),
                                         _code(x.dtype), n, c, k, d, h, w, scale, _stream()), "head_bwd")
    return dx, dw.reshape(k, c, 1, 1, 1), db


def evonorm_finalize(stats, n, c, groups, voxels, eps=1e-5):
    mean_rstd = torch.empty((n, groups, 2), dtype=torch.float32, device=stats.device)
    chan = torch.empty(_lib.lib().brats_gn_ws_doubles(n, c), dtype=torch.float64, device=stats.device)
# ... 441 lines not shown
```

### include/brats_hip.h

```cpp
#ifndef BRATS_HIP_H
#define BRATS_HIP_H
#include <stddef.h>
#include <stdint.h>

#ifdef __cplusplus
extern "C" {
#endif

typedef void* brats_stream_t;

enum { BRATS_F32 = 0, BRATS_BF16 = 1, BRATS_F16 = 2, BRATS_X3_BF16 = 3, BRATS_X3_F16 = 4 };
enum { BRATS_E_ARG = -1, BRATS_E_UNSUPPORTED = -2, BRATS_E_HIP = -3 };
enum { BRATS_ACT_NONE = 0, BRATS_ACT_RELU = 1, BRATS_ACT_LEAKY = 2, BRATS_ACT_ELU = 3, BRATS_ACT_SWISH = 4, BRATS_ACT_MISH = 5 };

#define BRATS_ABI_VERSION 7
int brats_abi_version(void);
const char* brats_last_error(void);

int brats_dropout(const void* x, int xpitch, void* out, int opitch, int dtype, size_t voxels, int C, float p,
                  const void* state, int unit, brats_stream_t s);

int brats_ncdhw_to_ndhwc(const float* src, void* dst, int dtype, int N, int C, int cpad, int dst_pitch,
                         int D, int H, int W, brats_stream_t s);
int brats_ndhwc_to_ncdhw(const void* src, int src_pitch, float* dst, int dtype, int N, int C,
                         int D, int H, int W, brats_stream_t s);

enum { BRATS_PACK_FWD = 0, BRATS_PACK_DGRAD = 1 };
size_t brats_conv3d_packed_bytes(int dtype, int ksize, int cin, int cout, int ck);
int brats_conv3d_chunk(int dtype, int ksize, int dil, int c1, int c2, int cout);
int brats_conv3d_pack_weights(const float* w, void* packed, int dtype, int mode, int ksize,
                              int cout_w, int cin_w, int cin_off, int cin_cnt, int ck, brats_stream_t s);
typedef struct {
  const float* w;
  void* out;
  int dtype, mode, taps, cin_w, cin_real, cin_off, rows, rows16, kdim, ck, ms_n, reserved;
  unsigned long long total;
} brats_pack_job;
int brats_conv3d_pack_blocks(int kdim, int ck, int rows);
int brats_conv3d_pack_weights_multi(const brats_pack_job* jobs, const int* blocks , int nblocks,
                                    brats_stream_t s);
int brats_conv3d_pack_weights_multi_f16(const brats_pack_job* jobs, const int* blocks , int nblocks,
                                    brats_stream_t s);
int brats_conv3d_tiles_per_sample(int D, int H, int W);
int brats_conv3d_split_granule(int cout);
int brats_conv3d_set_vs8(int mode);
int brats_conv3d_set_kp(int mode);
int brats_conv3d_fwd(const void* x1, int c1, int pitch1, const void* x2, int c2, int pitch2,
                     const void* packed_w, const float* bias, void* y, int ypitch,
                     void* y2, int y2pitch, int ysplit, float* stats,
                     int dtype, int ksize, int dil, int N, int D, int H, int W, int cout,
                     brats_stream_t s);
int brats_conv3d_pre_ok(int dtype, int ksize, int dil, int c1, int c2, int cout);
int brats_conv3d_fwd_pre(const void* x1, int c1, int pitch1, const float* ss1, const void* x2, int c2, int pitch2,
                         const float* ss2, int act, float slope, const void* packed_w, const float* bias, void* y, int ypitch,
                         float* stats, int dtype, int dil, int N, int D, int H, int W, int cout, brats_stream_t s);
int brats_conv3d_bstats_ok(int dtype, int ksize, int dil, int c1, int cout);
int brats_conv3d_fwd_bstats(const void* x1, int c1, int pitch1, const void* packed_w, void* y, int ypitch,
                            const void* fwd_y, int fwd_pitch, const float* scale_shift, int act, float slope,
                            float* tile_stats, int dtype, int dil, int N, int D, int H, int W, int cout, brats_stream_t s);
int brats_conv3d_x3_fwd(const void* x1, int c1, int pitch1, const void* x2, int c2, int pitch2, const float* xamax,
                        const void* packed_w, const float* bias, void* y, int ypitch, void* y2, int y2pitch, int ysplit,
                        float* stats, int dtype, int dil, int N, int D, int H, int W, int cout, brats_stream_t s);
int brats_conv3d_x3_fwd_bstats(const void* x1, int c1, int pitch1, const float* xamax, const void* packed_w, void* y, int ypitch,
                               const void* fwd_y, int fwd_pitch, const float* scale_shift, int act, float slope,
                               float* tile_stats, int dtype, int dil, int N, int D, int H, int W, int cout, brats_stream_t s);
int brats_conv3d_f8_chunk(int c1, int c2);
size_t brats_conv3d_f8_packed_bytes(int cin, int cout, int ck);
int brats_conv3d_f8_pack_weights(const float* w, void* packed, int mode, int cout_w, int cin_w, int cin_off,
                                 int cin_cnt, int ck, brats_stream_t s);
int brats_conv3d_f8_fwd(const void* x1, int c1, int pitch1, const float* amax1, const void* x2, int c2, int pitch2,
                        const float* amax2, float xscale, const void* packed_w, const float* bias, void* y, int ypitch,
                        void* y2, int y2pitch, int ysplit, float* stats, int dil, int N, int D, int H, int W, int cout,
                        brats_stream_t s);
int brats_conv3d_f8_fwd_f16(const void* x1, int c1, int pitch1, const float* amax1, const void* x2, int c2, int pitch2,
                        const float* amax2, float xscale, const void* packed_w, const float* bias, void* y, int ypitch,
                        void* y2, int y2pitch, int ysplit, float* stats, int dil, int N, int D, int H, int W, int cout,
                        brats_stream_t s);
int brats_absmax(const void* x, int pitch, int dtype, size_t rows, int C, float* out, brats_stream_t s);
size_t brats_conv3d_wgrad_ws_bytes(int dtype, int ksize, int N, int D, int H, int W, int c1, int c2, int cout);
int brats_conv3d_set_wgrad_alltaps(int mode);
int brats_conv3d_set_x3_wgrad_fused(int mode);
int brats_conv3d_wgrad(const void* x1, int c1, int pitch1, const void* x2, int c2, int pitch2,
                       const void* dy, int dypitch, float* ws, float* dw, float* dbias,
                       int dtype, int ksize, int dil, int N, int D, int H, int W, int cout,
                       brats_stream_t s);
int brats_conv3d_x3_wgrad(const void* x1, int c1, int pitch1, const void* x2, int c2, int pitch2, const void* dy, int dypitch,
                          const float* amax_dy, float* ws, float* dw, float* dbias, int dtype, int dil, int N, int D, int H,
                          int W, int cout, brats_stream_t s);
size_t brats_conv3d_wgrad_f8_ws_bytes(int N, int D, int H, int W, int c1, int c2, int cout);
int brats_conv3d_wgrad_f8(const void* x1, int c1, int pitch1, const float* amax1, const void* x2, int c2, int pitch2,
                          const float* amax2, const void* dy, int dypitch, const float* amax_dy, float* ws, float* dw,
                          int N, int D, int H, int W, int cout, brats_stream_t s);
int brats_conv3d_wgrad_f8_f16(const void* x1, int c1, int pitch1, const float* amax1, const void* x2, int c2, int pitch2,
                          const float* amax2, const void* dy, int dypitch, const float* amax_dy, float* ws, float* dw,
                          int N, int D, int H, int W, int cout, brats_stream_t s);
size_t brats_conv3d_wgrad_shift_ws_bytes(int dtype, int ksize, int N, int D, int H, int W, int cin, int cout);
int brats_conv3d_wgrad_shift(const void* x, int cin, int xpitch, const void* dy, int dypitch, float* ws, float* dw,
                             float* dbias, int dtype, int ksize, int dil, int N, int D, int H, int W, int cout,
                             brats_stream_t s);
int brats_conv3d_x3_wgrad_shift(const void* x, int cin, int xpitch, const void* dy, int dypitch, const float* amax_dy,
                                float* ws, float* dw, float* dbias, int dtype, int ksize, int dil, int N, int D, int H, int W,
                                int cout, brats_stream_t s);

size_t brats_gn_ws_doubles(int N, int C);
int brats_gn_finalize(const float* stats, int tiles_per_sample, int N, int C, int groups,
                      double count_per_channel, float eps, const float* gamma, const float* beta,
                      float* mean_rstd , float* scale_shift ,
                      double* chan_ws , brats_stream_t s);
int brats_affine_act_fwd(const void* y, int ypitch, const float* scale_shift, void* z, int zpitch,
                         int dtype, int act, float slope, const float* slope_dev, int N, int voxels, int C, float* amax,
                         brats_stream_t s);
int brats_affine_act_pool_fwd(const void* y, int ypitch, const float* scale_shift, void* z, int zpitch, void* pooled,
                              int ppitch, unsigned char* argmax ,
                              int dtype, int act, float slope, const float* slope_dev, int N, int D, int H, int W, int C,
                              int with_avg, float* amax, brats_stream_t s);
size_t brats_gn_bwd_ws_floats(int N, int C);
int brats_gn_act_bwd(const void* dz, int dzpitch, const void* y, int ypitch, const float* scale_shift,
                     const float* mean_rstd, const float* gamma, void* dy, int dypitch,
                     float* red , float* dgamma, float* dbeta,
                     int dtype, int act, float slope, const float* slope_dev, int N, int voxels, int C, int groups,
                     float* amax , brats_stream_t s);
int brats_gn_act_bwd_tiles(const float* tile_stats, int tiles_per_sample, const void* dz, int dzpitch, const void* y,
                           int ypitch, const float* scale_shift, const float* mean_rstd, const float* gamma, void* dy,
                           int dypitch, float* red , float* dgamma, float* dbeta, int dtype, int act,
                           float slope, int N, int voxels, int C, int groups,
                           float* amax , brats_stream_t s);
size_t brats_gn_bwd_head_ws_floats(int N, int C, int K);
int brats_gn_act_bwd_head(const float* dlogits, const float* hw, int K, const void* y, int ypitch, const float* scale_shift,
                          const float* mean_rstd, const float* gamma, void* dy, int dypitch, float* red ,
                          float* hws, float* dgamma, float* dbeta, float* dhw, float* dhb, int dtype, int act, float slope,
                          int N, int voxels, int C, int groups, float* amax, brats_stream_t s);
int brats_gn_act_bwd_pool(const void* dskip, int dskip_pitch, const void* dpool, int dpool_pitch, const unsigned char* argmax,
                          const void* y, int ypitch, const float* scale_shift, const float* mean_rstd, const float* gamma,
                          void* dy, int dypitch, float* red, float* dgamma, float* dbeta, int dtype, int act, float slope,
                          int N, int D, int H, int W, int C, int groups, float* amax, brats_stream_t s);
size_t brats_prelu_ws_floats(int N);
int brats_prelu_slope_grad(const void* dz, int dzpitch, const void* y, int ypitch, const float* scale_shift, float* ws,
                           float* dslope, int dtype, int N, int voxels, int C, brats_stream_t s);

size_t brats_chan_ws_floats(int N, int C, int vals);
int brats_evonorm_finalize(const float* stats, int tiles_per_sample, int N, int C, int groups,
                           double count_per_channel, float eps, float* mean_rstd, double* chan_ws,
                           brats_stream_t s);
int brats_evonorm_fwd(const void* x, int xpitch, const float* mean_rstd, const float* gamma,
                      const float* beta, void* z, int zpitch, float* chansum, int dtype, int N,
                      int voxels, int C, int groups,
                      float* amax , brats_stream_t s);
int brats_evonorm_bwd(const void* dz, int dzpitch, const void* x, int xpitch, const float* mean_rstd,
                      const float* gamma, void* dx, int dxpitch, float* red ,
                      float* dgamma, float* dbeta, const double* chan_sums, float* dconvbias,
                      int dtype, int N, int voxels, int C, int groups,
                      float* amax ,
                      const float* gscale, const float* gadd ,
                      brats_stream_t s);
size_t brats_evonorm_bwd_tiles_ws_floats(int N, int C);
int brats_evonorm_bwd_tiles(const float* tile_stats, int tiles_per_sample, const void* dz, int dzpitch, const void* x,
                            int xpitch, const float* mean_rstd, const float* gamma, const float* beta, void* dx, int dxpitch,
                            float* red, float* dgamma, float* dbeta, const double* chan_sums, float* dconvbias, int dtype,
                            int N, int voxels, int C, int groups, float* amax, brats_stream_t s);
int brats_se_fwd(const float* chansum, float inv_vox, const float* w1, const float* b1, const float* w2, const float* b2,
                 float* gate1p , float* hidden , int N, int C, int Ch, brats_stream_t s);
int brats_se_bwd(const float* dgate, const float* chansum, float inv_vox, const float* hidden, const float* gate1p,
                 const float* w1, const float* w2, float* gadd , float* dw1, float* db1, float* dw2, float* db2,
                 int N, int C, int Ch, brats_stream_t s);
int brats_evonorm_se_bwd(const void* dout, int dopitch, const void* x, int xpitch, const float* mean_rstd, const float* gamma,
                         const float* beta, void* dx, int dxpitch, float* ws, float* dgamma, float* dbeta,
                         const double* chan_sums, float* dconvbias, const float* se_chansum, const float* hidden,
                         const float* gate1p, const float* w1, const float* w2, float* gadd, float* dw1, float* db1,
                         float* dw2, float* db2, int Ch,
                         const float* dlogits ,
                         const float* hw , int K, float* hws ,
                         float* dhw , float* dhb ,
                         int dtype, int N, int voxels, int C, int groups, float* amax, brats_stream_t s);
int brats_evonorm_se_bwd_pool(const void* dskip, int dskip_pitch, const void* dpool, int dpool_pitch, const unsigned char* argmax,
                              int with_avg, int D, int H, int W, const void* x, int xpitch, const float* mean_rstd,
                              const float* gamma, const float* beta, void* dx, int dxpitch, float* ws, float* dgamma,
                              float* dbeta, const double* chan_sums, float* dconvbias, const float* se_chansum,
                              const float* hidden, const float* gate1p, const float* w1, const float* w2, float* gadd,
                              float* dw1, float* db1, float* dw2, float* db2, int Ch, int dtype, int N, int C, int groups,
                              float* amax, brats_stream_t s);
int brats_evonorm_se_fwd(const void* x, int xpitch, const float* mean_rstd, const float* gamma, const float* beta,
                         const float* w1, const float* b1, const float* w2, const float* b2, void* out, int opitch,
                         float* ws, float* chansum_out, float* gate1p, float* hidden, int Ch, int dtype, int N, int voxels,
                         int C, int groups, float* amax ,
                         brats_stream_t s);
int brats_channel_dot(const void* a, int apitch, const void* b , int bpitch, float* out ,
                      int dtype, int N, int voxels, int C, brats_stream_t s);
int brats_channel_scale(const void* a, int apitch, const float* scale , const float* add ,
                        void* dst, int dpitch, int dtype, int N, int voxels, int C,
                        float* amax , brats_stream_t s);
typedef struct { const void* x; const void* w; int xpitch, cin, ksize, dil; } brats_dconv_term;
typedef struct { brats_dconv_term term[4]; int nterms, rows; const float* bias; void* y; int ypitch, reserved; } brats_dconv_job;
size_t brats_dconv_packed_bytes(int dtype, int ksize, int kdim, int rows);
int brats_dconv_pack_weights(const float* w, void* packed, int dtype, int mode, int ksize, int cout_w, int cin_w,
                             int cin_off, int cin_cnt, brats_stream_t s);
int brats_dconv_run(const brats_dconv_job* jobs, int njobs, int dtype, int N, int D, int H, int W, brats_stream_t s);

int brats_maxpool2_fwd(const void* x, int xpitch, void* y, int ypitch,
                       unsigned char* argmax ,
                       int dtype, int N, int C, int D, int H, int W, int with_avg, brats_stream_t s);
int brats_maxpool2_bwd(const void* x, int xpitch, const void* y, int ypitch, const void* dy, int dypitch,
                       const void* dx_skip, int dxskip_pitch, void* dx, int dxpitch, int dtype,
                       int N, int C, int D, int H, int W, int with_avg, brats_stream_t s);
int brats_maxpool2_bwd_idx(const unsigned char* argmax, const void* dy, int dypitch, const void* dx_skip ,
                           int dxskip_pitch, void* dx, int dxpitch, int dtype, int N, int C, int D, int H, int W,
                           int with_avg, brats_stream_t s);

int brats_upsample_fwd(const void* x, int xpitch, void* y, int ypitch, int dtype, int N, int C,
                       int D, int H, int W, int scale, brats_stream_t s);
size_t brats_upsample_bwd_ws_bytes(int dtype, int N, int C, int D, int H, int W, int scale);
int brats_upsample_bwd(const void* dy, int dypitch, void* dx, int dxpitch, void* tmp, int dtype,
                       int N, int C, int D, int H, int W, int scale, brats_stream_t s);
int brats_upsample_bwd_set_fused(int mode);

size_t brats_conv3d_narrow_packed_bytes(int C, int K);
int brats_conv3d_narrow_pack(const float* w, float* packed, int mode, int cout_w, int cin_w, brats_stream_t s);
int brats_conv3d_narrow_fwd(const void* x, int C, int xpitch, const float* packed_w, const float* bias, const float* add, float* out,
                            int dtype, int K, int N, int D, int H, int W, brats_stream_t s);

int brats_head_fwd(const void* x, int xpitch, const float* w , const float* b, float* lowres ,
                   float* out , int dtype, int N, int C, int K,
                   int D, int H, int W, int scale, brats_stream_t s);
int brats_gn_head_fwd(const void* y, int ypitch, const float* scale_shift, int act, float slope, const float* w ,
                      const float* b, float* out, int dtype, int N, int C, int K, int voxels, brats_stream_t s);
int brats_evonorm_head_fwd(const void* y, int ypitch, const float* scale_shift, const float* w , const float* b,
                           float* out, int dtype, int N, int C, int K, int voxels, brats_stream_t s);
size_t brats_head_bwd_ws_bytes(int N, int C, int K, int D, int H, int W, int scale);
int brats_head_bwd(const void* x, int xpitch, const float* w, const float* dout, float* ws,
                   void* dx, int dxpitch, float* dw, float* db, int dtype, int N, int C, int K,
                   int D, int H, int W, int scale, brats_stream_t s);

int brats_sw_gather(const float* src, float* dst, const int* windows, int B, int C, int D, int H, int W,
                    int rd, int rh, int rw, int pad_z, int pad_y, int pad_x, float cval, int pad_mode, brats_stream_t s);
int brats_sw_accumulate(const float* prob, const float* importance, float* out, float* count, int K,
                        int Dp, int Hp, int Wp, int rd, int rh, int rw, int n, int z0, int y0, int x0,
                        brats_stream_t s);
int brats_sw_accumulate_multi(const float* prob, const float* importance, float* out, float* count, const int* windows,
                              int B, int NB, int K, int Dp, int Hp, int Wp, int rd, int rh, int rw, brats_stream_t s);
int brats_sw_finalize(const float* out, const float* count, float* dst, int NK, int Dp, int Hp, int Wp,
                      int D, int H, int W, int pad_z, int pad_y, int pad_x, brats_stream_t s);

int brats_spatial_signed_perm(const float* src, float* dst, int planes, int s0, int s1, int s2,
                              int p0, int p1, int p2, int f0, int f1, int f2, int mode, brats_stream_t s);

size_t brats_dice_ws_floats(int N, int K);
int brats_dice_stats(const float* logits, const float* target, float* sums , float* ws, int N, int K,
                     size_t voxels, brats_stream_t s);
int brats_dice_grad(const float* logits, const float* target, const float* coef ,
                    float* dlogits, int N, int K, size_t voxels, brats_stream_t s);

int brats_pad_crop(const float* src, float* dst, int planes, int sd, int sh, int sw, int dd, int dh,
                   int dw, int oz, int oy, int ox, float fill, brats_stream_t s);
int brats_post_threshold(const float* prob, const float* img, float* seg, uint8_t* labels, int N, int K,
                         int C, size_t voxels, float scale, float thresh, brats_stream_t s);
int brats_overlap_counts(const float* pred, const float* target, unsigned long long* counts, int NK,
                         size_t voxels, brats_stream_t s);

size_t brats_cc_ws_bytes(int N, int D, int H, int W);
int brats_cc_filter(uint8_t* labels, int N, int D, int H, int W, int min_size, void* ws, brats_stream_t s);
size_t brats_rare_fill_ws_bytes(int N, int D, int H, int W);
int brats_rare_fill(uint8_t* labels, int N, int D, int H, int W, int axis, int max_count, void* ws,
                    brats_stream_t s);

size_t brats_hausdorff_ws_bytes(int NK, int D, int H, int W);
int brats_hausdorff(const float* pred, const float* target, int NK, int D, int H, int W, double percentile, int directed,
                    float* out, void* ws, brats_stream_t s);

enum { BRATS_MASK_F32 = 0, BRATS_MASK_U8 = 1 };
size_t brats_edt_ws_bytes(int planes, int D, int H, int W);
int brats_edt(const void* mask, int mask_kind, int planes, int D, int H, int W, int mode, float* out, void* ws,
              brats_stream_t s);

size_t brats_dist_loss_ws_floats(void);
int brats_sigmoid_argmax_onehot(const float* logits, uint8_t* onehot, int N, int K, size_t voxels, brats_stream_t s);
int brats_hd_loss_stats(const float* logits, const float* target, const float* tdm, const float* pdm, float alpha,
                        float* sum, float* ws, size_t total, brats_stream_t s);
int brats_hd_loss_grad(const float* logits, const float* target, const float* tdm, const float* pdm, float alpha,
                       const float* scale, float* dlogits, size_t total, brats_stream_t s);
int brats_boundary_loss_stats(const float* logits, const float* dist, float* sum, float* ws, size_t total,
// ... 84 lines not shown
```

Before: 140.3 patches/s.

## Fuse GroupNorm+activation backward into first-layer weight-gradient kernel

For the first conv unit, where no input gradient is needed, the GN/activation backward elementwise step is no longer a separate pass that writes dy to memory. A small kernel now computes per-channel GN backward coefficients, and the all-taps wgrad kernel reads dz and y and rebuilds dy in registers before staging it to LDS. This removes one full-resolution read/write pass over the largest activation. The cost is extra loads and arithmetic inside the wgrad kernel and a larger LDS footprint, and the path applies only to bf16 ReLU/leaky layers with the 3x1 form.

```diff
diff --git a/brats21_amd/csrc/conv_wgrad.hip b/brats21_amd/csrc/conv_wgrad.hip
--- a/brats21_amd/csrc/conv_wgrad.hip
+++ b/brats21_amd/csrc/conv_wgrad.hip
@@ -1,6 +1,7 @@
 #include <stdlib.h>
 #include "twin_begin.hpp"
 #include "common.hpp"
+#include "gn_bwd_elem.hpp"
 
 typedef __attribute__((ext_vector_type(4))) short s16x4;
 
@@ -13,6 +14,9 @@
   int nlane;
   int ntaps, dil;
   int seglen, nsegz;
+  const void* gy; int gyp;
+  const float* coef;
+  int act; float slope;
 };
 
 constexpr int WG_TZ = 4, WG_TY = 4, WG_TX = 16, WG_VOX = 256;
@@ -436,15 +440,17 @@
   static constexpr int XB = XI * 512 * 16;
   static constexpr int LDS = 2 * XB + WG_VOX * SY;
   static constexpr int PAIRS = 27 * CIF, PPW = (PAIRS + 7) / 8;
+  static constexpr int COEF_LDS = CO * GN_BWD_COEFS * 4;
   static_assert(YPIECES % 512 == 0, "");
 };
 
-template <int COF, int CIF>
-__global__ __launch_bounds__(512, 1) void conv_wgrad_alltaps2_kernel(const WgradParams p) {
+template <int COF, int CIF, bool GN>
+DEVI void conv_wgrad_alltaps2_body(const WgradParams& p) {
   typedef bf16_t T;
   using G = Wg3b<COF, CIF>;
   extern __shared__ __attribute__((aligned(16))) char lds[];
   char* ldy = lds + 2 * G::XB;
+  float* ldc = (float*)(ldy + WG_VOX * G::SY);
   const int tid = threadIdx.x, lane = tid & 63;
   const int wave = __builtin_amdgcn_readfirstlane(tid >> 6);
   const int q = lane >> 4, v = lane & 15;
@@ -471,6 +477,8 @@
   }
   const unsigned xsample_bytes = (unsigned)p.D * p.H * p.W * xpitch * 2;
   const unsigned ysample_bytes = (unsigned)p.D * p.H * p.W * p.dyp * 2;
+  const int gpb = GN ? p.gyp * 2 : 0;
+  const unsigned gsample_bytes = GN ? (unsigned)p.D * p.H * p.W * p.gyp * 2 : 0u;
 
   int poff[G::PPW];
 #pragma unroll
@@ -486,10 +494,14 @@
     for (int m = 0; m < COF; ++m) acc[jj][m] = f32x4{0.f, 0.f, 0.f, 0.f};
 
   u32x4 ry[G::YI];
+  u32x4 rg[GN ? G::YI : 1];
+  unsigned okm = 0;
+  int n_next = 0, n_cur = -1;
+  const float nslope = GN ? act_neg_slope(p.act, p.slope) : 0.f;
   struct TileLoads {
     rsrc4_t xrs;
-    __amdgpu_buffer_rsrc_t yrs;
-    int xorg, yorg;
+    __amdgpu_buffer_rsrc_t yrs, grs;
+    int xorg, yorg, gorg;
     unsigned zm, ym, xm, inter;
     char* xdst;
   };
@@ -505,6 +517,11 @@
     L.yrs = __builtin_amdgcn_make_buffer_rsrc((void*)((const T*)p.dy + sample_vox * p.dyp + co0), (short)0, (int)ysample_bytes, 0x00020000);
     L.xorg = (((z0 - 1) * p.H + (y0 - 1)) * p.W + (x0 - 1)) * xpb;
     L.yorg = ((z0 * p.H + y0) * p.W + x0) * ypb;
+    if constexpr (GN) {
+      L.grs = __builtin_amdgcn_make_buffer_rsrc((void*)((const T*)p.gy + sample_vox * p.gyp + co0), (short)0, (int)gsample_bytes, 0x00020000);
+      L.gorg = ((z0 * p.H + y0) * p.W + x0) * gpb;
+      n_next = n;
+    }
     L.xdst = lds + buf * G::XB + wave * 1024;
     auto inside = [](int o, int size, int hn) {
       const int lo = o >= 1 ? 0 : 1 - o, hi = size - o + 1 < hn ? size - o + 1 : hn;
@@ -528,6 +545,31 @@
     const int yo = ((z * p.H + y) * p.W + x) * ypb + part * 16;
     const unsigned ok = (L.inter | ((L.zm >> (z + 1)) & (L.ym >> (y + 1)) & (L.xm >> (x + 1)))) & 1u;
     ry[i] = __builtin_bit_cast(u32x4, __builtin_amdgcn_raw_buffer_load_b128(L.yrs, (L.yorg + yo) | ((int)ok - 1), 0, 0));
+    if constexpr (GN) {
+      const int go = ((z * p.H + y) * p.W + x) * gpb + part * 16;
+      rg[i] = __builtin_bit_cast(u32x4, __builtin_amdgcn_raw_buffer_load_b128(L.grs, (L.gorg + go) | ((int)ok - 1), 0, 0));
+      okm = (okm & ~(1u << i)) | (ok << i);
+    }
+  };
+  auto compose_y = [&](auto i_) {
+    constexpr int i = i_;
+    const float* cf = ldc + ((tid + 512 * i) % G::YPPV) * 8;
+    float g[8], yy[8], o[8];
+#pragma unroll
+    for (int k = 0; k < 4; ++k) {
+      unpack2(ry[i][k], g[2 * k], g[2 * k + 1]);
+      unpack2(rg[i][k], yy[2 * k], yy[2 * k + 1]);
+    }
+#pragma unroll
+    for (int h = 0; h < 2; ++h) {
+      const f32x4 sc = *(const f32x4*)(cf + 4 * h), sh = *(const f32x4*)(cf + G::CO + 4 * h), ca = *(const f32x4*)(cf + 2 * G::CO + 4 * h),
+                  cb = *(const f32x4*)(cf + 3 * G::CO + 4 * h), ck = *(const f32x4*)(cf + 4 * G::CO + 4 * h);
+#pragma unroll
+      for (int j = 0; j < 4; ++j) o[4 * h + j] = gn_bwd_dy(g[4 * h + j], yy[4 * h + j], sc[j], sh[j], ca[j], cb[j], ck[j], nslope);
+    }
+    const uint32_t keep = 0u - ((okm >> i) & 1u);
+#pragma unroll
+    for (int k = 0; k < 4; ++k) ry[i][k] = pack2(o[2 * k], o[2 * k + 1]) & keep;
   };
 
   const int tile_first = lane8 * tpx + gsub;
@@ -548,6 +590,15 @@
   }
   for (int tile = tile_first; tile < tile_end; tile += g8, cur ^= 1) {
     WG_STAMP(4);
+    if constexpr (GN) {
+      if (n_next != n_cur) {
+        n_cur = n_next;
+        const float* src = p.coef + ((size_t)n_cur * p.cout + co0) * GN_BWD_COEFS;
+        for (int t = tid; t < G::CO * GN_BWD_COEFS; t += 512) ldc[(t % GN_BWD_COEFS) * G::CO + t / GN_BWD_COEFS] = src[t];
+        __syncthreads();
+      }
+      static_for<0, G::YI>([&](auto i_) { compose_y(i_); });
+    }
     asm volatile("s_waitcnt vmcnt(0)" ::: "memory");
     WG_STAMP(0);
     __syncthreads();
@@ -617,6 +668,14 @@
       }
     }
   }
+}
+
+template <int COF, int CIF>
+__global__ __launch_bounds__(512, 1) void conv_wgrad_alltaps2_kernel(const WgradParams p) {
+  conv_wgrad_alltaps2_body<COF, CIF, false>(p);
+}
+__global__ __launch_bounds__(512, 1) void conv_wgrad_alltaps2_gn_kernel(const WgradParams p) {
+  conv_wgrad_alltaps2_body<3, 1, true>(p);
 }
 
 template <int COF, int CIF> struct Wg3f {
@@ -930,6 +989,10 @@
   const void* x2; int c2, p2;
   const void* dy; int dyp;
   int N, D, H, W, cout;
+  bool gn = false;
+  const void* gy = nullptr; int gyp = 0;
+  const float* coef = nullptr;
+  int act = 0; float slope = 0.f;
   int cin() const { return c1 + c2; }
   size_t vox() const { return (size_t)N * D * H * W; }
 };
@@ -937,7 +1000,8 @@
   return WgradArgs{nullptr, c1, 0, nullptr, c2 > 0 ? c2 : 0, 0, nullptr, 0, N, D, H, W, cout};
 }
 static int wgrad_sample_overflow(const WgradArgs& a, int esize) {
-  const int mp = a.p1 > a.p2 ? (a.p1 > a.dyp ? a.p1 : a.dyp) : (a.p2 > a.dyp ? a.p2 : a.dyp);
+  int mp = a.p1 > a.p2 ? (a.p1 > a.dyp ? a.p1 : a.dyp) : (a.p2 > a.dyp ? a.p2 : a.dyp);
+  if (a.gyp > mp) mp = a.gyp;
   return (double)a.D * a.H * a.W * mp * esize >= 2147483648.0 ? mp : 0;
 }
 
@@ -954,6 +1018,7 @@
   p.N = a.N; p.D = a.D; p.H = a.H; p.W = a.W; p.cin = a.cin(); p.cout = a.cout;
   p.tz = t.tz; p.ty = t.ty; p.tx = t.tx; p.ntiles = t.ntiles;
   p.nlane = nlane; p.nsplit = nsplit; p.ntaps = ntaps; p.dil = dil;
+  p.gy = a.gy; p.gyp = a.gyp; p.coef = a.coef; p.act = a.act; p.slope = a.slope;
   return p;
 }
 
@@ -1001,6 +1066,7 @@
 enum WgradForm {
   WG_TAP_PLANE, WG_SHIFTED_TAP,
   WG_ALLTAPS2_33, WG_ALLTAPS2_42, WG_ALLTAPS2_31,
+  WG_ALLTAPS2_31_GN,
   WG_ALLTAPS_1, WG_ALLTAPS_1_4,
   WG_F8_33, WG_F8_42
 };
@@ -1030,6 +1096,7 @@
     pl.cot = cout / (16 * pl.cof); pl.cit = narrow ? 1 : cin / (16 * pl.cif);
     if (wgrad_blocks_g8(pl.tiles.ntiles, pl.cot * pl.cit, &pl.nlane, &pl.g8)) {
       pl.form = wide ? (narrow ? WG_ALLTAPS_1_4 : WG_ALLTAPS2_42) : narrow ? (c1 % 8 == 0 ? WG_ALLTAPS2_31 : WG_ALLTAPS_1) : WG_ALLTAPS2_33;
+      if (a.gn && pl.form == WG_ALLTAPS2_31) pl.form = WG_ALLTAPS2_31_GN;
       pl.groups = 1;
       pl.clear = false;
       pl.nsplit = pl.nlane * pl.g8;
@@ -1104,6 +1171,8 @@
     case WG_ALLTAPS2_33: return wgrad_alltaps_launch<conv_wgrad_alltaps2_kernel<3, 3>, Wg3b<3, 3>::LDS>(p, grid, st);
     case WG_ALLTAPS2_42: return wgrad_alltaps_launch<conv_wgrad_alltaps2_kernel<4, 2>, Wg3b<4, 2>::LDS>(p, grid, st);
     case WG_ALLTAPS2_31: return wgrad_alltaps_launch<conv_wgrad_alltaps2_kernel<3, 1>, Wg3b<3, 1>::LDS>(p, grid, st);
+    case WG_ALLTAPS2_31_GN:
+      return wgrad_alltaps_launch<conv_wgrad_alltaps2_gn_kernel, Wg3b<3, 1>::LDS + Wg3b<3, 1>::COEF_LDS>(p, grid, st);
     case WG_ALLTAPS_1: return wgrad_alltaps_launch<conv_wgrad_alltaps_kernel<1>, Wg3<1>::LDS>(p, grid, st);
     case WG_ALLTAPS_1_4: return wgrad_alltaps_launch<conv_wgrad_alltaps_kernel<1, 4>, Wg3<1, 4>::LDS>(p, grid, st);
     default: BRATS_FAIL(BRATS_E_UNSUPPORTED, "wgrad: form %d is not a 16-bit / f32 kernel", (int)pl.form);
@@ -1250,6 +1319,37 @@
                                   int D, int H, int W, int cout, brats_stream_t s) {
   return wgrad_impl(false, WgradArgs{x1, c1, pitch1, x2, c2, pitch2, dy, dypitch, N, D, H, W, cout}, nullptr, ws, dw, dbias, dtype, ksize, dil, s);
 }
+static bool wgrad_gn_form(int dtype, const WgradArgs& a, int act) {
+  if (dtype != BRATS_BF16 || (act != BRATS_ACT_RELU && act != BRATS_ACT_LEAKY) || a.c1 <= 0 || a.cout <= 0) return false;
+  if (a.N <= 0 || a.D <= 0 || a.H <= 0 || a.W <= 0) return false;
+  return wgrad_plan(dtype, false, 3, 1, a).form == WG_ALLTAPS2_31_GN;
+}
+extern "C" int BRATS_API(brats_conv3d_wgrad_gn_ok)(int dtype, int c1, int cout, int N, int D, int H, int W, int act) {
+  WgradArgs a = wgrad_shape(N, D, H, W, c1, 0, cout);
+  a.gn = true;
+  return wgrad_gn_form(dtype, a, act) ? 1 : 0;
+}
+extern "C" int BRATS_API(brats_conv3d_wgrad_gn)(const void* x, int c1, int xpitch, const void* dz, int dzpitch, const void* y, int ypitch,
+                                                const float* coef, int act, float slope, float* ws, float* dw, int dtype, int N, int D,
+                                                int H, int W, int cout, brats_stream_t s) {
+  if (!x || !dz || !y || !coef || !ws || !dw) BRATS_FAIL(BRATS_E_ARG, "wgrad_gn: null pointer");
+  WgradArgs a{x, c1, xpitch, nullptr, 0, 0, dz, dzpitch, N, D, H, W, cout};
+  a.gn = true; a.gy = y; a.gyp = ypitch; a.coef = coef; a.act = act; a.slope = slope;
+  if (!wgrad_gn_form(dtype, a, act))
+    BRATS_FAIL(BRATS_E_UNSUPPORTED, "wgrad_gn: not built for %d -> %d channels at %dx%dx%dx%d, dtype %d, act %d "
+               "(brats_conv3d_wgrad_gn_ok() == 0: use brats_gn_act_bwd_tiles + brats_conv3d_wgrad)", c1, cout, N, D, H, W, dtype, act);
+  if (xpitch % 8 || dzpitch % 8 || ypitch % 8 || xpitch < c1 || dzpitch < cout || ypitch < cout)
+    BRATS_FAIL(BRATS_E_ARG, "wgrad_gn: pitches must be multiples of 8 and cover the channels");
+  if (const int mp = wgrad_sample_overflow(a, 2))
+    BRATS_FAIL(BRATS_E_UNSUPPORTED, "wgrad_gn: one sample of %dx%dx%d x pitch %d exceeds the 2 GiB buffer-offset range", D, H, W, mp);
+  hipStream_t st = (hipStream_t)s;
+  const WgradPlan pl = wgrad_plan(dtype, false, 3, 1, a);
+  const int rc = wgrad_run(pl, dtype, 1, a, ws, pl.slab_bytes(), st);
+  if (rc) return rc;
+  wgrad_reduce_launch((const float*)ws, dw, pl.nsplit, a.cout, a.cin(), pl.ntaps, st);
+  BRATS_CHECK_LAUNCH();
+  return 0;
+}
 extern "C" int BRATS_API(brats_conv3d_x3_wgrad)(const void* x1, int c1, int pitch1, const void* x2, int c2, int pitch2, const void* dy,
                                      int dypitch, const float* amax_dy, float* ws, float* dw, float* dbias, int dtype, int dil,
                                      int N, int D, int H, int W, int cout, brats_stream_t s) {
diff --git a/brats21_amd/csrc/gn_bwd_elem.hpp b/brats21_amd/csrc/gn_bwd_elem.hpp
--- /dev/null
+++ b/brats21_amd/csrc/gn_bwd_elem.hpp
@@ -0,0 +1,16 @@
+#pragma once
+#include "common.hpp"
+
+DEVI float act_neg_slope(int act, float slope) { return act == BRATS_ACT_RELU ? 0.f : (act == BRATS_ACT_LEAKY ? slope : 1.f); }
+
+constexpr int GN_BWD_COEFS = 5;
+DEVI void gn_bwd_coefs(float gamma, float mean, float rstd, float m1, float m2, float& ca, float& cb, float& ck) {
+  ca = rstd * gamma;
+  cb = -rstd * rstd * m2;
+  ck = rstd * (mean * rstd * m2 - m1);
+}
+
+DEVI float gn_bwd_dy(float g, float y, float sc, float sh, float ca, float cb, float ck, float nslope) {
+  const float u = g * (y * sc + sh > 0.f ? 1.f : nslope);
+  return u * ca + (y * cb + ck);
+}
diff --git a/brats21_amd/csrc/norm.hip b/brats21_amd/csrc/norm.hip
--- a/brats21_amd/csrc/norm.hip
+++ b/brats21_amd/csrc/norm.hip
@@ -1,5 +1,6 @@
 #include "twin_begin.hpp"
 #include "common.hpp"
+#include "gn_bwd_elem.hpp"
 
 #include "se.hpp"
 
@@ -206,7 +207,6 @@
 DEVI float act_grad(float x, int act, float slope) {
   if (act == BRATS_ACT_RELU) return x > 0.f ? 1.f : 0.f;
   if (act == BRATS_ACT_LEAKY) return x > 0.f ? 1.f : slope;
-  if constexpr (!HEAVY) return 1.f;
   if (act == BRATS_ACT_ELU) return x > 0.f ? 1.f : __expf(x);
   if (act == BRATS_ACT_SWISH) {
     const float sg = 1.f / (1.f + __expf(-x));
@@ -783,9 +783,7 @@
     sh[j] = scale_shift[((size_t)n * C + c) * 2 + 1];
     const float mean = mean_rstd[(n * groups + g) * 2], rstd = mean_rstd[(n * groups + g) * 2 + 1];
     const float m1 = m12[g * 2], m2 = m12[g * 2 + 1];
-    ca[j] = rstd * gamma[c];
-    cb[j] = -rstd * rstd * m2;
-    ck[j] = rstd * (mean * rstd * m2 - m1);
+    gn_bwd_coefs(gamma[c], mean, rstd, m1, m2, ca[j], cb[j], ck[j]);
   }
   const T* dzb = dz + (size_t)n * voxels * dzpitch + c0;
   const T* yb = y + (size_t)n * voxels * ypitch + c0;
@@ -793,11 +791,16 @@
   const size_t stride = (size_t)gridDim.x * vl_n;
   size_t vox = live ? (size_t)blockIdx.x * vl_n + myvl : (size_t)voxels;
   float mx = 0.f;
+  const float nslope = act_neg_slope(act, slope);
   auto body = [&](const float* g, const float* yy, float* o) {
 #pragma unroll
     for (int j = 0; j < VW; ++j) {
-      const float u = g[j] * act_grad<HEAVY>(yy[j] * sc[j] + sh[j], act, slope);
-      o[j] = u * ca[j] + (yy[j] * cb[j] + ck[j]);
+      if constexpr (!HEAVY) {
+        o[j] = gn_bwd_dy(g[j], yy[j], sc[j], sh[j], ca[j], cb[j], ck[j], nslope);
+      } else {
+        const float u = g[j] * act_grad<HEAVY>(yy[j] * sc[j] + sh[j], act, slope);
+        o[j] = u * ca[j] + (yy[j] * cb[j] + ck[j]);
+      }
     }
     if (amax) {
 #pragma unroll
@@ -948,10 +951,8 @@
   return rc < 0 ? rc : 0;
 }
 
-__global__ void __launch_bounds__(256) gn_bwd_tiles_finish_kernel(const double* __restrict__ part, int splits, int N, int C, int groups,
-                                                                  const float* __restrict__ mean_rstd, float* __restrict__ red) {
-  const int i = blockIdx.x * blockDim.x + threadIdx.x;
-  if (i >= N * C) return;
+DEVI void gn_bwd_tiles_finish_one(const double* __restrict__ part, int splits, int N, int C, int groups,
+                                  const float* __restrict__ mean_rstd, float* __restrict__ red, int i) {
   const int n = i / C, c = i % C;
   double s1 = 0.0, s2 = 0.0;
   const double* src = part + ((size_t)n * C + c) * 2;
@@ -969,6 +970,74 @@
   const double mean = mean_rstd[(n * groups + g) * 2], rstd = mean_rstd[(n * groups + g) * 2 + 1];
   red[(size_t)i * 2] = (float)s1;
   red[(size_t)i * 2 + 1] = (float)(rstd * (s2 - mean * s1));
+}
+__global__ void __launch_bounds__(256) gn_bwd_tiles_finish_kernel(const double* __restrict__ part, int splits, int N, int C, int groups,
+                                                                  const float* __restrict__ mean_rstd, float* __restrict__ red) {
+  const int i = blockIdx.x * blockDim.x + threadIdx.x;
+  if (i >= N * C) return;
+  gn_bwd_tiles_finish_one(part, splits, N, C, groups, mean_rstd, red, i);
+}
+
+__global__ void __launch_bounds__(256) gn_bwd_tiles_coef_kernel(const double* __restrict__ part, int splits, int N, int C, int groups,
+                                                                int voxels, const float* __restrict__ scale_shift,
+                                                                const float* __restrict__ mean_rstd, const float* __restrict__ gamma,
+                                                                float* __restrict__ red, float* __restrict__ coef,
+                                                                float* __restrict__ dgamma, float* __restrict__ dbeta) {
+  extern __shared__ float m12[];
+  for (int i = threadIdx.x; i < N * C; i += blockDim.x) gn_bwd_tiles_finish_one(part, splits, N, C, groups, mean_rstd, red, i);
+  __syncthreads();
+  const int cpg = C / groups;
+  const float invM = 1.f / ((float)cpg * (float)voxels);
+  for (int i = threadIdx.x; i < N * groups; i += blockDim.x) {
+    const int n = i / groups, g = i % groups;
+    float t1 = 0.f, t2 = 0.f;
+    for (int j = 0; j < cpg; ++j) {
+      const int c = g * cpg + j;
+      t1 += gamma[c] * red[((size_t)n * C + c) * 2];
+      t2 += gamma[c] * red[((size_t)n * C + c) * 2 + 1];
+    }
+    m12[i * 2] = t1 * invM;
+    m12[i * 2 + 1] = t2 * invM;
+  }
+  if (dgamma) {
+    for (int c = threadIdx.x; c < C; c += blockDim.x) {
+      float b = 0.f, g = 0.f;
+      for (int m = 0; m < N; ++m) { b += red[((size_t)m * C + c) * 2]; g += red[((size_t)m * C + c) * 2 + 1]; }
+      dbeta[c] = b;
+      dgamma[c] = g;
+    }
+  }
+  __syncthreads();
+  for (int i = threadIdx.x; i < N * C; i += blockDim.x) {
+    const int n = i / C, c = i % C, g = c / cpg;
+    const float mean = mean_rstd[(n * groups + g) * 2], rstd = mean_rstd[(n * groups + g) * 2 + 1];
+    const float m1 = m12[(n * groups + g) * 2], m2 = m12[(n * groups + g) * 2 + 1];
+    float ca, cb, ck;
+    gn_bwd_coefs(gamma[c], mean, rstd, m1, m2, ca, cb, ck);
+    float* o = coef + (size_t)i * GN_BWD_COEFS;
+    o[0] = scale_shift[(size_t)i * 2];
+    o[1] = scale_shift[(size_t)i * 2 + 1];
+    o[2] = ca;
+    o[3] = cb;
+    o[4] = ck;
+  }
+}
+
+extern "C" int BRATS_API(brats_gn_bwd_tiles_coef)(const float* tile_stats, int tiles_per_sample, const float* scale_shift,
+                                                  const float* mean_rstd, const float* gamma, float* red, float* coef, float* dgamma,
+                                                  float* dbeta, int N, int voxels, int C, int groups, brats_stream_t s) {
+  if (!tile_stats || !red || !coef || !scale_shift || !mean_rstd || !gamma || tiles_per_sample <= 0)
+    BRATS_FAIL(BRATS_E_ARG, "gn_bwd_tiles_coef: null pointer");
+  if (N <= 0 || C <= 0 || groups <= 0 || C % groups || (size_t)N * groups * 2 * sizeof(float) > 32768)
+    BRATS_FAIL(BRATS_E_ARG, "gn_bwd_tiles_coef: N=%d C=%d groups=%d", N, C, groups);
+  hipStream_t st = (hipStream_t)s;
+  double* part = (double*)(red + (((size_t)N * C * 2 + 1) / 2) * 2);
+  const int splits = gn_splits(tiles_per_sample);
+  hipLaunchKernelGGL(gn_chan_reduce_kernel, dim3((C + 15) / 16, N, splits), dim3(256), 0, st, tile_stats, tiles_per_sample, C, part);
+  hipLaunchKernelGGL(gn_bwd_tiles_coef_kernel, dim3(1), dim3(256), (size_t)N * groups * 2 * sizeof(float), st, part, splits, N, C, groups,
+                     voxels, scale_shift, mean_rstd, gamma, red, coef, dgamma, dbeta);
+  BRATS_CHECK_LAUNCH();
+  return 0;
 }
 
 extern "C" int BRATS_API(brats_gn_act_bwd_tiles)(const float* tile_stats, int tiles_per_sample, const void* dz, int dzpitch, const void* y,
diff --git a/brats21_amd/networks/_program.py b/brats21_amd/networks/_program.py
--- a/brats21_amd/networks/_program.py
+++ b/brats21_amd/networks/_program.py
@@ -38,6 +38,7 @@
         self.fold_pool_bwd = os.environ.get("BRATS_FOLD_POOL", "1") != "0"
         self.fold_bwd_stats = os.environ.get("BRATS_FOLD_BWD_STATS", "1") != "0"
         self.fold_head_fwd = os.environ.get("BRATS_FOLD_HEAD_FWD", os.environ.get("BRATS_FOLD_HEAD", "1")) != "0"
+        self.fold_first_dy = os.environ.get("BRATS_FOLD_FIRST_DY", "1") != "0"
 
     def _init_dropout(self, p):
         if not 0.0 <= float(p) < 1.0:
diff --git a/brats21_amd/networks/equiunet.py b/brats21_amd/networks/equiunet.py
--- a/brats21_amd/networks/equiunet.py
+++ b/brats21_amd/networks/equiunet.py
@@ -283,6 +283,14 @@
     elif pool is not None:
         dy, dgamma, dbeta = ops.gn_act_bwd_pool(pool[0], pool[1], pool[2], y, scale_shift, mean_rstd, gamma_c,
                                                 unit.groups, kact, amax=amax)
+    elif (tiles is not None and not need_dx and cx.m.fold_first_dy and cx.drop is None and not unit.bcn and fp8 is None
+          and amax is None and slope_t is None and x2 is None and unit.dilation == 1 and ops.conv3d_wgrad_gn_ok(x, y, kact)):
+        coef, dgamma, dbeta = ops.gn_bwd_tiles_coef(tiles, y, scale_shift, mean_rstd, gamma_c, unit.groups)
+        dw = ops.conv3d_wgrad_gn(x, dz, y, coef, kact, out=cx.dest(unit.conv.weight))
+        dw = dw[:, :cin].contiguous() if dw.shape[1] != cin else dw
+        for prm, g in ((unit.conv.weight, dw), (unit.bn.weight, dgamma), (unit.bn.bias, dbeta)):
+            cx.put(prm, g)
+        return None
     elif tiles is not None:
         dy, dgamma, dbeta = ops.gn_act_bwd_tiles(tiles, dz, y, scale_shift, mean_rstd, gamma_c, unit.groups, kact,
                                                  amax=amax)
diff --git a/brats21_amd/ops.py b/brats21_amd/ops.py
--- a/brats21_amd/ops.py
+++ b/brats21_amd/ops.py
@@ -733,6 +733,46 @@
                                                  red.data_ptr(), dgamma.data_ptr(), dbeta.data_ptr(), _code(y.dtype), ACTS[act],
                                                  float(slope), n, d * h * w, c, groups, _f32(amax), _stream()), "gn_act_bwd_tiles")
     return dy, dgamma, dbeta
+
+
+def gn_bwd_tiles_coef(tile_stats, y, scale_shift, mean_rstd, gamma, groups=8):
+    n, d, h, w, c = y.shape
+    red = torch.empty(_lib.lib().brats_gn_bwd_ws_floats(n, c), dtype=torch.float32, device=y.device)
+    coef = torch.empty((n, c, 5), dtype=torch.float32, device=y.device)
+    dgamma = torch.empty(c, dtype=torch.float32, device=y.device)
+    dbeta = torch.empty(c, dtype=torch.float32, device=y.device)
+    _lib.check(_lib.lib().brats_gn_bwd_tiles_coef(tile_stats.data_ptr(), tile_stats.shape[1], scale_shift.data_ptr(),
+                                                  mean_rstd.data_ptr(), _f32(gamma), red.data_ptr(), coef.data_ptr(),
+                                                  dgamma.data_ptr(), dbeta.data_ptr(), n, d * h * w, c, groups, _stream()),
+               "gn_bwd_tiles_coef")
+    return coef, dgamma, dbeta
+
+
+def conv3d_wgrad_gn_ok(x, y, act="relu"):
+    n, d, h, w, c = x.shape
+    if not is16(x.dtype) or y.dtype != x.dtype or act not in ("relu", "leakyrelu"):
+        return False
+    return bool(_lib.lib().brats_conv3d_wgrad_gn_ok(_code(x.dtype), c, y.shape[-1], n, d, h, w, ACTS[act]))
+
+
+def conv3d_wgrad_gn(x, dz, y, coef, act="relu", slope=0.01, out=None):
+    ptr, c, p = _desc(x)
+    dzp, cout, dzpitch = _desc(dz)
+    yp, cy, ypitch = _desc(y)
+    n, d, h, w, _ = x.shape
+    if cy != cout or dz.dtype != x.dtype or y.dtype != x.dtype or tuple(dz.shape[:4]) != (n, d, h, w) or tuple(y.shape[:4]) != (n, d, h, w):
+        raise _lib.BratsHipError("conv3d_wgrad_gn: dz and y must have the layer output's shape and the input's dtype")
+    if tuple(coef.shape) != (n, cout, 5):
+        raise _lib.BratsHipError(f"conv3d_wgrad_gn: coef must be [N, cout, 5], got {tuple(coef.shape)}")
+    code = _code(x.dtype)
+    nbytes = _lib.lib().brats_conv3d_wgrad_ws_bytes(code, 3, n, d, h, w, c, 0, cout)
+    ws = torch.empty(max(nbytes, 4) // 4, dtype=torch.float32, device=x.device)
+    dw = _grad_out(out, (cout, c, 3, 3, 3), x.device)
+    with _span("conv_wgrad", c, cout, 3, 1, n, d, h, w, str(x.dtype)):
+        _lib.check(_lib.lib().brats_conv3d_wgrad_gn(ptr, c, p, dzp, dzpitch, yp, ypitch, _f32(coef), ACTS[act], float(slope),
+                                                    ws.data_ptr(), dw.data_ptr(), code, n, d, h, w, cout, _stream()),
+                   "conv3d_wgrad_gn")
+    return dw
 
 
 def gn_act_bwd_head(dlogits, head_weight, y, scale_shift, mean_rstd, gamma, groups=8, act="relu", slope=0.01, amax=None):
diff --git a/include/brats_hip.h b/include/brats_hip.h
--- a/include/brats_hip.h
+++ b/include/brats_hip.h
@@ -87,6 +87,10 @@
 int brats_conv3d_x3_wgrad(const void* x1, int c1, int pitch1, const void* x2, int c2, int pitch2, const void* dy, int dypitch,
                           const float* amax_dy, float* ws, float* dw, float* dbias, int dtype, int dil, int N, int D, int H,
                           int W, int cout, brats_stream_t s);
+int brats_conv3d_wgrad_gn_ok(int dtype, int c1, int cout, int N, int D, int H, int W, int act);
+int brats_conv3d_wgrad_gn(const void* x, int c1, int xpitch, const void* dz, int dzpitch, const void* y, int ypitch,
+                          const float* coef , int act, float slope, float* ws, float* dw, int dtype, int N,
+                          int D, int H, int W, int cout, brats_stream_t s);
 size_t brats_conv3d_wgrad_f8_ws_bytes(int N, int D, int H, int W, int c1, int c2, int cout);
 int brats_conv3d_wgrad_f8(const void* x1, int c1, int pitch1, const float* amax1, const void* x2, int c2, int pitch2,
                           const float* amax2, const void* dy, int dypitch, const float* amax_dy, float* ws, float* dw,
@@ -125,6 +129,9 @@
                            int dypitch, float* red , float* dgamma, float* dbeta, int dtype, int act,
                            float slope, int N, int voxels, int C, int groups,
                            float* amax , brats_stream_t s);
+int brats_gn_bwd_tiles_coef(const float* tile_stats, int tiles_per_sample, const float* scale_shift, const float* mean_rstd,
+                            const float* gamma, float* red , float* coef, float* dgamma, float* dbeta, int N,
+                            int voxels, int C, int groups, brats_stream_t s);
 size_t brats_gn_bwd_head_ws_floats(int N, int C, int K);
 int brats_gn_act_bwd_head(const float* dlogits, const float* hw, int K, const void* y, int ypitch, const float* scale_shift,
                           const float* mean_rstd, const float* gamma, void* dy, int dypitch, float* red ,
```

Measured after the change: 141.3 patches/s, median of 6. Within noise of the previous version (+0.7%).
